# docknetwork/crypto

Hardware: AMD Instinct MI355X
Metric: BLS12-381 G1 MSM/s at n=2^20 (1 GPU) and n=2^24 (8 GPU); bit-exact vs CPU (higher is better)
Workload: dtype i32 (13 signed 30-bit limbs, 381-bit modular integer; 64-bit column accumulators)

## Files before the change

### crypto_amd/csrc/k_g1_pre.hip

```cpp
#include "pre_kernels.hip.h"
#include "msm_launch.hip.h"
namespace msm {
template <class C> void launch_pre_step(hipStream_t s, const uint32_t *prev, size_t n, int c, uint32_t *tmp, uint32_t *out) {
    hipLaunchKernelGGL((k_pre_dbl<typename C::MSM>), dim3((unsigned)((n + 63) / 64)), dim3(64), 0, s, prev, n, c, tmp);
    const size_t groups = (n + PRE_GROUP - 1) / PRE_GROUP;
    hipLaunchKernelGGL((k_pre_norm<typename C::MSM>), dim3((unsigned)((groups + 63) / 64)), dim3(64), 0, s, prev, (const uint32_t *)tmp, n, out);
}
template void launch_pre_step<G1>(hipStream_t, const uint32_t *, size_t, int, uint32_t *, uint32_t *);
}
```

### crypto_amd/csrc/k_g2_pre.hip

```cpp
#include "pre_kernels.hip.h"
#include "msm_launch.hip.h"
namespace msm {
template <class C> void launch_pre_step(hipStream_t s, const uint32_t *prev, size_t n, int c, uint32_t *tmp, uint32_t *out) {
    hipLaunchKernelGGL((k_pre_dbl<typename C::MSM>), dim3((unsigned)((n + 63) / 64)), dim3(64), 0, s, prev, n, c, tmp);
    const size_t groups = (n + PRE_GROUP - 1) / PRE_GROUP;
    hipLaunchKernelGGL((k_pre_norm<typename C::MSM>), dim3((unsigned)((groups + 63) / 64)), dim3(64), 0, s, prev, (const uint32_t *)tmp, n, out);
}
template void launch_pre_step<G2>(hipStream_t, const uint32_t *, size_t, int, uint32_t *, uint32_t *);
}
```

### crypto_amd/csrc/k_psort.hip

```cpp
#include <atomic>
#include "psort_kernels.hip.h"
#include "sort_launch.hip.h"

namespace msm {
void launch_id_flags(hipStream_t s, const uint32_t *bases, int aff_stride, int flag_word, size_t n, uint8_t *out) {
    if (n) hipLaunchKernelGGL(k_id_flags, dim3((unsigned)((n + 255) / 256)), dim3(256), 0, s, bases, aff_stride, flag_word, n, out);
}
void launch_raw_record_hash(hipStream_t s, const uint8_t *raw, size_t stride, size_t x_off, size_t y_off, size_t inf_off, const uint8_t *is_inf, int words, size_t n, uint64_t *out) {
    if (n) hipLaunchKernelGGL(k_raw_record_hash, dim3((unsigned)((n + 255) / 256)), dim3(256), 0, s, raw, stride, x_off, y_off, inf_off, is_inf, words, n, out);
}
void launch_psort(hipStream_t s, const PsParams &q, uint32_t NB, uint32_t *cnt1, uint32_t *off1, uint32_t *bsums, void *pairs, uint32_t *off, uint32_t *entries,
                  uint32_t heavy_thr, uint32_t *heavy, uint32_t heavy_cap, const uint32_t *dyn_args, uint32_t *dyn) {
    const size_t lds1 = (size_t)q.P * 4;
    const size_t lds3 = ((size_t)4 * q.P + 2) * 4 + (size_t)PS_TILE * (size_t)q.W * 8;
    { static std::atomic<uint32_t> done{0}; int dev = 0; (void)hipGetDevice(&dev); const uint32_t bit = 1u << (dev & 31);
      if (!(done.load() & bit)) {
          (void)hipFuncSetAttribute((const void *)k_ps_scatter1<0, 0>, hipFuncAttributeMaxDynamicSharedMemorySize, 160 * 1024 - 2048);
          (void)hipFuncSetAttribute((const void *)k_ps_scatter1<20, 13>, hipFuncAttributeMaxDynamicSharedMemorySize, 160 * 1024 - 2048);
          (void)hipFuncSetAttribute((const void *)k_ps_scatter1<17, 16>, hipFuncAttributeMaxDynamicSharedMemorySize, 160 * 1024 - 2048);
          (void)hipFuncSetAttribute((const void *)k_ps_scatter1<16, 16>, hipFuncAttributeMaxDynamicSharedMemorySize, 160 * 1024 - 2048);
          done.fetch_or(bit); } }
    const int shape = (q.c == 20 && q.W == 13) ? 1 : ((q.c == 17 && q.W == 16) ? 2 : ((q.c == 16 && q.W == 16) ? 3 : 0));
    if (shape == 1) hipLaunchKernelGGL((k_ps_count1<20, 13>), dim3(q.ntiles), dim3(PS_TILE), lds1, s, q, cnt1);
    else if (shape == 2) hipLaunchKernelGGL((k_ps_count1<17, 16>), dim3(q.ntiles), dim3(PS_TILE), lds1, s, q, cnt1);
    else if (shape == 3) hipLaunchKernelGGL((k_ps_count1<16, 16>), dim3(q.ntiles), dim3(PS_TILE), lds1, s, q, cnt1);
    else hipLaunchKernelGGL((k_ps_count1<0, 0>), dim3(q.ntiles), dim3(PS_TILE), lds1, s, q, cnt1);
    launch_scan(s, cnt1, off1, nullptr, bsums, (size_t)q.P * q.ntiles);
    if (dyn) launch_dyn_chunk(s, off1 + (size_t)q.P * q.ntiles, dyn_args[0], dyn_args[1], dyn_args[2], dyn_args[3], dyn_args[4], dyn, dyn_args[5]);
    if (shape == 1) hipLaunchKernelGGL((k_ps_scatter1<20, 13>), dim3(q.ntiles), dim3(PS_TILE), lds3, s, q, (const uint32_t *)cnt1, (const uint32_t *)off1, (uint2 *)pairs);
    else if (shape == 2) hipLaunchKernelGGL((k_ps_scatter1<17, 16>), dim3(q.ntiles), dim3(PS_TILE), lds3, s, q, (const uint32_t *)cnt1, (const uint32_t *)off1, (uint2 *)pairs);
    else if (shape == 3) hipLaunchKernelGGL((k_ps_scatter1<16, 16>), dim3(q.ntiles), dim3(PS_TILE), lds3, s, q, (const uint32_t *)cnt1, (const uint32_t *)off1, (uint2 *)pairs);
    else hipLaunchKernelGGL((k_ps_scatter1<0, 0>), dim3(q.ntiles), dim3(PS_TILE), lds3, s, q, (const uint32_t *)cnt1, (const uint32_t *)off1, (uint2 *)pairs);
    const int wc = ((uint64_t)q.n * (uint64_t)q.W) / q.P >= PS_WC_MIN_PAIRS ? 1 : 0;
    const size_t lds4 = wc ? (size_t)2 * PS_PART * 4 + (size_t)PS_WC_TILE * 8 : (size_t)PS_DIRECT_CAP * 4;
    if (!wc) { static std::atomic<uint32_t> done5{0}; int dev = 0; (void)hipGetDevice(&dev); const uint32_t bit = 1u << (dev & 31);
      if (!(done5.load() & bit)) { (void)hipFuncSetAttribute((const void *)k_ps_bucket<false>, hipFuncAttributeMaxDynamicSharedMemorySize, (int)lds4); done5.fetch_or(bit); } }
    if (wc) { static std::atomic<uint32_t> done4{0}; int dev = 0; (void)hipGetDevice(&dev); const uint32_t bit = 1u << (dev & 31);
      if (!(done4.load() & bit)) { (void)hipFuncSetAttribute((const void *)k_ps_bucket<true>, hipFuncAttributeMaxDynamicSharedMemorySize, (int)lds4); done4.fetch_or(bit); } }
    if (wc) hipLaunchKernelGGL(k_ps_bucket<true>, dim3(q.P), dim3(1024), lds4, s, (const uint2 *)pairs, off1, q.ntiles, q.P, NB, q.part_log, off, entries, heavy_thr, heavy, heavy_cap, (const uint32_t *)dyn);
    else hipLaunchKernelGGL(k_ps_bucket<false>, dim3(q.P), dim3(1024), lds4, s, (const uint2 *)pairs, off1, q.ntiles, q.P, NB, q.part_log, off, entries, heavy_thr, heavy, heavy_cap, (const uint32_t *)dyn);
}
}
```

### crypto_amd/csrc/msm_driver.hip.h

```cpp
#pragma once
#include <chrono>
#include <thread>
#include "dock_ctx.hpp"
#include "bases_cache.hpp"
#include "host_field.hpp"
#include "msm_launch.hip.h"
#include "sort_launch.hip.h"
#include "qap_launch.hip.h"

namespace dock {
using namespace msm;

template <class HF>
void host_fold(const uint64_t *win_abi, const uint8_t *win_inf, int W, int c, uint64_t *out_xyz) {
    typedef hostf::HXyzz<HF> PT;
    PT acc = PT::identity();
    const size_t FWORDS = sizeof(HF) / 8;
    for (int w = W - 1; w >= 0; w--) {
        if (!acc.inf) for (int k = 0; k < c; k++) acc.dbl_in_place();
        if (!win_inf[w]) {
            PT t; t.inf = false;
            const uint64_t *src = win_abi + (size_t)w * 4 * FWORDS;
            memcpy(&t.x, src, sizeof(HF)); memcpy(&t.y, src + FWORDS, sizeof(HF)); memcpy(&t.zz, src + 2 * FWORDS, sizeof(HF)); memcpy(&t.zzz, src + 3 * FWORDS, sizeof(HF));
            acc.add_in_place(t);
        }
    }
    HF X, Y, Z; acc.to_normalised_jacobian(X, Y, Z);
    memcpy(out_xyz, &X, sizeof(HF)); memcpy(out_xyz + FWORDS, &Y, sizeof(HF)); memcpy(out_xyz + 2 * FWORDS, &Z, sizeof(HF));
}

template <class HF>
int32_t host_fold_jacobian(const uint64_t *xyz, size_t k, uint64_t *out_xyz) {
    if (!out_xyz || (k && !xyz)) return DGPU_E_BADARG;
    typedef hostf::HXyzz<HF> PT;
    const size_t FWORDS = sizeof(HF) / 8;
    PT acc = PT::identity();
    for (size_t i = 0; i < k; i++) {
        HF X, Y, Z;
        memcpy(&X, xyz + i * 3 * FWORDS, sizeof(HF)); memcpy(&Y, xyz + i * 3 * FWORDS + FWORDS, sizeof(HF)); memcpy(&Z, xyz + i * 3 * FWORDS + 2 * FWORDS, sizeof(HF));
        if (Z.is_zero()) continue;
        PT t; t.inf = false; t.x = X; t.y = Y; t.zz = Z * Z; t.zzz = t.zz * Z;
        acc.add_in_place(t);
    }
    HF X, Y, Z; acc.to_normalised_jacobian(X, Y, Z);
    memcpy(out_xyz, &X, sizeof(HF)); memcpy(out_xyz + FWORDS, &Y, sizeof(HF)); memcpy(out_xyz + 2 * FWORDS, &Z, sizeof(HF));
    return DGPU_OK;
}

template <class HF>
int32_t host_lincomb(const uint64_t *points_xy, const uint8_t *is_inf, const uint64_t *scalars, size_t k, uint64_t *out_xyz) {
    if (!out_xyz || k > DGPU_MAX_LINCOMB || (k && (!points_xy || !scalars))) return DGPU_E_BADARG;
    typedef hostf::HXyzz<HF> PT;
    const size_t FWORDS = sizeof(HF) / 8;
    std::vector<PT> tab(k * 15);
    std::vector<uint8_t> live(k, 0);
    for (size_t i = 0; i < k; i++) {
        HF X, Y;
        memcpy(&X, points_xy + i * 2 * FWORDS, sizeof(HF)); memcpy(&Y, points_xy + i * 2 * FWORDS + FWORDS, sizeof(HF));
        const uint64_t *sc = scalars + 4 * i;
        uint64_t any = 0; for (size_t w = 0; w < 2 * FWORDS; w++) any |= points_xy[i * 2 * FWORDS + w];
        if ((is_inf && is_inf[i]) || !any || !(sc[0] | sc[1] | sc[2] | sc[3])) continue;
        live[i] = 1;
        PT p; p.inf = false; p.x = X; p.y = Y; p.zz = HF::one(); p.zzz = HF::one();
        tab[i * 15] = p;
        for (int m = 1; m < 15; m++) { PT t = tab[i * 15 + m - 1]; if (m == 1) t.dbl_in_place(); else t.add_in_place(p); tab[i * 15 + m] = t; }
    }
    PT acc = PT::identity();
    for (int w = 63; w >= 0; w--) {
        for (int d = 0; d < 4; d++) acc.dbl_in_place();
        for (size_t i = 0; i < k; i++) {
            if (!live[i]) continue;
            const unsigned nib = (unsigned)(scalars[4 * i + (w >> 4)] >> ((w & 15) * 4)) & 15u;
            if (nib) acc.add_in_place(tab[i * 15 + nib - 1]);
        }
    }
    HF X, Y, Z; acc.to_normalised_jacobian(X, Y, Z);
    memcpy(out_xyz, &X, sizeof(HF)); memcpy(out_xyz + FWORDS, &Y, sizeof(HF)); memcpy(out_xyz + 2 * FWORDS, &Z, sizeof(HF));
    return DGPU_OK;
}

template <class HF> void write_identity(uint64_t *out_xyz) {
    typedef hostf::HXyzz<HF> PT; PT id = PT::identity(); HF X, Y, Z; id.to_normalised_jacobian(X, Y, Z);
    const size_t FWORDS = sizeof(HF) / 8; memcpy(out_xyz, &X, sizeof(HF)); memcpy(out_xyz + FWORDS, &Y, sizeof(HF)); memcpy(out_xyz + 2 * FWORDS, &Z, sizeof(HF));
}

constexpr size_t PLAIN_PSORT_MIN_N = (size_t)1 << 17;
struct PlainGeom {
    int c, W; uint32_t B, NB; int mshift, G; size_t NG, Emax; int CH; size_t T, nblk; bool wide; size_t n_pad; int RANGES, rb_log; unsigned sort_grid; size_t lds_bytes;
    uint32_t min_chunk, max_chunks, lanes_per_chunk, HEAVY_CAP;
    bool psort;
};
template <class C> int32_t plain_geometry(size_t n, PlainGeom &g) {
    if (n >= (1ull << 31)) return DGPU_E_BADARG;
    g.c = choose_c(n, C::NFP == 2);
    g.W = 255 / g.c + 1;
    g.B = 1u << (g.c - 1);
    if ((uint64_t)g.W * g.B >= (1ull << 31) || (uint64_t)n * g.W >= (1ull << 32)) return DGPU_E_BADARG;
    g.NB = (uint32_t)g.W * g.B;
    g.mshift = std::max(0, g.c - 1 - 12);
    g.G = (int)(g.B >> (6 + g.mshift));
    g.NG = (size_t)g.W * g.G;
    g.Emax = (size_t)n * g.W;
    g.CH = C::NFP == 2 ? choose_chunk(g.Emax, 32, 150000, 2) : choose_chunk(g.Emax, 16, 300000, 1);
    g.T = (g.Emax + g.CH - 1) / g.CH;
    g.nblk = scan_blocks(g.NB);
    g.wide = g.c > 16;
    g.n_pad = (n + 7) & ~(size_t)7;
    g.RANGES = 1; while ((g.B / g.RANGES) * 4 > 64 * 1024 || g.W * g.RANGES < 256) { if (g.B / g.RANGES <= 64) break; g.RANGES *= 2; }
    g.rb_log = 0; while ((1u << g.rb_log) < g.B / g.RANGES) g.rb_log++;
    g.sort_grid = (unsigned)(8 * ((g.W + 7) / 8) * g.RANGES);
    g.lds_bytes = ((size_t)1 << g.rb_log) * 4;
    g.min_chunk = C::NFP == 2 ? 32u : 16u; g.max_chunks = C::NFP == 2 ? 150000u : 300000u; g.lanes_per_chunk = C::NFP == 2 ? 2u : 1u;
    g.HEAVY_CAP = (uint32_t)(g.Emax / (16u * 16u)) + 1;
    g.psort = g.W <= PS_MAX_W && n >= PLAIN_PSORT_MIN_N;
    return DGPU_OK;
}
template <class C> int32_t ws_plain(Slot &sl, const PlainGeom &g) {
    int32_t rc;
    const size_t NB = g.NB, T = g.T;
    if ((rc = sl.flags.ensure(64))) return rc;
    if ((rc = sl.cnt.ensure((NB + 1) * 4))) return rc;
    if ((rc = sl.off.ensure((NB + 1) * 4))) return rc;
    if ((rc = sl.cursor.ensure((NB + 1) * 4))) return rc;
    if ((rc = sl.bsums.ensure((g.nblk + 2) * 4))) return rc;
    if ((rc = sl.entries.ensure(g.Emax * 4))) return rc;
    if ((rc = sl.bucket.ensure(soa_points(NB) * C::XW * 4))) return rc;
    if ((rc = sl.bucket_inf.ensure(NB))) return rc;
    if ((rc = sl.head.ensure(soa_points(T) * C::XW * 4))) return rc;
    if ((rc = sl.tail.ensure(soa_points(T) * C::XW * 4))) return rc;
    if ((rc = sl.head_b.ensure(T * 4))) return rc;
    if ((rc = sl.tail_b.ensure(T * 4))) return rc;
    if ((rc = sl.part_inf.ensure(T * 2))) return rc;
    if ((rc = sl.l1.ensure(g.NG * 2 * C::XW * 4))) return rc;
    if ((rc = sl.l1_inf.ensure(g.NG * 2))) return rc;
    if ((rc = sl.win.ensure((size_t)g.W * 4 * C::ABI_W * 4))) return rc;
    if ((rc = sl.win_inf.ensure(g.W))) return rc;
    if ((rc = sl.digits.ensure((size_t)g.W * g.n_pad * (g.wide ? 4 : 2)))) return rc;
    if (g.psort) {
        const size_t n_terms = g.Emax / g.W;
        const uint32_t P = (g.NB + (1u << ps_part_log(g.NB)) - 1) >> ps_part_log(g.NB);
        const size_t n1 = (size_t)P * ((n_terms + PS_TILE - 1) / PS_TILE);
        if ((rc = sl.cnt.ensure((n1 + 1) * 4))) return rc;
        if ((rc = sl.cursor.ensure((n1 + 1) * 4))) return rc;
        if ((rc = sl.bsums.ensure((scan_blocks(n1) + 2) * 4))) return rc;
        if ((rc = sl.digits.ensure(g.Emax * 8))) return rc;
    }
    if ((rc = sl.heavy.ensure(((size_t)g.HEAVY_CAP + 1) * 4))) return rc;
    if ((rc = sl.dyn.ensure(msm::dyn_words(T) * 4))) return rc;
    { const size_t hslots = 2 * (T / msm::HEAVY_RANGE + 2); if ((rc = sl.hpart.ensure(hslots * C::XW * 4))) return rc; if ((rc = sl.hpart_inf.ensure(hslots))) return rc; }
    return DGPU_OK;
}

inline size_t range_count(size_t n, bool operands_in_flight) { return operands_in_flight && n >= ((size_t)1 << 19) ? 2 : 1; }
inline size_t range_lo(size_t n, size_t K, size_t k) { return ((n * k / K) + 7) & ~(size_t)7; }
inline void range_bounds(size_t n, size_t K, size_t k, size_t &lo, size_t &hi) { lo = k == 0 ? 0 : std::min(n, range_lo(n, K, k)); hi = k + 1 == K ? n : std::min(n, range_lo(n, K, k + 1)); }
template <class C> int32_t ws_bucket_sets(Slot &sl, uint32_t NB, size_t K) {
    int32_t rc;
    if ((rc = sl.bucket.ensure(K * soa_points(NB) * C::XW * 4))) return rc;
    return sl.bucket_inf.ensure(K * (size_t)NB);
}

struct SmallSub { const uint32_t *tab; const uint8_t *tab_inf; };
template <class C> inline size_t small_sub_tab_bytes(size_t n) { return n * SMALL_MSM_S * SMALL_MSM_E * (size_t)C::ACC::XW * 4; }
template <class C> inline size_t small_sub_bytes(size_t n) { return small_sub_tab_bytes<C>(n) + n * SMALL_MSM_S * SMALL_MSM_E; }
template <class C> inline SmallSub small_sub_at(const void *aux, size_t handle_n, size_t offset) {
    const uint8_t *base = (const uint8_t *)aux;
    return SmallSub{(const uint32_t *)base + offset * SMALL_MSM_S * SMALL_MSM_E * (size_t)C::ACC::XW, base + small_sub_tab_bytes<C>(handle_n) + offset * SMALL_MSM_S * SMALL_MSM_E};
}
template <class C> int32_t ws_small(Slot &sl, size_t n) {
    int32_t rc;
    typedef typename C::ACC A;
    if ((rc = sl.bucket.ensure(n * SMALL_MSM_E * A::XW * 4))) return rc;
    if ((rc = sl.bucket_inf.ensure(n * SMALL_MSM_E))) return rc;
    if ((rc = sl.head.ensure((size_t)256 * A::XW * 4))) return rc;
    if ((rc = sl.part_inf.ensure(256))) return rc;
    if (!sl.small_cnt.p) {
        if ((rc = sl.small_cnt.ensure((size_t)SMALL_MSM_W * 4))) return rc;
        if (hipMemsetAsync(sl.small_cnt.p, 0, (size_t)SMALL_MSM_W * 4, sl.stream) != hipSuccess) { (void)hipGetLastError(); sl.small_cnt.release(); return DGPU_E_HIP; }
    }
    return sl.win.ensure((size_t)SMALL_MSM_W * 4 * C::ABI_W * 4 + 2 * SMALL_MSM_W);
}
template <class C, class HF, class ReadyS, class ReadyB>
int32_t msm_device_small(Slot &sl, const uint32_t *d_bases, const uint32_t *d_scalars, size_t n, uint64_t *out_xyz, ReadyS ready_scalars, ReadyB ready_bases, const SmallSub *sub = nullptr) {
    int32_t rc;
    if ((rc = ws_small<C>(sl, sub ? 1 : n))) return rc;
    hipStream_t s = sl.stream;
    constexpr int c = SMALL_MSM_C;
    const int S = sub ? SMALL_MSM_S : 1, W = SMALL_MSM_W / S;
    if ((rc = ready_scalars(0, 0, n))) return rc;
    if ((rc = ready_bases(0, 0, n))) return rc;
    constexpr size_t WBYTES = (size_t)SMALL_MSM_W * 4 * C::ABI_W * 4;
    static_assert(WBYTES + 2 * SMALL_MSM_W <= Slot::HPIN_BYTES, "pinned scratch");
    uint8_t *const hbuf = (uint8_t *)sl.hpin;
    uint8_t *const wbuf = hbuf;
    uint8_t *const d_inf = wbuf + WBYTES, *const d_bad = d_inf + SMALL_MSM_W;
    if (!sub) {
        StageTimer st(sl, "msm.small_table");
        launch_small_table<C>(s, d_bases, n, sl.bucket.as<uint32_t>(), sl.bucket_inf.as<uint8_t>());
    }
    {
        StageTimer st(sl, "msm.small_tree");
        launch_small_tree<C>(s, sub ? sub->tab : sl.bucket.as<uint32_t>(), sub ? sub->tab_inf : sl.bucket_inf.as<uint8_t>(), S, d_scalars, n, sl.head.as<uint32_t>(), sl.part_inf.as<uint8_t>(),
                             sl.small_cnt.as<uint32_t>(), (uint32_t *)wbuf, d_inf, d_bad);
    }
    HIPCHK(hipGetLastError());
    HIPCHK(hipStreamSynchronize(s));
    if (gs.prof) prof_flush(sl);
    const uint64_t *hwin = (const uint64_t *)hbuf; const uint8_t *hinf = hbuf + WBYTES, *hbad = hinf + SMALL_MSM_W;
    for (int w = 0; w < W; w++) if (hbad[w]) return DGPU_E_BADARG;
    host_fold<HF>(hwin, hinf, W, c, out_xyz);
    return DGPU_OK;
}

template <class C, class HF, class ReadyS, class ReadyB>
int32_t msm_device_ranges(Slot &sl, const uint32_t *d_bases, const uint32_t *d_scalars, size_t n, size_t K, uint64_t *out_xyz, bool bases_pending, ReadyS ready_scalars, ReadyB ready_bases, const SmallSub *sub = nullptr) {
    if (n == 0) { write_identity<HF>(out_xyz); return DGPU_OK; }
    if (K == 1 && n <= gs.small_max.load() && n <= SMALL_MSM_MAX_N) return msm_device_small<C, HF>(sl, d_bases, d_scalars, n, out_xyz, ready_scalars, ready_bases, sub);
    PlainGeom g; int32_t rc;
    if ((rc = plain_geometry<C>(n, g))) return rc;
    if ((rc = ws_plain<C>(sl, g))) return rc;
    if (K > 1 && (rc = ws_bucket_sets<C>(sl, g.NB, K))) return rc;
    const int c = g.c, W = g.W; const uint32_t NB = g.NB; const size_t T = g.T; const int CH = g.CH;
    hipStream_t s = sl.stream;
    const uint32_t heavy_thr = 0xffffffffu , HEAVY_CAP = g.HEAVY_CAP;
    uint32_t *const dyn = sl.dyn.as<uint32_t>();
    const size_t set_words = soa_points(NB) * C::XW;
    HIPCHK(hipMemsetAsync(sl.bucket_inf.p, 1, K * (size_t)NB, s));
    HIPCHK(hipMemsetAsync(sl.flags.p, 0, 4, s));
    for (size_t k = 0; k < K; k++) {
        size_t lo, hi; range_bounds(n, K, k, lo, hi);
        const size_t nk = hi - lo, nk_pad = (nk + 7) & ~(size_t)7;
        if (nk == 0) continue;
        uint32_t *const bucket = sl.bucket.as<uint32_t>() + k * set_words;
        uint8_t *const bucket_inf = sl.bucket_inf.as<uint8_t>() + k * (size_t)NB;
        const uint32_t *const bases_k = d_bases + lo * C::AFF_STRIDE, *const scalars_k = d_scalars + lo * 8;
        if ((rc = ready_scalars(k, lo, hi))) return rc;
        if (g.psort) {
            StageTimer st(sl, "msm.psort");
            PsParams q;
            q.scalars = scalars_k; q.idflag = nullptr ; q.n = nk; q.flag_base = 0;
            q.c = c; q.W = W; q.key_wstride = g.B; q.val_base = 0; q.val_wstride = 0;
            q.part_log = ps_part_log(NB); q.P = (NB + (1u << q.part_log) - 1) >> q.part_log; q.ntiles = (uint32_t)((nk + PS_TILE - 1) / PS_TILE);
            q.bad = sl.flags.as<uint32_t>();
            const uint32_t dyn_args[6] = {(uint32_t)forced_chunk(), g.min_chunk, g.max_chunks, g.lanes_per_chunk, (uint32_t)T, 0u};
            HIPCHK(hipMemsetAsync(sl.heavy.p, 0, 4, s));
            launch_psort(s, q, NB, sl.cnt.as<uint32_t>(), sl.cursor.as<uint32_t>(), sl.bsums.as<uint32_t>(), sl.digits.p, sl.off.as<uint32_t>(), sl.entries.as<uint32_t>(),
                         16u * (uint32_t)CH , sl.heavy.as<uint32_t>(), HEAVY_CAP, dyn_args, dyn);
        } else {
        {
            StageTimer st(sl, "msm.count");
            HIPCHK(hipMemsetAsync(sl.heavy.p, 0, 4, s));
            launch_digit_codes(s, g.wide, scalars_k, bases_pending ? nullptr : bases_k, C::AFF_STRIDE, C::FLAGW, nk, nk_pad, c, W, sl.digits.p, sl.flags.as<uint32_t>());
            launch_sort_sweep(s, g.wide, false, g.sort_grid, g.lds_bytes, sl.digits.p, nk, nk_pad, W, g.RANGES, g.rb_log, g.B, sl.cnt.as<uint32_t>(), nullptr, nullptr, heavy_thr, sl.heavy.as<uint32_t>(), HEAVY_CAP);
        }
        {
            StageTimer st(sl, "msm.scan");
            launch_scan(s, sl.cnt.as<uint32_t>(), sl.off.as<uint32_t>(), sl.cursor.as<uint32_t>(), sl.bsums.as<uint32_t>(), (size_t)NB);
            launch_dyn_chunk(s, sl.off.as<uint32_t>() + NB, (uint32_t)forced_chunk(), g.min_chunk, g.max_chunks, g.lanes_per_chunk, (uint32_t)T, dyn);
            launch_flag_heavy(s, sl.off.as<uint32_t>(), NB, dyn, sl.heavy.as<uint32_t>(), HEAVY_CAP);
        }
        {
            StageTimer st(sl, "msm.scatter");
            launch_sort_sweep(s, g.wide, true, g.sort_grid, g.lds_bytes, sl.digits.p, nk, nk_pad, W, g.RANGES, g.rb_log, g.B, nullptr, sl.off.as<uint32_t>(), sl.entries.as<uint32_t>(), heavy_thr, sl.heavy.as<uint32_t>(), HEAVY_CAP);
        }
        }
        if ((rc = ready_bases(k, lo, hi))) return rc;
        {
            StageTimer st(sl, "msm.accumulate");
#ifdef DGPU_DEV
            static const uint32_t dbg_mask = getenv("DGPU_DBG_NOGATHER") ? 1023u : 0xffffffffu;
#else
            constexpr uint32_t dbg_mask = 0xffffffffu;
#endif
            if (bases_pending || g.psort) launch_accumulate_skip_identity<C>(s, bases_k, sl.entries.as<uint32_t>(), sl.off.as<uint32_t>(), NB, bucket, bucket_inf,
                               sl.head.as<uint32_t>(), sl.tail.as<uint32_t>(), sl.head_b.as<uint32_t>(), sl.tail_b.as<uint32_t>(), sl.part_inf.as<uint8_t>(), T, (uint32_t)CH, dyn, msm::RowMap{});
            else launch_accumulate<C>(s, bases_k, sl.entries.as<uint32_t>(), sl.off.as<uint32_t>(), NB, bucket, bucket_inf,
                               sl.head.as<uint32_t>(), sl.tail.as<uint32_t>(), sl.head_b.as<uint32_t>(), sl.tail_b.as<uint32_t>(), sl.part_inf.as<uint8_t>(), T, (uint32_t)CH, dbg_mask, dyn);
        }
        {
            StageTimer st(sl, "msm.fixup");
            launch_fixup<C>(s, NB, bucket, bucket_inf, sl.head.as<uint32_t>(), sl.tail.as<uint32_t>(),
                               sl.head_b.as<uint32_t>(), sl.tail_b.as<uint32_t>(), sl.part_inf.as<uint8_t>(), T, sl.off.as<uint32_t>(), heavy_thr, dyn);
            launch_fixup_heavy<C>(s, sl.heavy.as<uint32_t>(), HEAVY_CAP, sl.off.as<uint32_t>(), (uint32_t)CH, NB, bucket, bucket_inf,
                               sl.head.as<uint32_t>(), sl.tail.as<uint32_t>(), sl.part_inf.as<uint8_t>(), T, dyn, sl.hpart.as<uint32_t>(), sl.hpart_inf.as<uint8_t>());
            if (k > 0) launch_merge_buckets<C>(s, NB, sl.bucket.as<uint32_t>(), sl.bucket_inf.as<uint8_t>(), bucket, bucket_inf);
        }
    }
    {
        StageTimer st(sl, "msm.reduce");
        launch_reduce_l0<C>(s, (unsigned)g.NG, sl.bucket.as<uint32_t>(), sl.bucket_inf.as<uint8_t>(), NB, g.mshift, sl.l1.as<uint32_t>(), sl.l1_inf.as<uint8_t>());
        launch_reduce_top<C>(s, (unsigned)W, sl.l1.as<uint32_t>(), sl.l1_inf.as<uint8_t>(), g.G, 6 + g.mshift, sl.win.as<uint32_t>(), sl.win_inf.as<uint8_t>(), gs.reduce_lanes.load() == 1 ? 1 : 4);
    }
    HIPCHK(hipGetLastError());
    std::vector<uint64_t> hwin((size_t)W * 2 * C::ABI_W);
    std::vector<uint8_t> hinf(W);
    const size_t wb = (size_t)W * 4 * C::ABI_W * 4, ib = ((size_t)W + 7) & ~(size_t)7;
    static_assert((size_t)64 * 4 * 24 * 4 + 64 + 16 <= Slot::HPIN_BYTES, "pinned scratch");
    std::vector<uint8_t> big;
    if (wb + ib + 4 > Slot::HPIN_BYTES) big.resize(wb + ib + 4);
    uint8_t *const hp = big.empty() ? (uint8_t *)sl.hpin : big.data();
    HIPCHK(hipMemcpyAsync(hp, sl.win.p, wb, hipMemcpyDeviceToHost, s));
    HIPCHK(hipMemcpyAsync(hp + wb, sl.win_inf.p, W, hipMemcpyDeviceToHost, s));
    HIPCHK(hipMemcpyAsync(hp + wb + ib, sl.flags.p, 4, hipMemcpyDeviceToHost, s));
    auto tsync0 = std::chrono::steady_clock::now();
    HIPCHK(hipStreamSynchronize(s));
    auto tsync1 = std::chrono::steady_clock::now();
    if (gs.prof) prof_flush(sl);
    uint32_t hbad; memcpy(&hbad, hp + wb + ib, 4);
    if (hbad) return DGPU_E_BADARG;
    memcpy(hwin.data(), hp, wb); memcpy(hinf.data(), hp + wb, W);
    host_fold<HF>(hwin.data(), hinf.data(), W, c, out_xyz);
    if (gs.prof) {
        auto t2 = std::chrono::steady_clock::now();
        prof_add_host("msm.host_wait", std::chrono::duration<double, std::milli>(tsync1 - tsync0).count());
        prof_add_host("msm.host_fold", std::chrono::duration<double, std::milli>(t2 - tsync1).count());
    }
    return DGPU_OK;
}
template <class C, class HF>
int32_t msm_device(Slot &sl, const uint32_t *d_bases, const uint32_t *d_scalars, size_t n, uint64_t *out_xyz, const SmallSub *sub = nullptr) {
    auto nothing = [](size_t, size_t, size_t) { return (int32_t)DGPU_OK; };
    return msm_device_ranges<C, HF>(sl, d_bases, d_scalars, n, 1, out_xyz, false, nothing, nothing, sub);
}

template <class C>
bool small_sub_for(Slot &sl, uint64_t handle_id, const Handle &h, size_t offset, size_t n, SmallSub &out, bool force = false) {
    if (h.n == 0 || h.n > SMALL_MSM_MAX_N || n > gs.small_max.load()) return false;
    void *aux = nullptr;
    {
        std::lock_guard<std::mutex> lk(gs.mu);
        auto it = gs.handles.find(handle_id);
        if (it == gs.handles.end()) return false;
        aux = it->second.aux;
        if (!aux && !force && ++it->second.small_uses < 2) return false;
    }
    if (!aux) {
        std::lock_guard<std::mutex> build(gs.small_mu);
        { std::lock_guard<std::mutex> lk(gs.mu); auto it = gs.handles.find(handle_id); if (it == gs.handles.end()) return false; aux = it->second.aux; }
        if (!aux) {
            void *p = nullptr;
            if (dev_malloc(&p, small_sub_bytes<C>(h.n)) != hipSuccess) { (void)hipGetLastError(); return false; }
            {
                StageTimer st(sl, "msm.small_subtable");
                launch_small_subtable<C>(sl.stream, (const uint32_t *)h.p, h.n, (uint32_t *)p, (uint8_t *)p + small_sub_tab_bytes<C>(h.n));
            }
            if (hipGetLastError() != hipSuccess || hipStreamSynchronize(sl.stream) != hipSuccess) { (void)hipGetLastError(); (void)hipFree(p); return false; }
            std::lock_guard<std::mutex> lk(gs.mu);
            auto it = gs.handles.find(handle_id);
            if (it == gs.handles.end()) { (void)hipFree(p); return false; }
            it->second.aux = aux = p;
        }
    }
    out = small_sub_at<C>(aux, h.n, offset);
    return true;
}

inline void shard_bounds(size_t n, size_t parts, std::vector<size_t> &lo) {
    lo.resize(parts + 1);
    const size_t base = n / parts, rem = n % parts;
    for (size_t k = 0; k <= parts; k++) lo[k] = k * base + std::min(k, rem);
}
template <class F> int32_t run_shards(size_t parts, F body) { return par_run(parts, body); }

inline int choose_c_pre(size_t n) {
    if (gs.window_bits.load() >= 16 && gs.window_bits.load() <= 22) return gs.window_bits.load();
    if (n < (1u << 15)) return 0;
    return n >= 320000 ? 20 : 16;
}

template <class HF>
void host_fold_shared(const uint64_t *a_abi, const uint8_t *a_inf, const uint64_t *s_abi, const uint8_t *s_inf, int PW, int lb, uint64_t *out_xyz) {
    typedef hostf::HXyzz<HF> PT;
    const size_t FWORDS = sizeof(HF) / 8;
    auto load = [&](const uint64_t *src, bool inf) { PT t = PT::identity(); if (!inf) { t.inf = false; memcpy(&t.x, src, sizeof(HF)); memcpy(&t.y, src + FWORDS, sizeof(HF)); memcpy(&t.zz, src + 2 * FWORDS, sizeof(HF)); memcpy(&t.zzz, src + 3 * FWORDS, sizeof(HF)); } return t; };
    PT suffix = PT::identity(), weighted = PT::identity(), total = PT::identity();
    for (int j = PW - 1; j >= 1; j--) { suffix.add_in_place(load(s_abi + (size_t)j * 4 * FWORDS, s_inf[j] != 0)); weighted.add_in_place(suffix); }
    for (int k = 0; k < lb; k++) weighted.dbl_in_place();
    for (int j = 0; j < PW; j++) total.add_in_place(load(a_abi + (size_t)j * 4 * FWORDS, a_inf[j] != 0));
    total.add_in_place(weighted);
    HF X, Y, Z; total.to_normalised_jacobian(X, Y, Z);
    memcpy(out_xyz, &X, sizeof(HF)); memcpy(out_xyz + FWORDS, &Y, sizeof(HF)); memcpy(out_xyz + 2 * FWORDS, &Z, sizeof(HF));
}

template <class HF>
void host_fold_marginals(const uint64_t *pts, const uint8_t *inf, int nm, int shift, uint64_t *out_xyz) {
    typedef hostf::HXyzz<HF> PT;
    const size_t FWORDS = sizeof(HF) / 8;
    auto load = [&](int i) { PT t = PT::identity(); if (!inf[i]) { const uint64_t *src = pts + (size_t)i * 4 * FWORDS; t.inf = false; memcpy(&t.x, src, sizeof(HF)); memcpy(&t.y, src + FWORDS, sizeof(HF)); memcpy(&t.zz, src + 2 * FWORDS, sizeof(HF)); memcpy(&t.zzz, src + 3 * FWORDS, sizeof(HF)); } return t; };
    PT acc = PT::identity();
    for (int t = nm - 1; t >= 0; t--) { if (!acc.inf) acc.dbl_in_place(); acc.add_in_place(load(1 + t)); }
    if (!acc.inf) for (int k = 0; k < shift; k++) acc.dbl_in_place();
    acc.add_in_place(load(0));
    HF X, Y, Z; acc.to_normalised_jacobian(X, Y, Z);
    memcpy(out_xyz, &X, sizeof(HF)); memcpy(out_xyz + FWORDS, &Y, sizeof(HF)); memcpy(out_xyz + 2 * FWORDS, &Z, sizeof(HF));
}

struct PreGeom { uint32_t NB; int mshift, lb, PW, G; size_t NG, Emax, T; int CH; uint32_t min_chunk, max_chunks, lanes_per_chunk, HEAVY_CAP; };
template <class C> int32_t pre_geometry(const PreTable &pt, size_t n, PreGeom &g) {
    const int c = pt.c, W = pt.W;
    g.NB = 1u << (c - 1);
    g.mshift = g.NB >= (1u << 18) ? 3 : (g.NB >= (1u << 17) ? 2 : (g.NB >= (1u << 16) ? 1 : 0));
    if (g.NB >= (1u << 19) && cur().busy.load() >= 3) g.mshift = 4;
    { const int f = gs.reduce_shift.load(); if (f >= 0 && c - 1 >= 6 + f) g.mshift = f; }
    g.lb = std::min(c - 1, 12 + g.mshift);
    g.PW = (int)(g.NB >> g.lb);
    g.G = 1 << (g.lb - 6 - g.mshift);
    g.NG = (size_t)g.PW * g.G;
    g.Emax = (size_t)n * W;
    if (g.Emax >= (1ull << 32) || (uint64_t)W * pt.n >= (1ull << 31) || W > PS_MAX_W) return DGPU_E_BADARG;
    g.CH = C::NFP == 2 ? choose_chunk(g.Emax, 32, 150000, 2) : choose_chunk(g.Emax, 16, 300000, 1);
    g.T = (g.Emax + g.CH - 1) / g.CH;
    g.min_chunk = C::NFP == 2 ? 32u : 16u; g.max_chunks = C::NFP == 2 ? 150000u : 300000u; g.lanes_per_chunk = C::NFP == 2 ? 2u : 1u;
    g.HEAVY_CAP = (uint32_t)(g.Emax / (16u * 16u)) + 1;
    return DGPU_OK;
}
template <class C> int32_t ws_pre(Slot &sl, const PreTable &pt, const PreGeom &g, size_t n) {
    const uint32_t NB = g.NB; const size_t T = g.T; const int PW = g.PW;
    const uint32_t P = (NB + (1u << ps_part_log(NB)) - 1) >> ps_part_log(NB);
    const size_t n1 = (size_t)P * ((n + PS_TILE - 1) / PS_TILE);
    int32_t rc;
    if ((rc = sl.flags.ensure(64))) return rc;
    if ((rc = sl.cnt.ensure((n1 + 1) * 4))) return rc;
    if ((rc = sl.cursor.ensure((n1 + 1) * 4))) return rc;
    if ((rc = sl.bsums.ensure((scan_blocks(n1) + 2) * 4))) return rc;
    if ((rc = sl.digits.ensure(g.Emax * 8))) return rc;
    if ((rc = sl.heavy.ensure(((size_t)g.HEAVY_CAP + 1) * 4))) return rc;
    if ((rc = sl.off.ensure(((size_t)NB + 1) * 4))) return rc;
    if ((rc = sl.entries.ensure(g.Emax * 4))) return rc;
    if ((rc = sl.bucket.ensure(soa_points(NB) * C::XW * 4))) return rc;
    if ((rc = sl.bucket_inf.ensure(NB))) return rc;
    if ((rc = sl.head.ensure(soa_points(T) * C::XW * 4))) return rc;
    if ((rc = sl.tail.ensure(soa_points(T) * C::XW * 4))) return rc;
    if ((rc = sl.head_b.ensure(T * 4))) return rc;
    if ((rc = sl.tail_b.ensure(T * 4))) return rc;
    if ((rc = sl.part_inf.ensure(T * 2))) return rc;
    const size_t NGw = std::max(g.NG, (size_t)(NB >> 9)), PWw = std::max((size_t)PW, (size_t)(NB >> 15));
    const size_t mpts = reduce_marginals_points<C>(NGw);
    if ((rc = sl.l1.ensure(std::max(NGw * 2, mpts) * C::XW * 4))) return rc;
    if ((rc = sl.l1_inf.ensure(std::max(NGw * 2, mpts)))) return rc;
    if ((rc = sl.win.ensure(std::max((size_t)2 * PWw, (size_t)32) * 4 * C::ABI_W * 4))) return rc;
    if ((rc = sl.win_inf.ensure(std::max((size_t)2 * PWw, (size_t)32)))) return rc;
    if ((rc = sl.dyn.ensure(msm::dyn_words(T) * 4))) return rc;
    { const size_t hslots = 2 * (T / msm::HEAVY_RANGE + 2); if ((rc = sl.hpart.ensure(hslots * C::XW * 4))) return rc; if ((rc = sl.hpart_inf.ensure(hslots))) return rc; }
    (void)pt;
    return DGPU_OK;
}
template <class C> inline size_t pre_rows_bytes(size_t n, int W) { return (size_t)W * n * C::AFF_STRIDE * 4; }
template <class C> inline size_t pre_tab_bytes(size_t n, int W) { return pre_rows_bytes<C>(n, W) + ((n + 15) & ~(size_t)15); }
template <class C> inline const uint8_t *pre_idflags(const PreTable &pt) { return (const uint8_t *)pt.tab + pre_rows_bytes<C>(pt.n, pt.W); }
inline size_t pre_off_bytes(const PreTable &pt) { return (((size_t)1 << (pt.c - 1)) + 1) * 4; }
inline size_t pre_entries_bytes(const PreTable &pt, size_t n) { return (size_t)n * pt.W * 4; }

template <class C>
int32_t pre_sort(Slot &sl, const PreTable &pt, const PreGeom &g, size_t boff, const uint32_t *d_scalars, size_t n, uint32_t *off, uint32_t *entries, uint32_t *dyn, bool reset_flag = true) {
    PsParams q;
    q.scalars = d_scalars; q.idflag = dyn ? pre_idflags<C>(pt) : nullptr ; q.n = n; q.flag_base = (uint32_t)boff;
    q.c = pt.c; q.W = pt.W; q.key_wstride = 0; q.val_base = (uint32_t)boff; q.val_wstride = (uint32_t)pt.n;
    q.part_log = ps_part_log(g.NB); q.P = (g.NB + (1u << q.part_log) - 1) >> q.part_log; q.ntiles = (uint32_t)((n + PS_TILE - 1) / PS_TILE);
    int32_t rc;
    if ((rc = ws_pre<C>(sl, pt, g, n))) return rc;
    q.bad = sl.flags.as<uint32_t>();
    const uint32_t heavy_thr = dyn ? 16u * (uint32_t)g.CH  : 0xffffffffu ;
    const uint32_t dyn_args[6] = {(uint32_t)forced_chunk(), g.min_chunk, g.max_chunks, g.lanes_per_chunk, (uint32_t)g.T, g.NB};
    StageTimer st(sl, "msm.psort");
    HIPCHK(hipMemsetAsync(sl.heavy.p, 0, 4, sl.stream));
    if (reset_flag) HIPCHK(hipMemsetAsync(sl.flags.p, 0, 4, sl.stream));
    launch_psort(sl.stream, q, g.NB, sl.cnt.as<uint32_t>(), sl.cursor.as<uint32_t>(), sl.bsums.as<uint32_t>(), sl.digits.p, off, entries,
                 heavy_thr, sl.heavy.as<uint32_t>(), g.HEAVY_CAP, dyn_args, dyn);
    return DGPU_OK;
}
template <class C>
int32_t pre_acc(Slot &sl, const PreTable &pt, const PreGeom &g, const uint32_t *off, const uint32_t *entries, bool derive_dyn, const msm::RowMap &map, size_t set) {
    const uint32_t NB = g.NB; const size_t T = g.T;
    uint32_t *const dyn = sl.dyn.as<uint32_t>();
    const uint32_t heavy_thr = 16u * (uint32_t)g.CH;
    hipStream_t s = sl.stream;
    uint32_t *const bucket = sl.bucket.as<uint32_t>() + set * soa_points(NB) * C::XW;
    uint8_t *const bucket_inf = sl.bucket_inf.as<uint8_t>() + set * (size_t)NB;
    HIPCHK(hipMemsetAsync(bucket_inf, 1, NB, s));
    if (derive_dyn) {
        HIPCHK(hipMemsetAsync(sl.heavy.p, 0, 4, s));
        launch_dyn_chunk(s, off + NB, (uint32_t)forced_chunk(), g.min_chunk, g.max_chunks, g.lanes_per_chunk, (uint32_t)T, dyn, NB);
        launch_flag_heavy(s, off, NB, dyn, sl.heavy.as<uint32_t>(), g.HEAVY_CAP);
    }
    {
        StageTimer st(sl, "msm.accumulate");
        if (derive_dyn) launch_accumulate_skip_identity<C>(s, (const uint32_t *)pt.tab, entries, off, NB, bucket, bucket_inf,
                           sl.head.as<uint32_t>(), sl.tail.as<uint32_t>(), sl.head_b.as<uint32_t>(), sl.tail_b.as<uint32_t>(), sl.part_inf.as<uint8_t>(), T, (uint32_t)g.CH, dyn, map);
        else launch_accumulate<C>(s, (const uint32_t *)pt.tab, entries, off, NB, bucket, bucket_inf,
                           sl.head.as<uint32_t>(), sl.tail.as<uint32_t>(), sl.head_b.as<uint32_t>(), sl.tail_b.as<uint32_t>(), sl.part_inf.as<uint8_t>(), T, (uint32_t)g.CH, 0xffffffffu, dyn);
    }
    {
        StageTimer st(sl, "msm.fixup");
        launch_fixup<C>(s, NB, bucket, bucket_inf, sl.head.as<uint32_t>(), sl.tail.as<uint32_t>(),
                           sl.head_b.as<uint32_t>(), sl.tail_b.as<uint32_t>(), sl.part_inf.as<uint8_t>(), T, off, heavy_thr, dyn);
        launch_fixup_heavy<C>(s, sl.heavy.as<uint32_t>(), g.HEAVY_CAP, off, (uint32_t)g.CH, NB, bucket, bucket_inf,
                           sl.head.as<uint32_t>(), sl.tail.as<uint32_t>(), sl.part_inf.as<uint8_t>(), T, dyn, sl.hpart.as<uint32_t>(), sl.hpart_inf.as<uint8_t>());
        if (set > 0) launch_merge_buckets<C>(s, NB, sl.bucket.as<uint32_t>(), sl.bucket_inf.as<uint8_t>(), bucket, bucket_inf);
    }
    return DGPU_OK;
}
template <class C, class HF>
int32_t pre_finish(Slot &sl, const PreGeom &g, bool check_flag, uint64_t *out_xyz) {
    const uint32_t NB = g.NB; const int PW = g.PW;
    hipStream_t s = sl.stream;
    uint32_t *win_a = sl.win.as<uint32_t>(), *win_s = win_a + (size_t)PW * 4 * C::ABI_W;
    uint8_t *inf_a = sl.win_inf.as<uint8_t>(), *inf_s = inf_a + PW;
    const int rl = gs.reduce_lanes.load();
    const bool marginals = (rl == 0 || rl == 2) && g.NG >= 2;
    int nm = 0;
    {
        StageTimer st(sl, "msm.reduce");
        if (marginals) nm = launch_reduce_marginals<C>(s, (unsigned)g.NG, sl.bucket.as<uint32_t>(), sl.bucket_inf.as<uint8_t>(), NB, g.mshift, sl.l1.as<uint32_t>(), sl.l1_inf.as<uint8_t>(), win_a, inf_a, rl == 0);
        else {
            launch_reduce_l0<C>(s, (unsigned)g.NG, sl.bucket.as<uint32_t>(), sl.bucket_inf.as<uint8_t>(), NB, g.mshift, sl.l1.as<uint32_t>(), sl.l1_inf.as<uint8_t>());
            launch_reduce_top_s<C>(s, (unsigned)PW, sl.l1.as<uint32_t>(), sl.l1_inf.as<uint8_t>(), g.G, 6 + g.mshift, win_a, inf_a, win_s, inf_s, gs.reduce_lanes.load() == 1 ? 1 : 4);
        }
    }
    HIPCHK(hipGetLastError());
    const size_t npts = marginals ? (size_t)nm + 1 : (size_t)2 * PW;
    std::vector<uint64_t> hwin(npts * 2 * C::ABI_W);
    std::vector<uint8_t> hinf(npts);
    const size_t wb = npts * 4 * C::ABI_W * 4, ib = (npts + 7) & ~(size_t)7;
    std::vector<uint8_t> big;
    if (wb + ib + 4 > Slot::HPIN_BYTES) big.resize(wb + ib + 4);
    uint8_t *const hp = big.empty() ? (uint8_t *)sl.hpin : big.data();
    memset(hp + wb + ib, 0, 4);
    HIPCHK(hipMemcpyAsync(hp, sl.win.p, wb, hipMemcpyDeviceToHost, s));
    HIPCHK(hipMemcpyAsync(hp + wb, sl.win_inf.p, npts, hipMemcpyDeviceToHost, s));
    if (check_flag) HIPCHK(hipMemcpyAsync(hp + wb + ib, sl.flags.p, 4, hipMemcpyDeviceToHost, s));
    auto tsync0 = std::chrono::steady_clock::now();
    HIPCHK(hipStreamSynchronize(s));
    auto tsync1 = std::chrono::steady_clock::now();
    if (gs.prof) prof_flush(sl);
    uint32_t hbad; memcpy(&hbad, hp + wb + ib, 4);
    if (hbad) return DGPU_E_BADARG;
    memcpy(hwin.data(), hp, wb); memcpy(hinf.data(), hp + wb, npts);
    if (marginals) host_fold_marginals<HF>(hwin.data(), hinf.data(), nm, g.mshift + (C::NFP == 2 ? 1 : 0), out_xyz);
    else host_fold_shared<HF>(hwin.data(), hinf.data(), hwin.data() + (size_t)PW * 2 * C::ABI_W, hinf.data() + PW, PW, g.lb, out_xyz);
    if (gs.prof) {
        auto t2 = std::chrono::steady_clock::now();
        prof_add_host("msm.host_wait", std::chrono::duration<double, std::milli>(tsync1 - tsync0).count());
        prof_add_host("msm.host_fold", std::chrono::duration<double, std::milli>(t2 - tsync1).count());
    }
    return DGPU_OK;
}
template <class C, class HF>
int32_t pre_tail(Slot &sl, const PreTable &pt, const PreGeom &g, const uint32_t *off, const uint32_t *entries, bool derive_dyn, uint64_t *out_xyz, const msm::RowMap &map = msm::RowMap{}) {
    int32_t rc;
    if ((rc = ws_pre<C>(sl, pt, g, g.Emax / pt.W))) return rc;
    if ((rc = pre_acc<C>(sl, pt, g, off, entries, derive_dyn, map, 0))) return rc;
    return pre_finish<C, HF>(sl, g, !derive_dyn, out_xyz);
}
template <class C, class HF, class ReadyS>
int32_t msm_device_pre_ranges(Slot &sl, const PreTable &pt, size_t boff, const uint32_t *d_scalars, size_t n, size_t K, uint64_t *out_xyz, ReadyS ready_scalars) {
    if (n == 0) { write_identity<HF>(out_xyz); return DGPU_OK; }
    PreGeom g; int32_t rc;
    if ((rc = pre_geometry<C>(pt, n, g))) return rc;
    if ((rc = ws_pre<C>(sl, pt, g, n))) return rc;
    if (K > 1 && (rc = ws_bucket_sets<C>(sl, g.NB, K))) return rc;
    HIPCHK(hipMemsetAsync(sl.flags.p, 0, 4, sl.stream));
    for (size_t k = 0; k < K; k++) {
        size_t lo, hi; range_bounds(n, K, k, lo, hi);
        if (hi == lo) continue;
        if ((rc = ready_scalars(k, lo, hi))) return rc;
        if ((rc = pre_sort<C>(sl, pt, g, boff + lo, d_scalars + lo * 8, hi - lo, sl.off.as<uint32_t>(), sl.entries.as<uint32_t>(), sl.dyn.as<uint32_t>(), false))) return rc;
        if ((rc = pre_acc<C>(sl, pt, g, sl.off.as<uint32_t>(), sl.entries.as<uint32_t>(), false, msm::RowMap{}, k))) return rc;
    }
    return pre_finish<C, HF>(sl, g, true, out_xyz);
}
template <class C, class HF>
int32_t msm_device_pre(Slot &sl, const PreTable &pt, size_t boff, const uint32_t *d_scalars, size_t n, uint64_t *out_xyz) {
    return msm_device_pre_ranges<C, HF>(sl, pt, boff, d_scalars, n, 1, out_xyz, [](size_t, size_t, size_t) { return (int32_t)DGPU_OK; });
}

inline int32_t scalars_sort(uint64_t table, size_t boff, uint64_t scalars, size_t soff, size_t n, uint64_t *sorted) {
    if (!sorted || n == 0) return DGPU_E_BADARG;
    if (!cur().ready) return DGPU_E_NODEVICE;
    HandleRef hb(table), hs(scalars);
    if (!hb.ok || !hs.ok || (hb.h.kind != 10 && hb.h.kind != 11) || hs.h.kind != 3 || hb.h.ctx != hs.h.ctx) return DGPU_E_BADARG;
    if (boff > hb.h.n || n > hb.h.n - boff || soff > hs.h.n || n > hs.h.n - soff) return DGPU_E_BADARG;
    CtxScope on_owner(hb.h.ctx);
    SLOT_ACQUIRE(L, sl);
    HIPCHK(hipSetDevice(cur().device));
    const PreTable &pt = *(const PreTable *)hb.h.p;
    PreGeom g; int32_t rc;
    if ((rc = pre_geometry<G1>(pt, n, g))) return rc;
    SortedScalars *ss = new SortedScalars{nullptr, nullptr, pre_off_bytes(pt), pre_entries_bytes(pt, n), n, pt.n, boff, pt.c, pt.W};
    ss->off = scalar_alloc(ss->off_bytes); ss->entries = scalar_alloc(ss->entries_bytes);
    auto drop = [&]() { scalar_release(cur_index(), ss->off, ss->off_bytes); scalar_release(cur_index(), ss->entries, ss->entries_bytes); delete ss; };
    if (!ss->off || !ss->entries) { drop(); return DGPU_E_OOM; }
    rc = pre_sort<G1>(sl, pt, g, boff, (const uint32_t *)hs.h.p + soff * 8, n, (uint32_t *)ss->off, (uint32_t *)ss->entries, nullptr);
    uint32_t hbad = 0;
    if (!rc && hipMemcpyAsync(&hbad, sl.flags.p, 4, hipMemcpyDeviceToHost, sl.stream) != hipSuccess) rc = DGPU_E_HIP;
    if (!rc && hipStreamSynchronize(sl.stream) != hipSuccess) { gs.last_hip = (int32_t)hipGetLastError(); rc = DGPU_E_HIP; }
    if (gs.prof) prof_flush(sl);
    if (!rc && hbad) rc = DGPU_E_BADARG;
    if (rc) { drop(); return rc; }
    *sorted = register_handle(ss, n, 12);
    return DGPU_OK;
}
template <class C, class HF>
int32_t msm_sorted(uint64_t table, uint64_t sorted, size_t row_shift, uint64_t *out, int kind) {
    if (!out) return DGPU_E_BADARG;
    if (!cur().ready) return DGPU_E_NODEVICE;
    HandleRef hb(table), hs(sorted);
    if (!hb.ok || !hs.ok || hb.h.kind != kind + 9 || hs.h.kind != 12 || hb.h.ctx != hs.h.ctx) return DGPU_E_BADARG;
    const PreTable &pt = *(const PreTable *)hb.h.p;
    const SortedScalars &ss = *(const SortedScalars *)hs.h.p;
    if (pt.c != ss.c || pt.W != ss.W || row_shift >= ss.rows || pt.n != ss.rows - row_shift) return DGPU_E_BADARG;
    CtxScope on_owner(hb.h.ctx);
    SLOT_ACQUIRE(L, sl);
    HIPCHK(hipSetDevice(cur().device));
    PreGeom g; int32_t rc;
    if ((rc = pre_geometry<C>(pt, ss.n, g))) return rc;
    msm::RowMap map;
    if (row_shift) {
        map.rows_src = (uint32_t)ss.rows; map.rows_dst = (uint32_t)pt.n; map.shift = (uint32_t)row_shift;
        map.magic = ~(uint64_t)0 / ss.rows + 1;
    }
    return pre_tail<C, HF>(sl, pt, g, (const uint32_t *)ss.off, (const uint32_t *)ss.entries, true, out, map);
}

template <class C> int32_t reserve_slots(int what, size_t n, size_t stride, const PreTable *pt);

template <class C>
int32_t bases_precompute(uint64_t handle, int32_t window_bits, int kind ) {
    if (window_bits != 0 && (window_bits < 16 || window_bits > 22)) return DGPU_E_BADARG;
    Handle hd;
    { Handle peek; if (!lookup_handle(handle, peek)) return DGPU_E_BADARG;
      if (peek.kind == kind + 6) {
          HandleRef ref(handle); if (!ref.ok) return DGPU_E_BADARG;
          const ShardSet &ss = *(const ShardSet *)ref.h.p;
          return run_shards(ss.sub.size(), [&](size_t k) { return bases_precompute<C>(ss.sub[k], window_bits, kind); });
      }
      if (peek.kind == kind + 9) return DGPU_OK; }
    if (!take_handle(handle, [kind](int k) { return k == kind; }, hd)) return DGPU_E_BADARG;
    auto put_back = [&](void *p, int k) { std::lock_guard<std::mutex> lk(gs.mu); gs.handles[handle] = Handle{p, hd.n, k, hd.ctx, 0, k == kind ? hd.aux : nullptr, hd.small_uses}; };
    CtxScope on_owner(hd.ctx);
    if (!cur().ready) { put_back(hd.p, kind); return DGPU_E_NODEVICE; }
    const size_t n = hd.n;
    const int c = window_bits ? window_bits : choose_c_pre(n);
    if (c == 0) {
        put_back(hd.p, kind);
        if (n && n <= SMALL_MSM_MAX_N) {
            HandleRef ref(handle);
            if (ref.ok) { SlotLock L; if (L.ok && hipSetDevice(cur().device) == hipSuccess) { SmallSub sub; (void)small_sub_for<C>(*L.s, handle, ref.h, 0, 0, sub, true); } }
        }
        return DGPU_OK;
    }
    const int W = 255 / c + 1;
    if (n == 0 || (uint64_t)W * n >= (1ull << 31)) { put_back(hd.p, kind); return n == 0 ? DGPU_OK : DGPU_E_BADARG; }
    void *tab = nullptr, *tmp = nullptr;
    int32_t rc = DGPU_OK;
    {
        SLOT_ACQUIRE(L, sl);
        if (hipSetDevice(cur().device) != hipSuccess) rc = DGPU_E_HIP;
        const size_t rec = (size_t)C::AFF_STRIDE * 4;
        if (!rc && dev_malloc(&tab, pre_tab_bytes<C>(n, W)) != hipSuccess) { (void)hipGetLastError(); rc = DGPU_E_OOM; }
        if (!rc && dev_malloc(&tmp, n * (size_t)C::XW * 4) != hipSuccess) { (void)hipGetLastError(); rc = DGPU_E_OOM; }
        if (!rc && hipMemcpyAsync(tab, hd.p, n * rec, hipMemcpyDeviceToDevice, sl.stream) != hipSuccess) rc = DGPU_E_HIP;
        if (!rc) {
            StageTimer st(sl, "msm.precompute");
            for (int w = 1; w < W; w++) launch_pre_step<C>(sl.stream, (const uint32_t *)tab + (size_t)(w - 1) * n * C::AFF_STRIDE, n, c, (uint32_t *)tmp, (uint32_t *)tab + (size_t)w * n * C::AFF_STRIDE);
            launch_id_flags(sl.stream, (const uint32_t *)tab, C::AFF_STRIDE, C::FLAGW, n, (uint8_t *)tab + pre_rows_bytes<C>(n, W));
        }
        if (!rc && (hipGetLastError() != hipSuccess || hipStreamSynchronize(sl.stream) != hipSuccess)) rc = DGPU_E_HIP;
        if (gs.prof) prof_flush(sl);
        if (tmp) (void)hipFree(tmp);
    }
    if (rc) { if (tab) (void)hipFree(tab); (void)hipGetLastError(); put_back(hd.p, kind); return rc; }
    (void)hipFree(hd.p);
    if (hd.aux) (void)hipFree(hd.aux);
    PreTable *npt = new PreTable{tab, n, c, W};
    put_back(npt, kind + 9);
    (void)reserve_slots<C>(3, n, 0, npt);
    return DGPU_OK;
}

struct RawBases {
    const uint8_t *p; size_t stride, x_off, y_off, inf_off; const uint8_t *is_inf;
    template <class C> static RawBases packed(const uint64_t *xy, const uint8_t *is_inf) {
        return RawBases{(const uint8_t *)xy, (size_t)2 * C::ABI_W * 4, 0, (size_t)C::ABI_W * 4, msm::NO_INF_OFF, is_inf};
    }
    template <class C> bool ok() const {
        const size_t fb = (size_t)C::ABI_W * 4;
        return stride >= 2 * fb && stride % 8 == 0 && x_off % 8 == 0 && y_off % 8 == 0 && x_off + fb <= stride && y_off + fb <= stride &&
               (inf_off == msm::NO_INF_OFF || inf_off < stride) && ((uintptr_t)p % 8) == 0 && stride <= 4096;
    }
};
constexpr size_t STAGE_CHUNK_BYTES = (size_t)16 << 20;

template <class C> int32_t ws_stage_bases(Slot &sl, const RawBases &rb, size_t n) {
    int32_t rc;
    if ((rc = sl.in_bases.ensure(n * rb.stride + 16))) return rc;
    if (rb.is_inf && (rc = sl.in_inf.ensure(n + 16))) return rc;
    return DGPU_OK;
}
template <class C>
int32_t stage_bases(Slot &sl, const RawBases &rb, size_t lo0, size_t hi0, uint32_t *d_out) {
    if (hi0 <= lo0) return DGPU_OK;
    const size_t n = hi0 - lo0;
    uint8_t *draw = sl.in_bases.as<uint8_t>();
    const uint8_t *dinf = nullptr;
    if (rb.is_inf) { HIPCHK(hipMemcpyAsync(sl.in_inf.as<uint8_t>() + lo0, rb.is_inf + lo0, n, hipMemcpyHostToDevice, sl.cstream)); dinf = sl.in_inf.as<uint8_t>(); }
    const size_t per = std::max<size_t>(1, STAGE_CHUNK_BYTES / rb.stride);
    size_t pieces = (n + per - 1) / per;
    if (pieces > 6) pieces = 6;
    const size_t len = (n + pieces - 1) / pieces;
    StageTimer st(sl, "msm.prep_bases");
    for (size_t lo = lo0; lo < hi0; lo += len) {
        const size_t cnt = std::min(len, hi0 - lo);
        hipEvent_t ev = sl.copy_ev[sl.ev_next++ % (Slot::N_COPY_EV + 1)];
        HIPCHK(hipMemcpyAsync(draw + lo * rb.stride, rb.p + lo * rb.stride, cnt * rb.stride, hipMemcpyHostToDevice, sl.cstream));
        HIPCHK(hipEventRecord(ev, sl.cstream));
        HIPCHK(hipStreamWaitEvent(sl.stream, ev, 0));
        launch_prep_bases_raw<C>(sl.stream, draw + lo * rb.stride, rb.stride, rb.x_off, rb.y_off, rb.inf_off, dinf ? dinf + lo : nullptr, cnt, d_out + lo * C::AFF_STRIDE);
    }
    return DGPU_OK;
}
template <class C> int32_t stage_bases(Slot &sl, const RawBases &rb, size_t n, uint32_t *d_out) { return stage_bases<C>(sl, rb, 0, n, d_out); }
inline int32_t stage_scalars(Slot &sl, const uint64_t *h, size_t lo, size_t hi, bool mont, uint32_t *d_out) {
    if (hi <= lo) return DGPU_OK;
    hipEvent_t ev = sl.copy_ev[sl.ev_next++ % (Slot::N_COPY_EV + 1)];
    HIPCHK(hipMemcpyAsync(d_out + lo * 8, h + lo * 4, (hi - lo) * 32, hipMemcpyHostToDevice, sl.cstream));
    HIPCHK(hipEventRecord(ev, sl.cstream));
    HIPCHK(hipStreamWaitEvent(sl.stream, ev, 0));
    if (mont) ntt::launch_fr_mont_to_canonical(sl.stream, d_out + lo * 8, hi - lo);
    return DGPU_OK;
}
inline int32_t stage_scalars(Slot &sl, const uint64_t *h, size_t n, bool mont, uint32_t *d_out) { return stage_scalars(sl, h, 0, n, mont, d_out); }

template <class C> int32_t ws_for(Slot &sl, int what, size_t n, size_t stride, const PreTable *pt) {
    if (n == 0) return DGPU_OK;
    int32_t rc;
    if ((rc = sl.in_scalars.ensure(n * 32))) return rc;
    if (what == 1) {
        if ((rc = sl.in_bases.ensure(n * stride + 16))) return rc;
        if ((rc = sl.in_inf.ensure(n + 16))) return rc;
        if ((rc = sl.prepped.ensure(n * C::AFF_STRIDE * 4))) return rc;
    }
    if (what == 3) { PreGeom g; if ((rc = pre_geometry<C>(*pt, n, g))) return rc; if ((rc = ws_pre<C>(sl, *pt, g, n))) return rc; return ws_bucket_sets<C>(sl, g.NB, range_count(n, true)); }
    if (n <= SMALL_MSM_MAX_N && (rc = ws_small<C>(sl, n))) return rc;
    PlainGeom g; if ((rc = plain_geometry<C>(n, g))) return rc;
    if ((rc = ws_plain<C>(sl, g))) return rc;
    return ws_bucket_sets<C>(sl, g.NB, range_count(n, true));
}
template <class C> int32_t reserve_slots(int what, size_t n, size_t stride, const PreTable *pt) {
    Ctx &cx = cur();
    if (!cx.ready) return DGPU_E_NODEVICE;
    int32_t first = DGPU_OK;
    for (int k = 0; k < N_SLOTS; k++) {
        std::lock_guard<std::mutex> lk(cx.slots[k].mu);
        if (hipSetDevice(cx.device) != hipSuccess) return DGPU_E_HIP;
        const int32_t rc = ws_for<C>(cx.slots[k], what, n, stride, pt);
        if (rc && !first) first = rc;
    }
    return first;
}
template <class C> void reserve_idle_slots(const Slot *mine, int what, size_t n, size_t stride) {
    Ctx &cx = cur();
    for (int k = 0; k < N_SLOTS; k++) {
        Slot &o = cx.slots[k];
        if (&o == mine || !o.mu.try_lock()) continue;
        (void)ws_for<C>(o, what, n, stride, nullptr);
        o.mu.unlock();
    }
}

template <class C, class HF>
int32_t msm_oneshot_here(const RawBases &rb, const uint64_t *scalars, size_t n, bool mont, uint64_t *out) {
    if (!cur().ready) return DGPU_E_NODEVICE;
    SLOT_ACQUIRE(L, sl);
    HIPCHK(hipSetDevice(cur().device));
    if (n == 0) { write_identity<HF>(out); return DGPU_OK; }
    int32_t rc;
    const uint64_t allocs0 = g_dev_allocs.load();
    if ((rc = ws_for<C>(sl, 1, n, rb.stride, nullptr))) return rc;
    const size_t K = range_count(n, true);
    const bool grew = g_dev_allocs.load() != allocs0;
    rc = msm_device_ranges<C, HF>(sl, sl.prepped.as<uint32_t>(), sl.in_scalars.as<uint32_t>(), n, K, out, true,
                                  [&](size_t, size_t lo, size_t hi) { return stage_scalars(sl, scalars, lo, hi, mont, sl.in_scalars.as<uint32_t>()); },
                                  [&](size_t, size_t lo, size_t hi) { return stage_bases<C>(sl, rb, lo, hi, sl.prepped.as<uint32_t>()); });
    if (rc) { (void)hipStreamSynchronize(sl.cstream); (void)hipStreamSynchronize(sl.stream); }
    if (grew) reserve_idle_slots<C>(&sl, 1, n, rb.stride);
    return rc;
}
template <class C, class HF> bool msm_oneshot_cached(const RawBases &rb, const uint64_t *scalars, size_t n, bool mont, uint64_t *out, int kind, int32_t &rc);
template <class C, class HF>
int32_t msm_oneshot_ctx(const RawBases &rb, const uint64_t *scalars, size_t n, bool mont, uint64_t *out) {
    if (gcache.enabled.load(std::memory_order_relaxed) && n >= gcache.min_n.load(std::memory_order_relaxed)) {
        int32_t rc;
        if (msm_oneshot_cached<C, HF>(rb, scalars, n, mont, out, C::NFP, rc)) return rc;
    }
    return msm_oneshot_here<C, HF>(rb, scalars, n, mont, out);
}
template <class C, class HF>
int32_t msm_oneshot(const RawBases &rb, const uint64_t *scalars, size_t n, bool mont, uint64_t *out) {
    if (!out || (n && (!rb.p || !scalars)) || n >= (1ull << 31) || !rb.ok<C>()) return DGPU_E_BADARG;
    if (!cur().ready) return DGPU_E_NODEVICE;
    if (!tl_no_min && n < gs.min_gpu_n) return DGPU_E_TOO_SMALL;
    if (n >= gs.auto_shard_min_n.load(std::memory_order_relaxed)) {
        const std::vector<int> cx = ready_contexts(0);
        if (cx.size() > 1) {
            std::vector<size_t> lo; shard_bounds(n, cx.size(), lo);
            const size_t JW = 3 * sizeof(HF) / 8;
            std::vector<uint64_t> parts(cx.size() * JW);
            const int32_t rc = run_shards(cx.size(), [&](size_t k) {
                CtxScope here(cx[k]);
                RawBases part = rb; part.p = rb.p + lo[k] * rb.stride; if (rb.is_inf) part.is_inf = rb.is_inf + lo[k];
                return msm_oneshot_ctx<C, HF>(part, scalars + lo[k] * 4, lo[k + 1] - lo[k], mont, parts.data() + k * JW);
            });
            if (rc) return rc;
            return host_fold_jacobian<HF>(parts.data(), cx.size(), out);
        }
    }
    return msm_oneshot_ctx<C, HF>(rb, scalars, n, mont, out);
}

template <class C>
void bases_register(void *p, size_t n, uint64_t *handle, int kind) {
    *handle = register_handle(p, n, kind);
    (void)reserve_slots<C>(2, n, 0, nullptr);
    if (n && n <= SMALL_MSM_MAX_N && n <= gs.small_max.load()) {
        HandleRef ref(*handle);
        if (ref.ok) { SlotLock L; if (L.ok && hipSetDevice(cur().device) == hipSuccess) { SmallSub sub; (void)small_sub_for<C>(*L.s, *handle, ref.h, 0, 0, sub, true); } }
    }
}
template <class C>
int32_t bases_upload(const RawBases &rb, size_t n, uint64_t *handle, int kind, std::vector<uint64_t> *rec_hash = nullptr) {
    if (!handle || (n && !rb.p) || n >= (1ull << 31) || !rb.ok<C>()) return DGPU_E_BADARG;
    if (!cur().ready) return DGPU_E_NODEVICE;
    void *p = nullptr;
    {
        SLOT_ACQUIRE(L, sl);
        HIPCHK(hipSetDevice(cur().device));
        if (dev_malloc(&p, std::max<size_t>(n, 1) * C::AFF_STRIDE * 4) != hipSuccess) { (void)hipGetLastError(); return DGPU_E_OOM; }
        int32_t rc = ws_stage_bases<C>(sl, rb, n);
        if (!rc) rc = stage_bases<C>(sl, rb, n, (uint32_t *)p);
        if (!rc && rec_hash && n) {
            rc = sl.digits.ensure(n * 8);
            if (!rc) {
                launch_raw_record_hash(sl.stream, sl.in_bases.as<uint8_t>(), rb.stride, rb.x_off, rb.y_off, rb.inf_off, rb.is_inf ? sl.in_inf.as<uint8_t>() : nullptr, C::ABI_W / 2, n, sl.digits.as<uint64_t>());
                if (hipMemcpyAsync(rec_hash->data(), sl.digits.p, n * 8, hipMemcpyDeviceToHost, sl.stream) != hipSuccess) { (void)hipGetLastError(); rc = DGPU_E_HIP; }
            }
        }
        if (hipStreamSynchronize(sl.cstream) != hipSuccess || hipStreamSynchronize(sl.stream) != hipSuccess) { if (!rc) rc = DGPU_E_HIP; }
        if (gs.prof) prof_flush(sl);
        if (rc) { (void)hipFree(p); return rc; }
    }
    bases_register<C>(p, n, handle, kind);
    return DGPU_OK;
}

template <class C, class HF>
int32_t msm_handle(uint64_t bases, size_t offset, const uint64_t *scalars, size_t n, int mont, uint64_t *out, int kind, bool check_min = true) {
    if (!out || (n && !scalars)) return DGPU_E_BADARG;
    if (!cur().ready) return DGPU_E_NODEVICE;
    if (check_min && !tl_no_min && n < std::min<size_t>(gs.min_gpu_n, DGPU_MIN_GPU_N_HANDLE)) return DGPU_E_TOO_SMALL;
    HandleRef hb(bases);
    if (!hb.ok || (hb.h.kind != kind && hb.h.kind != kind + 9) || offset > hb.h.n || n > hb.h.n - offset) return DGPU_E_BADARG;
    CtxScope on_owner(hb.h.ctx);
    SLOT_ACQUIRE(L, sl);
    HIPCHK(hipSetDevice(cur().device));
    int32_t rc;
    if ((rc = sl.in_scalars.ensure(std::max<size_t>(n, 1) * 32))) return rc;
    const size_t K = range_count(n, true);
    auto ready = [&](size_t, size_t lo, size_t hi) { return stage_scalars(sl, scalars, lo, hi, mont != 0, sl.in_scalars.as<uint32_t>()); };
    auto nothing = [](size_t, size_t, size_t) { return (int32_t)DGPU_OK; };
    if (hb.h.kind == kind + 9) rc = msm_device_pre_ranges<C, HF>(sl, *(const PreTable *)hb.h.p, offset, sl.in_scalars.as<uint32_t>(), n, K, out, ready);
    else {
        SmallSub sub; const bool have = K == 1 && n && small_sub_for<C>(sl, bases, hb.h, offset, n, sub);
        rc = msm_device_ranges<C, HF>(sl, (const uint32_t *)hb.h.p + offset * C::AFF_STRIDE, sl.in_scalars.as<uint32_t>(), n, K, out, false, ready, nothing, have ? &sub : nullptr);
    }
    if (rc) { (void)hipStreamSynchronize(sl.cstream); (void)hipStreamSynchronize(sl.stream); }
    return rc;
}

inline size_t many_chunk_rows(size_t n) {
    const int forced = gs.many_chunk.load();
    if (forced > 0) return (size_t)forced;
    const size_t r = ((size_t)1 << 17) / std::max<size_t>(n, 1);
    return std::min<size_t>(4096, std::max<size_t>(r, 1));
}
template <class C> int32_t ws_many(Slot &sl, size_t n, size_t rows, const ManyGeom &g) {
    int32_t rc;
    typedef typename C::ACC A;
    constexpr size_t WPS = SMALL_MSM_W / SMALL_MSM_S;
    if ((rc = sl.flags.ensure(64))) return rc;
    if ((rc = sl.in_scalars.ensure(rows * n * 32))) return rc;
    if ((rc = sl.bucket.ensure(rows * WPS * A::XW * 4))) return rc;
    if ((rc = sl.bucket_inf.ensure(rows * WPS))) return rc;
    if (g.nblk > 1) {
        if ((rc = sl.head.ensure(rows * WPS * g.nblk * A::XW * 4))) return rc;
        if ((rc = sl.part_inf.ensure(rows * WPS * g.nblk))) return rc;
        if ((rc = sl.cnt.ensure(rows * WPS * 4))) return rc;
    }
    if ((rc = sl.win.ensure(rows * 3 * C::ABI_W * 4))) return rc;
    return sl.win_inf.ensure(rows);
}
template <class C>
int32_t msm_device_many(Slot &sl, const SmallSub &sub, const uint64_t *scalars, size_t row_stride, size_t n, size_t m, bool mont, uint64_t *out, uint8_t *out_inf) {
    int32_t rc;
    constexpr size_t JW = 3 * C::ABI_W / 2;
    const ManyGeom g = many_geometry(n);
    const size_t chunk = std::min(m, many_chunk_rows(n));
    const uint64_t allocs0 = g_dev_allocs.load();
    if ((rc = ws_many<C>(sl, n, chunk, g))) return rc;
    if (g_dev_allocs.load() != allocs0) {
        Ctx &cx = cur();
        for (int k = 0; k < N_SLOTS; k++) {
            Slot &o = cx.slots[k];
            if (&o == &sl || !o.mu.try_lock()) continue;
            (void)ws_many<C>(o, n, chunk, g);
            o.mu.unlock();
        }
    }
    hipStream_t s = sl.stream;
    uint32_t *const d_sc = sl.in_scalars.as<uint32_t>(), *const d_bad = sl.flags.as<uint32_t>();
    HIPCHK(hipMemsetAsync(d_bad, 0, 4, s));
    uint32_t *const hbad = (uint32_t *)sl.hpin;
    for (size_t r0 = 0; r0 < m; r0 += chunk) {
        const size_t rows = std::min(chunk, m - r0);
        const uint64_t *src = scalars + r0 * row_stride * 4;
        hipEvent_t ev = sl.copy_ev[sl.ev_next++ % (Slot::N_COPY_EV + 1)];
        if (row_stride == n) HIPCHK(hipMemcpyAsync(d_sc, src, rows * n * 32, hipMemcpyHostToDevice, sl.cstream));
        else HIPCHK(hipMemcpy2DAsync(d_sc, n * 32, src, row_stride * 32, n * 32, rows, hipMemcpyHostToDevice, sl.cstream));
        HIPCHK(hipEventRecord(ev, sl.cstream));
        HIPCHK(hipStreamWaitEvent(s, ev, 0));
        if (mont) ntt::launch_fr_mont_to_canonical(s, d_sc, rows * n);
        if (g.nblk > 1) HIPCHK(hipMemsetAsync(sl.cnt.p, 0, rows * (SMALL_MSM_W / SMALL_MSM_S) * 4, s));
        {
            StageTimer st(sl, "msm.many_tree");
            launch_many_tree<C>(s, sub.tab, sub.tab_inf, d_sc, n, n, rows, sl.head.as<uint32_t>(), sl.part_inf.as<uint8_t>(), sl.cnt.as<uint32_t>(), sl.bucket.as<uint32_t>(), sl.bucket_inf.as<uint8_t>(), d_bad);
        }
        {
            StageTimer st(sl, "msm.many_fold");
            launch_many_fold<C>(s, sl.bucket.as<uint32_t>(), sl.bucket_inf.as<uint8_t>(), rows, sl.win.as<uint32_t>(), sl.win_inf.as<uint8_t>());
        }
        HIPCHK(hipGetLastError());
        HIPCHK(hipMemcpyAsync(out + r0 * JW, sl.win.p, rows * JW * 8, hipMemcpyDeviceToHost, s));
        if (out_inf) HIPCHK(hipMemcpyAsync(out_inf + r0, sl.win_inf.p, rows, hipMemcpyDeviceToHost, s));
        HIPCHK(hipMemcpyAsync(hbad, d_bad, 4, hipMemcpyDeviceToHost, s));
        HIPCHK(hipStreamSynchronize(s));
        if (gs.prof) prof_flush(sl);
        if (*hbad) return DGPU_E_BADARG;
    }
    return DGPU_OK;
}
template <class C, class HF>
int32_t msm_handle_many(uint64_t bases, size_t offset, const uint64_t *scalars, size_t row_stride, size_t n, size_t m, int mont, uint64_t *out, uint8_t *out_inf, int kind) {
    if (m == 0) return DGPU_OK;
    constexpr size_t JW = 3 * sizeof(HF) / 8;
    if (!out || (n && (!scalars || row_stride < n)) || m >= (1ull << 31) || n >= (1ull << 31) || row_stride >= (1ull << 31)) return DGPU_E_BADARG;
    if (!cur().ready) return DGPU_E_NODEVICE;
    if (!tl_no_min && m * n < std::min<size_t>(gs.min_gpu_n, DGPU_MIN_GPU_N_HANDLE)) return DGPU_E_TOO_SMALL;
    bool served = false;
    int32_t rc = DGPU_OK;
    {
        HandleRef hb(bases);
        if (!hb.ok || (hb.h.kind != kind && hb.h.kind != kind + 9) || offset > hb.h.n || n > hb.h.n - offset) return DGPU_E_BADARG;
        if (n == 0) {
            for (size_t j = 0; j < m; j++) { write_identity<HF>(out + j * JW); if (out_inf) out_inf[j] = 1; }
            return DGPU_OK;
        }
        if (hb.h.kind == kind && hb.h.n <= SMALL_MSM_MAX_N && n <= gs.small_max.load()) {
            CtxScope on_owner(hb.h.ctx);
            SLOT_ACQUIRE(L, sl);
            HIPCHK(hipSetDevice(cur().device));
            SmallSub sub;
            if (small_sub_for<C>(sl, bases, hb.h, offset, n, sub, true)) {
                served = true;
                rc = msm_device_many<C>(sl, sub, scalars, row_stride, n, m, mont != 0, out, out_inf);
                if (rc) { (void)hipStreamSynchronize(sl.cstream); (void)hipStreamSynchronize(sl.stream); }
            }
        }
    }
    if (served) return rc;
    for (size_t j = 0; j < m; j++) {
        if ((rc = msm_handle<C, HF>(bases, offset, scalars + 4 * row_stride * j, n, mont, out + j * JW, kind, false))) return rc;
        if (out_inf) { uint64_t z = 0; for (size_t k = 2 * JW / 3; k < JW; k++) z |= out[j * JW + k]; out_inf[j] = z == 0; }
    }
    return DGPU_OK;
}

constexpr size_t SEG_CHUNK_TERMS = (size_t)1 << 16, SEG_CHUNK_SEGS = 4096;
constexpr size_t SEG_DEVICE_FOLD_MIN = 24;
template <class C> int32_t ws_seg(Slot &sl, const RawBases &rb, size_t terms, size_t nseg, size_t blocks, size_t pslots) {
    int32_t rc;
    typedef typename C::ACC A;
    constexpr size_t W = SMALL_MSM_W, WIN_BYTES = std::max<size_t>(A::XW * 4, 4 * C::ABI_W * 4);
    if ((rc = sl.flags.ensure(64))) return rc;
    if ((rc = sl.in_scalars.ensure(terms * 32))) return rc;
    if ((rc = ws_stage_bases<C>(sl, rb, terms))) return rc;
    if ((rc = sl.prepped.ensure(terms * C::AFF_STRIDE * 4))) return rc;
    if ((rc = sl.bucket.ensure(terms * SMALL_MSM_E * A::XW * 4))) return rc;
    if ((rc = sl.bucket_inf.ensure(terms * SMALL_MSM_E))) return rc;
    if ((rc = sl.entries.ensure(blocks * 64 * sizeof(SegDesc)))) return rc;
    if ((rc = sl.l1.ensure(nseg * W * WIN_BYTES))) return rc;
    if ((rc = sl.l1_inf.ensure(nseg * W))) return rc;
    if (pslots) {
        if ((rc = sl.head.ensure(pslots * W * A::XW * 4))) return rc;
        if ((rc = sl.part_inf.ensure(pslots * W))) return rc;
        if ((rc = sl.cnt.ensure(pslots * W * 4))) return rc;
    }
    if ((rc = sl.win.ensure(nseg * 3 * C::ABI_W * 4))) return rc;
    return sl.win_inf.ensure(nseg);
}
inline bool jac_is_identity(const uint64_t *xyz, size_t JW) { uint64_t z = 0; for (size_t k = 2 * JW / 3; k < JW; k++) z |= xyz[k]; return z == 0; }
template <class C, class HF>
int32_t msm_seg_chunk(Slot &sl, const RawBases &rb, const uint64_t *scalars, const uint64_t *seg_end, size_t s0, size_t s1, bool mont, const SegLayout &lay, bool device_fold,
                      std::vector<uint64_t> &hwin, std::vector<uint8_t> &hinf, uint64_t *out, uint8_t *out_inf) {
    constexpr size_t JW = 3 * sizeof(HF) / 8, W = SMALL_MSM_W, WW = 4 * sizeof(HF) / 8;
    const size_t t0 = s0 ? seg_end[s0 - 1] : 0, T = seg_end[s1 - 1] - t0, ns = s1 - s0;
    hipStream_t s = sl.stream;
    uint32_t *const d_sc = sl.in_scalars.as<uint32_t>(), *const d_bad = sl.flags.as<uint32_t>();
    uint32_t *const hbad = (uint32_t *)sl.hpin;
    int32_t rc;
    HIPCHK(hipMemsetAsync(d_bad, 0, 4, s));
    HIPCHK(hipMemcpyAsync(sl.entries.p, lay.desc.data(), lay.blocks * 64 * sizeof(SegDesc), hipMemcpyHostToDevice, sl.cstream));
    RawBases part = rb; part.p = rb.p + t0 * rb.stride; if (rb.is_inf) part.is_inf = rb.is_inf + t0;
    if ((rc = stage_scalars(sl, scalars + t0 * 4, T, mont, d_sc))) return rc;
    if ((rc = stage_bases<C>(sl, part, T, sl.prepped.as<uint32_t>()))) return rc;
    {
        StageTimer st(sl, "msm.small_table");
        launch_small_table<C>(s, sl.prepped.as<uint32_t>(), T, sl.bucket.as<uint32_t>(), sl.bucket_inf.as<uint8_t>());
    }
    if (lay.pslots) HIPCHK(hipMemsetAsync(sl.cnt.p, 0, lay.pslots * W * 4, s));
    {
        StageTimer st(sl, "msm.seg_tree");
        launch_seg_tree<C>(s, sl.bucket.as<uint32_t>(), sl.bucket_inf.as<uint8_t>(), d_sc, sl.entries.p, lay.blocks, sl.head.as<uint32_t>(), sl.part_inf.as<uint8_t>(), sl.cnt.as<uint32_t>(),
                           sl.l1.as<uint32_t>(), sl.l1_inf.as<uint8_t>(), !device_fold, d_bad);
    }
    if (device_fold) {
        {
            StageTimer st(sl, "msm.seg_fold");
            launch_seg_fold<C>(s, sl.l1.as<uint32_t>(), sl.l1_inf.as<uint8_t>(), ns, sl.win.as<uint32_t>(), sl.win_inf.as<uint8_t>());
        }
        HIPCHK(hipGetLastError());
        HIPCHK(hipMemcpyAsync(out + s0 * JW, sl.win.p, ns * JW * 8, hipMemcpyDeviceToHost, s));
        if (out_inf) HIPCHK(hipMemcpyAsync(out_inf + s0, sl.win_inf.p, ns, hipMemcpyDeviceToHost, s));
    } else {
        HIPCHK(hipGetLastError());
        hwin.resize(ns * W * WW); hinf.resize(ns * W);
        HIPCHK(hipMemcpyAsync(hwin.data(), sl.l1.p, ns * W * WW * 8, hipMemcpyDeviceToHost, s));
        HIPCHK(hipMemcpyAsync(hinf.data(), sl.l1_inf.p, ns * W, hipMemcpyDeviceToHost, s));
    }
    HIPCHK(hipMemcpyAsync(hbad, d_bad, 4, hipMemcpyDeviceToHost, s));
    HIPCHK(hipStreamSynchronize(s));
    if (gs.prof) prof_flush(sl);
    if (*hbad) return DGPU_E_BADARG;
    if (!device_fold) {
        const size_t TH = std::min<size_t>(std::min<size_t>(ns, 16), std::max<size_t>(1, std::thread::hardware_concurrency()));
        auto tail = [&](size_t g) {
            host_fold<HF>(hwin.data() + g * W * WW, hinf.data() + g * W, (int)W, SMALL_MSM_C, out + (s0 + g) * JW);
            if (out_inf) out_inf[s0 + g] = jac_is_identity(out + (s0 + g) * JW, JW);
        };
        if (TH <= 1) { for (size_t g = 0; g < ns; g++) tail(g); }
        else if ((rc = par_run(TH, [&](size_t k) -> int32_t { for (size_t g = k; g < ns; g += TH) tail(g); return DGPU_OK; }))) return rc;
    }
    return DGPU_OK;
}
template <class C, class HF>
int32_t msm_segments(const uint64_t *bases, const uint8_t *is_inf, const uint64_t *scalars, size_t N, const uint64_t *seg_end, size_t nseg, int mont, uint64_t *out, uint8_t *out_inf) {
    if (nseg == 0) return DGPU_OK;
    constexpr size_t JW = 3 * sizeof(HF) / 8;
    if (!bases || !scalars || !out || !seg_end || N >= (1ull << 31)) return DGPU_E_BADARG;
    { uint64_t prev = 0; for (size_t g = 0; g < nseg; g++) { if (seg_end[g] < prev) return DGPU_E_BADARG; prev = seg_end[g]; } if (prev != N) return DGPU_E_BADARG; }
    if (!cur().ready) return DGPU_E_NODEVICE;
    if (!tl_no_min && N < gs.min_gpu_n) return DGPU_E_TOO_SMALL;
    const RawBases rb = RawBases::packed<C>(bases, is_inf);
    const size_t reach = std::min<size_t>(SMALL_MSM_MAX_N, gs.small_max.load());
    const int forced_terms = gs.seg_chunk.load(), forced_fold = gs.seg_fold.load();
    const size_t chunk_terms = forced_terms > 0 ? (size_t)forced_terms : SEG_CHUNK_TERMS;
    auto len = [&](size_t g) { return (size_t)(seg_end[g] - (g ? seg_end[g - 1] : 0)); };
    struct Chunk { size_t s0, s1; };
    std::vector<Chunk> chunks; std::vector<size_t> slow;
    for (size_t g = 0; g < nseg;) {
        if (len(g) > reach) { slow.push_back(g++); continue; }
        size_t e = g, terms = 0;
        while (e < nseg && len(e) <= reach && e - g < SEG_CHUNK_SEGS && (e == g || terms + len(e) <= chunk_terms)) terms += len(e++);
        chunks.push_back(Chunk{g, e});
        g = e;
    }
    if (!chunks.empty()) {
        SLOT_ACQUIRE(L, sl);
        HIPCHK(hipSetDevice(cur().device));
        SegLayout lay;
        size_t mt = 0, ms = 0, mb = 0, mp = 0;
        for (const Chunk &c : chunks) {
            const size_t T = seg_end[c.s1 - 1] - (c.s0 ? seg_end[c.s0 - 1] : 0);
            if (T == 0) continue;
            seg_layout(seg_end, c.s0, c.s1, lay);
            mt = std::max(mt, T); ms = std::max(ms, c.s1 - c.s0); mb = std::max(mb, lay.blocks); mp = std::max(mp, lay.pslots);
        }
        int32_t rc;
        const uint64_t allocs0 = g_dev_allocs.load();
        if (mt && (rc = ws_seg<C>(sl, rb, mt, ms, mb, mp))) return rc;
        if (g_dev_allocs.load() != allocs0) {
            Ctx &cx = cur();
            for (int k = 0; k < N_SLOTS; k++) {
                Slot &o = cx.slots[k];
                if (&o == &sl || !o.mu.try_lock()) continue;
                (void)ws_seg<C>(o, rb, mt, ms, mb, mp);
                o.mu.unlock();
            }
        }
        std::vector<uint64_t> hwin; std::vector<uint8_t> hinf;
        for (const Chunk &c : chunks) {
            const size_t T = seg_end[c.s1 - 1] - (c.s0 ? seg_end[c.s0 - 1] : 0), ns = c.s1 - c.s0;
            if (T == 0) {
                for (size_t g = c.s0; g < c.s1; g++) { write_identity<HF>(out + g * JW); if (out_inf) out_inf[g] = 1; }
                continue;
            }
            seg_layout(seg_end, c.s0, c.s1, lay);
            const bool device_fold = forced_fold == 2 || (forced_fold != 1 && ns >= SEG_DEVICE_FOLD_MIN);
            rc = msm_seg_chunk<C, HF>(sl, rb, scalars, seg_end, c.s0, c.s1, mont != 0, lay, device_fold, hwin, hinf, out, out_inf);
            if (rc) { (void)hipStreamSynchronize(sl.cstream); (void)hipStreamSynchronize(sl.stream); return rc; }
        }
    }
    for (size_t g : slow) {
        const size_t lo = g ? seg_end[g - 1] : 0;
        RawBases part = rb; part.p = rb.p + lo * rb.stride; if (rb.is_inf) part.is_inf = rb.is_inf + lo;
        const int32_t rc = msm_oneshot_ctx<C, HF>(part, scalars + lo * 4, len(g), mont != 0, out + g * JW);
        if (rc) return rc;
        if (out_inf) out_inf[g] = jac_is_identity(out + g * JW, JW);
    }
    return DGPU_OK;
}

template <class C> inline size_t cache_entry_bytes(size_t n, int c) {
    if (c == 0) c = choose_c_pre(n);
    if (c == 0) return n * (size_t)C::AFF_STRIDE * 4 + (n <= SMALL_MSM_MAX_N ? small_sub_bytes<C>(n) : 0);
    return pre_tab_bytes<C>(n, 255 / c + 1);
}
template <class C>
bool cache_acquire(const RawBases &rb, size_t n, int kind, int table_c, std::shared_ptr<CacheEntry> &e, size_t &off, bool verify_now = true, bool *was_resident = nullptr) {
    const CacheKey key{rb.p, n, rb.stride, rb.x_off, rb.y_off, rb.inf_off, rb.is_inf, kind, cur_index()};
    constexpr int words = C::ABI_W / 2;
    std::vector<std::shared_ptr<CacheEntry>> dropped;
    e.reset(); off = 0;
    bool fill = false;
    {
        std::lock_guard<std::mutex> lk(gcache.mu);
        for (auto &c : gcache.entries) if (c->state == CacheEntry::READY && key.inside(c->k, &off)) { e = c; e->last_use = ++gcache.tick; break; }
    }
    if (was_resident) *was_resident = (bool)e;
    if (e && verify_now && !cache_verify(*e, key, off, words)) {
        std::lock_guard<std::mutex> lk(gcache.mu);
        cache_remove_locked(e.get(), dropped);
        gcache.stale++; e.reset();
    }
    if (e) return true;
    off = 0;
    const uint64_t fp = range_fingerprint(key, words);
    size_t budget_auto = 0;
    if (gcache.budget.load() == CACHE_BUDGET_AUTO) {
        size_t fr = 0, tot = 0;
        if (hipSetDevice(cur().device) == hipSuccess && hipMemGetInfo(&fr, &tot) == hipSuccess) budget_auto = fr / 4; else (void)hipGetLastError();
    }
    {
        std::lock_guard<std::mutex> lk(gcache.mu);
        if (gcache.budget.load() == CACHE_BUDGET_AUTO) gcache.budget = budget_auto;
        std::shared_ptr<CacheEntry> seen;
        for (auto &c : gcache.entries) if (c->state != CacheEntry::READY && c->k.same(key)) { seen = c; break; }
        if (!seen) {
            size_t n_seen = 0, oldest = gcache.entries.size();
            for (size_t i = 0; i < gcache.entries.size(); i++) if (gcache.entries[i]->state == CacheEntry::SEEN) { n_seen++; if (oldest == gcache.entries.size() || gcache.entries[i]->last_use < gcache.entries[oldest]->last_use) oldest = i; }
            if (n_seen >= CACHE_MAX_SEEN) { dropped.push_back(std::move(gcache.entries[oldest])); gcache.entries.erase(gcache.entries.begin() + oldest); }
            auto c = std::make_shared<CacheEntry>(); c->k = key; c->fp = fp; c->last_use = ++gcache.tick;
            gcache.entries.push_back(std::move(c));
        } else if (seen->state == CacheEntry::SEEN) {
            seen->last_use = ++gcache.tick;
            if (seen->fp != fp) seen->fp = fp;
            else if (cache_make_room_locked(cache_entry_bytes<C>(n, table_c), seen.get(), dropped)) { seen->state = CacheEntry::FILLING; e = seen; fill = true; }
        }
    }
    if (!fill) { gcache.misses++; return false; }
    e->rec_hash.resize(n);
    uint64_t h = 0;
    int32_t frc = bases_upload<C>(rb, n, &h, kind, &e->rec_hash);
    if (!frc) {
        frc = bases_precompute<C>(h, table_c, kind);
        if (frc) { (void)dgpu_bases_free(h); h = 0; }
    }
    std::lock_guard<std::mutex> lk(gcache.mu);
    if (frc) { cache_remove_locked(e.get(), dropped); e.reset(); gcache.misses++; return false; }
    e->handle = h; e->bytes = cache_entry_bytes<C>(n, table_c); gcache.fills++;
    bool listed = false;
    for (auto &c : gcache.entries) if (c.get() == e.get()) listed = true;
    if (listed) {
        e->state = CacheEntry::READY; e->last_use = ++gcache.tick; gcache.used += e->bytes;
        for (size_t i = 0; i < gcache.entries.size();) {
            size_t o; CacheEntry &c = *gcache.entries[i];
            if (&c != e.get() && c.state == CacheEntry::READY && c.k.inside(e->k, &o)) { gcache.used -= c.bytes; dropped.push_back(std::move(gcache.entries[i])); gcache.entries.erase(gcache.entries.begin() + i); }
            else i++;
        }
    }
    return true;
}
template <class C, class HF>
bool msm_oneshot_cached(const RawBases &rb, const uint64_t *scalars, size_t n, bool mont, uint64_t *out, int kind, int32_t &rc) {
    std::shared_ptr<CacheEntry> e; size_t off = 0;
    const bool full = gcache.verify_samples.load(std::memory_order_relaxed) < 0;
    bool was_resident = false;
    if (!cache_acquire<C>(rb, n, kind, 0, e, off, !full, &was_resident)) return false;
    if (full && was_resident) {
        const CacheKey key{rb.p, n, rb.stride, rb.x_off, rb.y_off, rb.inf_off, rb.is_inf, kind, cur_index()};
        bool same = true; int32_t mrc = DGPU_OK;
        const int32_t prc = par_run(2, [&](size_t part) -> int32_t {
            if (part == 0) mrc = msm_handle<C, HF>(e->handle, off, scalars, n, mont, out, kind, false);
            else same = cache_verify(*e, key, off, C::ABI_W / 2);
            return DGPU_OK;
        });
        if (prc) same = false;
        if (!same) {
            std::vector<std::shared_ptr<CacheEntry>> dropped;
            std::lock_guard<std::mutex> lk(gcache.mu);
            cache_remove_locked(e.get(), dropped);
            gcache.stale++; return false;
        }
        rc = mrc;
    } else
    rc = msm_handle<C, HF>(e->handle, off, scalars, n, mont, out, kind, false);
    if (rc != DGPU_OK && rc != DGPU_E_BADARG) {
        std::vector<std::shared_ptr<CacheEntry>> dropped;
        std::lock_guard<std::mutex> lk(gcache.mu);
        cache_remove_locked(e.get(), dropped);
        gcache.misses++; return false;
    }
    gcache.hits++;
    return true;
}
struct ViewPin { std::shared_ptr<CacheEntry> e; uint64_t temp = 0; bool check = false; CacheKey key{}; int words = 0; };
template <class C>
int32_t view_acquire(const RawBases &rb, size_t n, int kind, int table_c, uint64_t *handle, void **pin) {
    if (!handle || !pin || (n && !rb.p) || n >= (1ull << 31) || !rb.ok<C>()) return DGPU_E_BADARG;
    if (!cur().ready) return DGPU_E_NODEVICE;
    ViewPin *vp = new ViewPin();
    size_t off = 0;
    const bool full = gcache.verify_samples.load(std::memory_order_relaxed) < 0;
    bool was_resident = false;
    if (n && gcache.enabled.load() && n >= gcache.min_n.load() && cache_acquire<C>(rb, n, kind, table_c, vp->e, off, !full, &was_resident)) {
        if (off == 0 && vp->e->k.n == n) {
            gcache.hits++; *handle = vp->e->handle; *pin = vp;
            if (full && was_resident) { vp->check = true; vp->key = CacheKey{rb.p, n, rb.stride, rb.x_off, rb.y_off, rb.inf_off, rb.is_inf, kind, cur_index()}; vp->words = C::ABI_W / 2; }
            return DGPU_OK;
        }
        vp->e.reset();
    }
    const int32_t rc = bases_upload<C>(rb, n, &vp->temp, kind);
    if (rc) { delete vp; return rc; }
    *handle = vp->temp; *pin = vp;
    return DGPU_OK;
}
inline bool view_verify(void *pin) {
    ViewPin *vp = (ViewPin *)pin;
    if (!vp || !vp->check || !vp->e) return true;
    if (cache_verify(*vp->e, vp->key, 0, vp->words)) return true;
    std::vector<std::shared_ptr<CacheEntry>> dropped;
    std::lock_guard<std::mutex> lk(gcache.mu);
    cache_remove_locked(vp->e.get(), dropped);
    gcache.stale++;
    return false;
}
inline void view_release(void *pin) {
    ViewPin *vp = (ViewPin *)pin;
    if (!vp) return;
    if (vp->temp) (void)dgpu_bases_free(vp->temp);
    delete vp;
}

template <class C, class HF>
int32_t msm_resident(uint64_t bases, size_t boff, uint64_t scalars, size_t soff, size_t n, uint64_t *out, int kind, bool check_min = true) {
    if (!out) return DGPU_E_BADARG;
    if (!cur().ready) return DGPU_E_NODEVICE;
    if (check_min && !tl_no_min && n < std::min<size_t>(gs.min_gpu_n, DGPU_MIN_GPU_N_HANDLE)) return DGPU_E_TOO_SMALL;
    HandleRef hb(bases), hs(scalars);
    if (!hb.ok || !hs.ok || (hb.h.kind != kind && hb.h.kind != kind + 9) || hs.h.kind != 3 || hb.h.ctx != hs.h.ctx) return DGPU_E_BADARG;
    if (boff > hb.h.n || n > hb.h.n - boff || soff > hs.h.n || n > hs.h.n - soff) return DGPU_E_BADARG;
    CtxScope on_owner(hb.h.ctx);
    SLOT_ACQUIRE(L, sl);
    HIPCHK(hipSetDevice(cur().device));
    if (hb.h.kind == kind + 9) return msm_device_pre<C, HF>(sl, *(const PreTable *)hb.h.p, boff, (const uint32_t *)hs.h.p + soff * 8, n, out);
    SmallSub sub; const bool have = n && small_sub_for<C>(sl, bases, hb.h, boff, n, sub);
    return msm_device<C, HF>(sl, (const uint32_t *)hb.h.p + boff * C::AFF_STRIDE, (const uint32_t *)hs.h.p + soff * 8, n, out, have ? &sub : nullptr);
}

template <class C, class HF>
int32_t msm_sharded_oneshot(const uint64_t *bases, const uint8_t *is_inf, const uint64_t *scalars, size_t n, int32_t ngpus, bool mont, uint64_t *out) {
    if (!out || (n && (!bases || !scalars)) || n >= (1ull << 31) || ngpus < 0) return DGPU_E_BADARG;
    const std::vector<int> cx = ready_contexts(ngpus);
    if (cx.empty()) return DGPU_E_NODEVICE;
    if (ngpus > 0 && (int)cx.size() < ngpus) return DGPU_E_BADARG;
    if (!tl_no_min && n < gs.min_gpu_n) return DGPU_E_TOO_SMALL;
    std::vector<size_t> lo; shard_bounds(n, cx.size(), lo);
    const size_t JW = 3 * sizeof(HF) / 8, BW = 2 * sizeof(HF) / 8;
    std::vector<uint64_t> parts(cx.size() * JW);
    int32_t rc = run_shards(cx.size(), [&](size_t k) {
        CtxScope here(cx[k]);
        const size_t cnt = lo[k + 1] - lo[k];
        return msm_oneshot_here<C, HF>(RawBases::packed<C>(bases + lo[k] * BW, is_inf ? is_inf + lo[k] : nullptr), scalars + lo[k] * 4, cnt, mont, parts.data() + k * JW);
    });
    if (rc) return rc;
    return host_fold_jacobian<HF>(parts.data(), cx.size(), out);
}
template <class C>
int32_t bases_upload_sharded(const uint64_t *bases, const uint8_t *is_inf, size_t n, int32_t ngpus, uint64_t *handle, int kind ) {
    if (!handle || (n && !bases) || n >= (1ull << 31) || ngpus < 0) return DGPU_E_BADARG;
    const std::vector<int> cx = ready_contexts(ngpus);
    if (cx.empty()) return DGPU_E_NODEVICE;
    if (ngpus > 0 && (int)cx.size() < ngpus) return DGPU_E_BADARG;
    ShardSet *ss = new ShardSet();
    ss->n = n; ss->sub.assign(cx.size(), 0); shard_bounds(n, cx.size(), ss->lo);
    const size_t BW = 2 * C::ABI_W / 2;
    int32_t rc = run_shards(cx.size(), [&](size_t k) {
        CtxScope here(cx[k]);
        return bases_upload<C>(RawBases::packed<C>(bases + ss->lo[k] * BW, is_inf ? is_inf + ss->lo[k] : nullptr), ss->lo[k + 1] - ss->lo[k], &ss->sub[k], kind);
    });
    if (rc) { for (uint64_t h : ss->sub) if (h) (void)dgpu_bases_free(h); delete ss; return rc; }
    *handle = register_handle(ss, n, kind + 6);
    return DGPU_OK;
}
template <class C, class HF>
int32_t msm_sharded_handle(uint64_t bases, const uint64_t *scalars, size_t n, int mont, uint64_t *out, int kind) {
    if (!out || (n && !scalars)) return DGPU_E_BADARG;
    HandleRef hb(bases);
    if (!hb.ok || hb.h.kind != kind + 6 || n > hb.h.n) return DGPU_E_BADARG;
    if (!tl_no_min && n < gs.min_gpu_n) return DGPU_E_TOO_SMALL;
    const ShardSet &ss = *(const ShardSet *)hb.h.p;
    const size_t G = ss.sub.size(), JW = 3 * sizeof(HF) / 8;
    std::vector<uint64_t> parts(G * JW);
    int32_t rc = run_shards(G, [&](size_t k) {
        const size_t lo = std::min(ss.lo[k], n), hi = std::min(ss.lo[k + 1], n);
        return msm_handle<C, HF>(ss.sub[k], 0, scalars + lo * 4, hi - lo, mont, parts.data() + k * JW, kind, false);
    });
    if (rc) return rc;
    return host_fold_jacobian<HF>(parts.data(), G, out);
}
template <class C, class HF>
int32_t msm_sharded_resident(uint64_t bases, uint64_t scalars, uint64_t *out, int kind) {
    if (!out) return DGPU_E_BADARG;
    HandleRef hb(bases), hs(scalars);
    if (!hb.ok || !hs.ok || hb.h.kind != kind + 6 || hs.h.kind != 9) return DGPU_E_BADARG;
    const ShardSet &sb = *(const ShardSet *)hb.h.p, &sv = *(const ShardSet *)hs.h.p;
    if (sb.sub.size() != sv.sub.size() || sv.n > sb.n) return DGPU_E_BADARG;
    for (size_t k = 0; k < sb.sub.size(); k++) if (sv.lo[k] != std::min(sb.lo[k], sv.n) || sv.lo[k + 1] != std::min(sb.lo[k + 1], sv.n)) return DGPU_E_BADARG;
    if (sv.n < gs.min_gpu_n) return DGPU_E_TOO_SMALL;
    const size_t G = sb.sub.size(), JW = 3 * sizeof(HF) / 8;
    std::vector<uint64_t> parts(G * JW);
    int32_t rc = run_shards(G, [&](size_t k) { return msm_resident<C, HF>(sb.sub[k], 0, sv.sub[k], 0, sv.lo[k + 1] - sv.lo[k], parts.data() + k * JW, kind, false); });
    if (rc) return rc;
    return host_fold_jacobian<HF>(parts.data(), G, out);
}


}
```

### crypto_amd/csrc/msm_launch.hip.h

```cpp
#pragma once
#include <hip/hip_runtime.h>
#include "msm_kernels.hip.h"
#include "many_fold.hip.h"
#include "seg_layout.hip.h"

namespace msm {

template <class C> void launch_prep_bases(hipStream_t s, const uint32_t *abi, const uint8_t *is_inf, size_t n, uint32_t *out);
template <class C> void launch_prep_bases_fp(hipStream_t s, const uint32_t *abi, const uint8_t *is_inf, size_t n, uint32_t *out);
template <class C> void launch_prep_bases_raw(hipStream_t s, const uint8_t *raw, size_t stride, size_t x_off, size_t y_off, size_t inf_off, const uint8_t *is_inf, size_t n, uint32_t *out);
template <class C> void launch_accumulate(hipStream_t s, const uint32_t *bases, const uint32_t *entries, const uint32_t *off, uint32_t NB, uint32_t *bucket, uint8_t *bucket_inf,
                                          uint32_t *head, uint32_t *tail, uint32_t *head_b, uint32_t *tail_b, uint8_t *part_inf, size_t T, uint32_t CH, uint32_t dbg_mask, const uint32_t *dyn = nullptr);
template <class C> void launch_accumulate_skip_identity(hipStream_t s, const uint32_t *bases, const uint32_t *entries, const uint32_t *off, uint32_t NB, uint32_t *bucket, uint8_t *bucket_inf,
                                          uint32_t *head, uint32_t *tail, uint32_t *head_b, uint32_t *tail_b, uint8_t *part_inf, size_t T, uint32_t CH, const uint32_t *dyn, const RowMap &map);
template <class C> void launch_fixup(hipStream_t s, uint32_t NB, uint32_t *bucket, uint8_t *bucket_inf, const uint32_t *head, const uint32_t *tail, const uint32_t *head_b,
                                     const uint32_t *tail_b, const uint8_t *part_inf, size_t T, const uint32_t *off, uint32_t heavy_thr, const uint32_t *dyn = nullptr);
template <class C> void launch_fixup_heavy(hipStream_t s, const uint32_t *heavy, uint32_t heavy_cap, const uint32_t *off, uint32_t CH, uint32_t NB, uint32_t *bucket, uint8_t *bucket_inf,
                                           const uint32_t *head, const uint32_t *tail, const uint8_t *part_inf, size_t T, uint32_t *dyn, uint32_t *hpart, uint8_t *hpart_inf);
template <class C> void launch_merge_buckets(hipStream_t s, uint32_t NB, uint32_t *dst, uint8_t *dst_inf, const uint32_t *src, const uint8_t *src_inf);
template <class C> void launch_reduce_l0(hipStream_t s, unsigned NG, const uint32_t *bucket, const uint8_t *bucket_inf, uint32_t NB, int mshift, uint32_t *l1, uint8_t *l1_inf);
template <class C> int launch_reduce_marginals(hipStream_t s, unsigned NG, const uint32_t *bucket, const uint8_t *bucket_inf, uint32_t NB, int mshift, uint32_t *cls, uint8_t *cls_inf, uint32_t *win_abi, uint8_t *win_inf, bool quad);
template <class C> size_t reduce_marginals_points(size_t NG);
template <class C> void launch_reduce_top(hipStream_t s, unsigned W, const uint32_t *l1, const uint8_t *l1_inf, int G, int gshift, uint32_t *win_abi, uint8_t *win_inf, int lanes);

constexpr int SMALL_MSM_C = 4, SMALL_MSM_W = 64, SMALL_MSM_E = 8, SMALL_MSM_LEAVES = 128, SMALL_MSM_S = 4;
constexpr size_t SMALL_MSM_MAX_N = 8192;
inline int small_per_group(size_t L, int subtables) { const int g = (int)((L + 256 * (size_t)subtables - 1) / (256 * (size_t)subtables)); return g < 2 ? 2 : g; }
template <class C> void launch_small_table(hipStream_t s, const uint32_t *bases, size_t n, uint32_t *tab, uint8_t *tab_inf);
template <class C> void launch_small_subtable(hipStream_t s, const uint32_t *bases, size_t n, uint32_t *tab, uint8_t *tab_inf);
template <class C> void launch_small_tree(hipStream_t s, const uint32_t *tab, const uint8_t *tab_inf, int subtables, const uint32_t *scalars, size_t n, uint32_t *partial, uint8_t *partial_inf,
                                          uint32_t *count, uint32_t *win_abi, uint8_t *win_inf, uint8_t *win_bad);

template <class C> void launch_many_tree(hipStream_t s, const uint32_t *tab, const uint8_t *tab_inf, const uint32_t *scalars, size_t n, size_t row_stride, size_t rows, uint32_t *partial,
                                         uint8_t *partial_inf, uint32_t *count, uint32_t *win, uint8_t *win_inf, uint32_t *bad_flag);
template <class C> void launch_many_fold(hipStream_t s, const uint32_t *win, const uint8_t *win_inf, size_t rows, uint32_t *out_xyz, uint8_t *out_inf);

template <class C> void launch_seg_tree(hipStream_t s, const uint32_t *tab, const uint8_t *tab_inf, const uint32_t *scalars, const void *desc, size_t blocks, uint32_t *partial,
                                        uint8_t *partial_inf, uint32_t *count, uint32_t *win, uint8_t *win_inf, bool abi, uint32_t *bad_flag);
template <class C> void launch_seg_fold(hipStream_t s, const uint32_t *win, const uint8_t *win_inf, size_t nseg, uint32_t *out_xyz, uint8_t *out_inf);

template <class C> void launch_pre_step(hipStream_t s, const uint32_t *prev, size_t n, int c, uint32_t *tmp, uint32_t *out);
template <class C> void launch_reduce_top_s(hipStream_t s, unsigned W, const uint32_t *l1, const uint8_t *l1_inf, int G, int gshift, uint32_t *win_abi, uint8_t *win_inf, uint32_t *win_s_abi, uint8_t *win_s_inf, int lanes);

}
```

### crypto_amd/csrc/msm_launch_impl.hip.h

```cpp
#pragma once
#include "msm_launch.hip.h"
#include "reduce_kernels.hip.h"

namespace msm {
template <class C> void launch_prep_bases(hipStream_t s, const uint32_t *abi, const uint8_t *is_inf, size_t n, uint32_t *out) {
    hipLaunchKernelGGL((k_prep_bases<typename C::MSM>), dim3((unsigned)((n + 255) / 256)), dim3(256), 0, s, abi, is_inf, n, out);
}
template <class C> void launch_prep_bases_raw(hipStream_t s, const uint8_t *raw, size_t stride, size_t x_off, size_t y_off, size_t inf_off, const uint8_t *is_inf, size_t n, uint32_t *out) {
    hipLaunchKernelGGL((k_prep_bases_raw<typename C::MSM>), dim3((unsigned)((n + 255) / 256)), dim3(256), 0, s, raw, stride, x_off, y_off, inf_off, is_inf, n, out);
}
template <class C> void launch_prep_bases_fp(hipStream_t s, const uint32_t *abi, const uint8_t *is_inf, size_t n, uint32_t *out) {
    hipLaunchKernelGGL((k_prep_bases<C>), dim3((unsigned)((n + 255) / 256)), dim3(256), 0, s, abi, is_inf, n, out);
}
template <class C> void launch_accumulate(hipStream_t s, const uint32_t *bases, const uint32_t *entries, const uint32_t *off, uint32_t NB, uint32_t *bucket, uint8_t *bucket_inf,
                                          uint32_t *head, uint32_t *tail, uint32_t *head_b, uint32_t *tail_b, uint8_t *part_inf, size_t T, uint32_t CH, uint32_t dbg_mask, const uint32_t *dyn) {
    typedef typename C::ACC A;
    hipLaunchKernelGGL((k_accumulate<A>), dim3((unsigned)((T * A::LPP + 255) / 256)), dim3(256), 0, s, bases, entries, off, NB, bucket, bucket_inf, head, tail, head_b, tail_b, part_inf, T, CH, dbg_mask, dyn, RowMap{});
}
template <class C> void launch_accumulate_skip_identity(hipStream_t s, const uint32_t *bases, const uint32_t *entries, const uint32_t *off, uint32_t NB, uint32_t *bucket, uint8_t *bucket_inf,
                                          uint32_t *head, uint32_t *tail, uint32_t *head_b, uint32_t *tail_b, uint8_t *part_inf, size_t T, uint32_t CH, const uint32_t *dyn, const RowMap &map) {
    typedef typename C::ACC A;
    hipLaunchKernelGGL((k_accumulate<A, true>), dim3((unsigned)((T * A::LPP + 255) / 256)), dim3(256), 0, s, bases, entries, off, NB, bucket, bucket_inf, head, tail, head_b, tail_b, part_inf, T, CH, 0xffffffffu, dyn, map);
}
template <class C> void launch_fixup(hipStream_t s, uint32_t NB, uint32_t *bucket, uint8_t *bucket_inf, const uint32_t *head, const uint32_t *tail, const uint32_t *head_b,
                                     const uint32_t *tail_b, const uint8_t *part_inf, size_t T, const uint32_t *off, uint32_t heavy_thr, const uint32_t *dyn) {
    if constexpr (C::NFP == 2) hipLaunchKernelGGL((k_fixup_pair<G2P>), dim3((unsigned)((2 * T + 255) / 256)), dim3(256), 0, s, NB, bucket, bucket_inf, head, tail, head_b, tail_b, part_inf, T, off, heavy_thr, dyn);
    else hipLaunchKernelGGL((k_fixup<typename C::MSM>), dim3((unsigned)((T + 255) / 256)), dim3(256), 0, s, NB, bucket, bucket_inf, head, tail, head_b, tail_b, part_inf, T, off, heavy_thr, dyn);
}
template <class C> void launch_fixup_heavy(hipStream_t s, const uint32_t *heavy, uint32_t heavy_cap, const uint32_t *off, uint32_t CH, uint32_t NB, uint32_t *bucket, uint8_t *bucket_inf,
                                           const uint32_t *head, const uint32_t *tail, const uint8_t *part_inf, size_t T, uint32_t *dyn, uint32_t *hpart, uint8_t *hpart_inf) {
    typedef typename C::ACC A;
    hipLaunchKernelGGL((k_fixup_heavy<A>), dim3(512), dim3(A::HEAVY_T), 0, s, heavy, heavy_cap, off, CH, NB, bucket, bucket_inf, head, tail, part_inf, T, dyn);
    hipLaunchKernelGGL((k_fixup_heavy_ranges<A>), dim3(64, 32), dim3(A::HEAVY_T), 0, s, off, head, tail, part_inf, (const uint32_t *)dyn, hpart, hpart_inf);
    hipLaunchKernelGGL((k_fixup_heavy_join<A>), dim3(32), dim3(A::HEAVY_T), 0, s, off, NB, bucket, bucket_inf, (const uint32_t *)dyn, (const uint32_t *)hpart, (const uint8_t *)hpart_inf);
}
template <class C> void launch_merge_buckets(hipStream_t s, uint32_t NB, uint32_t *dst, uint8_t *dst_inf, const uint32_t *src, const uint8_t *src_inf) {
    typedef typename C::ACC A;
    hipLaunchKernelGGL((k_merge_buckets<A>), dim3((unsigned)(((size_t)NB * A::LPP + 255) / 256)), dim3(256), 0, s, NB, dst, dst_inf, src, src_inf);
}
template <class C> void launch_reduce_l0(hipStream_t s, unsigned NG, const uint32_t *bucket, const uint8_t *bucket_inf, uint32_t NB, int mshift, uint32_t *l1, uint8_t *l1_inf) {
    const unsigned blocks = (NG + 3) / 4;
    if constexpr (C::NFP == 2) hipLaunchKernelGGL((k_reduce_l0_pair<G2P>), dim3(blocks), dim3(256), 0, s, bucket, bucket_inf, NB, mshift, l1, l1_inf, NG);
    else hipLaunchKernelGGL((k_reduce_l0<typename C::MSM>), dim3(blocks), dim3(256), 0, s, bucket, bucket_inf, NB, mshift, l1, l1_inf, NG);
}
template <class C> inline void red_levels(bool quad, int &PL, int &KK) { typedef RedGeom<typename C::ACC> RG; PL = quad ? 64 : RG::PL; KK = quad ? 6 : RG::K; }
template <class C> size_t reduce_marginals_points(size_t NG) {
    typedef RedGeom<typename C::ACC> RG;
    size_t best = 0;
    for (int quad = 0; quad < 2; quad++) {
        int PL, KK; red_levels<C>(quad != 0, PL, KK);
        size_t total = (size_t)(RG::K + 2) * NG, cnt = NG; int nm = RG::K;
        while (cnt > 1) { const int steps = std::min(KK, red_log2((unsigned)cnt)); const size_t chunks = std::max<size_t>(1, cnt / PL); nm += steps; total += (size_t)(nm + 2) * chunks; cnt = chunks; }
        best = std::max(best, total + 64);
    }
    return best;
}
template <class C> int launch_reduce_marginals(hipStream_t s, unsigned NG, const uint32_t *bucket, const uint8_t *bucket_inf, uint32_t NB, int mshift, uint32_t *cls, uint8_t *cls_inf, uint32_t *win_abi, uint8_t *win_inf, bool quad) {
    typedef typename C::ACC A; typedef RedGeom<A> RG;
    hipLaunchKernelGGL((k_reduce_m0<A>), dim3((NG + 3) / 4), dim3(256), 0, s, bucket, bucket_inf, NB, mshift, cls, cls_inf, NG);
    int PL, KK; red_levels<C>(quad, PL, KK);
    unsigned cnt = NG; int nm = RG::K;
    uint32_t *in = cls; uint8_t *in_inf = cls_inf;
    while (cnt > 1) {
        const int steps = std::min(KK, red_log2(cnt));
        const unsigned chunks = std::max(1u, cnt / (unsigned)PL), npairs = 1u + (unsigned)(nm + 1) / 2u, waves = npairs * chunks;
        uint32_t *out = in + (size_t)(nm + 2) * cnt * A::XW; uint8_t *out_inf = in_inf + (size_t)(nm + 2) * cnt;
        if (quad) hipLaunchKernelGGL((k_reduce_cls_quad<A>), dim3(waves), dim3(256 * A::LPP), 0, s, (const uint32_t *)in, (const uint8_t *)in_inf, cnt, nm, out, out_inf, chunks == 1 ? 1 : 0, win_abi, win_inf);
        else hipLaunchKernelGGL((k_reduce_cls<A>), dim3((waves + 3) / 4), dim3(256), 0, s, (const uint32_t *)in, (const uint8_t *)in_inf, cnt, nm, out, out_inf, chunks == 1 ? 1 : 0, win_abi, win_inf);
        nm += steps; cnt = chunks; in = out; in_inf = out_inf;
    }
    return nm;
}
template <class C> void launch_reduce_top(hipStream_t s, unsigned W, const uint32_t *l1, const uint8_t *l1_inf, int G, int gshift, uint32_t *win_abi, uint8_t *win_inf, int lanes) {
    if (lanes == 4) {
        typedef typename C::ACC A;
        hipLaunchKernelGGL((k_reduce_top_quad<A>), dim3(W), dim3(256 * A::LPP), 0, s, l1, l1_inf, G, gshift, win_abi, win_inf, (uint32_t *)nullptr, (uint8_t *)nullptr);
        return;
    }
    if constexpr (C::NFP == 2) hipLaunchKernelGGL((k_reduce_top_pair<G2P>), dim3(W), dim3(64), 0, s, l1, l1_inf, G, gshift, win_abi, win_inf, (uint32_t *)nullptr, (uint8_t *)nullptr);
    else hipLaunchKernelGGL((k_reduce_top<typename C::MSM>), dim3(W), dim3(64), 0, s, l1, l1_inf, G, gshift, win_abi, win_inf, (uint32_t *)nullptr, (uint8_t *)nullptr);
}
template <class C> void launch_reduce_top_s(hipStream_t s, unsigned W, const uint32_t *l1, const uint8_t *l1_inf, int G, int gshift, uint32_t *win_abi, uint8_t *win_inf, uint32_t *win_s_abi, uint8_t *win_s_inf, int lanes) {
    if (lanes == 4) {
        typedef typename C::ACC A;
        hipLaunchKernelGGL((k_reduce_top_quad<A>), dim3(W), dim3(256 * A::LPP), 0, s, l1, l1_inf, G, gshift, win_abi, win_inf, win_s_abi, win_s_inf);
        return;
    }
    if constexpr (C::NFP == 2) hipLaunchKernelGGL((k_reduce_top_pair<G2P>), dim3(W), dim3(64), 0, s, l1, l1_inf, G, gshift, win_abi, win_inf, win_s_abi, win_s_inf);
    else hipLaunchKernelGGL((k_reduce_top<typename C::MSM>), dim3(W), dim3(64), 0, s, l1, l1_inf, G, gshift, win_abi, win_inf, win_s_abi, win_s_inf);
}
}
```

### crypto_amd/csrc/pre_kernels.hip.h

```cpp
#pragma once
#include <hip/hip_runtime.h>
#include "msm_kernels.hip.h"
#include "fp_inv.hip.h"

namespace msm {
using namespace bls29;

constexpr int PRE_GROUP = 8;

__device__ __forceinline__ void inv_key(Fp &k, const Fp &a) { fp_norm(k, a); }
__device__ __forceinline__ void inv_key(Fp &k, const Fp2 &a) { Fp n0, n1, t; fp_sqr(n0, a.c0); fp_sqr(n1, a.c1); fp_add(t, n0, n1); fp_norm(k, t); }
__device__ __forceinline__ void inv_from_key(Fp &r, const Fp &, const Fp &kinv) { r = kinv; }
__device__ __forceinline__ void inv_key(Fp &k, const Fs &a) { fp_from_fs(k, a); }
__device__ __forceinline__ void inv_from_key(Fs &r, const Fs &, const Fp &kinv) { fs_from_fp(r, kinv); }
__device__ __forceinline__ void inv_key(Fp &k, const Fs2 &a) { Fs n0, n1, t; fs_sqr(n0, a.c0); fs_sqr(n1, a.c1); fs_add(t, n0, n1); fs_bal(t, t); fp_from_fs(k, t); }
__device__ __forceinline__ void inv_from_key(Fs2 &r, const Fs2 &a, const Fp &kinv) {
    Fs ki, n1; fs_from_fp(ki, kinv); fs_mul(r.c0, a.c0, ki); fs_mul(n1, a.c1, ki); fs_neg(r.c1, n1);
}
__device__ __forceinline__ void inv_from_key(Fp2 &r, const Fp2 &a, const Fp &kinv) {
    Fp n1, z; fp_mul(r.c0, a.c0, kinv); fp_mul(n1, a.c1, kinv); fp_zero(z); fp_sub<4>(r.c1, z, n1); fp_norm(r.c1, r.c1);
}

template <class C>
__global__ void __launch_bounds__(64) k_pre_dbl(const uint32_t *__restrict__ prev, size_t n, int c, uint32_t *__restrict__ tmp) {
    typedef typename C::F F;
    const size_t i = (size_t)blockIdx.x * blockDim.x + threadIdx.x;
    if (i >= n) return;
    const uint32_t *rec = prev + i * C::AFF_STRIDE;
    if (rec[C::FLAGW] != 0) return;
    Aff<F> p; load_aff<C>(p, rec);
    Xyzz<F> acc; xyzz_dbl_affine(acc, p);
    for (int k = 1; k < c; k++) { Xyzz<F> d; xyzz_dbl(d, acc); acc = d; }
    uint32_t *dst = tmp + i * C::XW;
    const uint32_t *w = reinterpret_cast<const uint32_t *>(&acc);
#pragma unroll
    for (int k = 0; k < C::XW; k += 4) *reinterpret_cast<uint4 *>(dst + k) = make_uint4(w[k], w[k + 1], w[k + 2], w[k + 3]);
}

template <class C> __device__ __forceinline__ void load_xyzz_aos(Xyzz<typename C::F> &p, const uint32_t *__restrict__ src) {
    uint32_t *w = reinterpret_cast<uint32_t *>(&p);
#pragma unroll
    for (int k = 0; k < C::XW; k += 4) { uint4 v = *reinterpret_cast<const uint4 *>(src + k); w[k] = v.x; w[k + 1] = v.y; w[k + 2] = v.z; w[k + 3] = v.w; }
}

template <class C>
__global__ void __launch_bounds__(64) k_pre_norm(const uint32_t *__restrict__ prev, const uint32_t *__restrict__ tmp, size_t n, uint32_t *__restrict__ out) {
    typedef typename C::F F;
    const size_t t = (size_t)blockIdx.x * blockDim.x + threadIdx.x;
    const size_t i0 = t * PRE_GROUP;
    if (i0 >= n) return;
    Fp pre[PRE_GROUP], run; fp_set_one(run);
    bool live[PRE_GROUP];
#pragma unroll
    for (int k = 0; k < PRE_GROUP; k++) {
        const size_t i = i0 + k;
        live[k] = i < n && prev[i * C::AFF_STRIDE + C::FLAGW] == 0;
        pre[k] = run;
        if (live[k]) {
            F zzz; const uint32_t *src = tmp + i * C::XW + 3 * C::FW; uint32_t *w = reinterpret_cast<uint32_t *>(&zzz);
            for (int j = 0; j < C::FW; j++) w[j] = src[j];
            Fp key; inv_key(key, zzz);
            Fp nr; fp_mul(nr, run, key); run = nr;
        }
    }
    Fp inv; fp_inv_device(inv, run);
#pragma unroll
    for (int k = PRE_GROUP - 1; k >= 0; k--) {
        const size_t i = i0 + k;
        if (i >= n) continue;
        uint32_t *dst = out + i * C::AFF_STRIDE;
        if (!live[k]) { for (int j = 0; j < C::AFF_STRIDE; j++) dst[j] = prev[i * C::AFF_STRIDE + j]; continue; }
        Xyzz<F> p; load_xyzz_aos<C>(p, tmp + i * C::XW);
        Fp key, kinv, ni; inv_key(key, p.zzz);
        fp_mul(kinv, inv, pre[k]);
        fp_mul(ni, inv, key); inv = ni;
        F i3, tt, i2, xn, yn; Aff<F> a;
        inv_from_key(i3, p.zzz, kinv);
        fmul(tt, p.zz, i3); fsqr(i2, tt);
        fnorm(xn, p.x); fnorm(yn, p.y);
        fmul(a.x, xn, i2); fmul(a.y, yn, i3);
        store_aff_record<C>(dst, a);
    }
}

}
```

### crypto_amd/csrc/psort_kernels.hip.h

```cpp
#pragma once
#include "dyn_chunk.hip.h"
#include <hip/hip_runtime.h>
#include <stdint.h>
#include "sort_launch.hip.h"

namespace msm {


__device__ __forceinline__ uint32_t lds_inc_agg(uint32_t *cnt, uint32_t bin, bool active) {
    const uint64_t mask = __ballot(active);
    if (mask == 0) return 0;
    const int lane = threadIdx.x & 63, first = __ffsll((long long)mask) - 1;
    const uint32_t fb = (uint32_t)__shfl((int)bin, first, 64);
    const bool same = active && bin == fb;
    const uint64_t smask = __ballot(same);
    uint32_t base = 0;
    if (lane == first) base = atomicAdd(&cnt[fb], (uint32_t)__popcll(smask));
    base = (uint32_t)__shfl((int)base, first, 64);
    if (same) return base + (uint32_t)__popcll(smask & ((1ull << lane) - 1ull));
    return active ? atomicAdd(&cnt[bin], 1u) : 0u;
}

template <int CC, int CW, class F> __device__ __forceinline__ void ps_digits(const PsParams &q, size_t i, bool live, F f) {
    uint4 a = make_uint4(0, 0, 0, 0), b = a;
    if (live) { const uint4 *p = reinterpret_cast<const uint4 *>(q.scalars + i * 8); a = p[0]; b = p[1]; }
    uint32_t s[8] = {a.x, a.y, a.z, a.w, b.x, b.y, b.z, b.w & 0x7fffffffu};
    uint32_t carry = 0;
    if constexpr (CC != 0) {
        constexpr uint32_t B = 1u << (CC - 1);
#pragma unroll
        for (int w = 0; w < CW; w++) {
            const int bitpos = w * CC;
            uint32_t raw = 0;
            if (bitpos < 256) {
                const int wd = bitpos >> 5, sh = bitpos & 31;
                const uint32_t lo = s[wd], hi = wd + 1 < 8 ? s[wd + 1] : 0u;
                raw = (sh ? ((lo >> sh) | (hi << (32 - sh))) : lo) & ((1u << CC) - 1u);
            }
            const uint32_t v = raw + carry;
            const uint32_t neg = v > B ? 1u : 0u;
            const uint32_t mag = neg ? (2u * B - v) : v;
            carry = neg;
            f(w, mag - 1, neg, live && mag != 0);
        }
    } else {
        const uint32_t B = 1u << (q.c - 1);
        for (int w = 0; w < q.W; w++) {
            const int bitpos = w * q.c;
            uint32_t raw = 0;
            if (bitpos < 256) {
                const int wd = bitpos >> 5, sh = bitpos & 31;
                uint64_t v = 0;
#pragma unroll
                for (int k = 0; k < 8; k++) { if (k == wd) v |= s[k]; if (k == wd + 1) v |= (uint64_t)s[k] << 32; }
                raw = (uint32_t)(v >> sh) & ((1u << q.c) - 1u);
            }
            const uint32_t v = raw + carry;
            const uint32_t neg = v > B ? 1u : 0u;
            const uint32_t mag = neg ? (2u * B - v) : v;
            carry = neg;
            f(w, mag - 1, neg, live && mag != 0);
        }
    }
}
__device__ __forceinline__ bool ps_live(const PsParams &q, size_t i) {
    return i < q.n && (!q.idflag || q.idflag[(size_t)q.flag_base + i] == 0);
}

__global__ void __launch_bounds__(256) k_id_flags(const uint32_t *__restrict__ bases, int aff_stride, int flag_word, size_t n, uint8_t *__restrict__ out) {
    const size_t i = (size_t)blockIdx.x * blockDim.x + threadIdx.x;
    if (i < n) out[i] = bases[i * (size_t)aff_stride + flag_word] != 0 ? 1 : 0;
}

__global__ void __launch_bounds__(256) k_raw_record_hash(const uint8_t *__restrict__ raw, size_t stride, size_t x_off, size_t y_off, size_t inf_off, const uint8_t *__restrict__ is_inf,
                                                         int words, size_t n, uint64_t *__restrict__ out) {
    const size_t i = (size_t)blockIdx.x * blockDim.x + threadIdx.x;
    if (i >= n) return;
    const uint8_t *pt = raw + i * stride;
    uint64_t h = 0x9E3779B97F4A7C15ull;
    for (int part = 0; part < 2; part++) {
        const uint8_t *src = pt + (part ? y_off : x_off);
        for (int k = 0; k < words; k++) {
            const uint2 v = *reinterpret_cast<const uint2 *>(src + 8 * k);
            h = (h ^ ((uint64_t)v.x | ((uint64_t)v.y << 32))) * 0xff51afd7ed558ccdull;
            h ^= h >> 32;
        }
    }
    uint64_t flag = 0;
    if (is_inf && is_inf[i]) flag = 1;
    if (inf_off != ~(size_t)0 && pt[inf_off]) flag = 1;
    h = (h ^ flag) * 0xc4ceb9fe1a85ec53ull;
    out[i] = h ^ (h >> 29);
}

__device__ __forceinline__ uint32_t ps_tile_of_block(uint32_t b, uint32_t ntiles) {
    const uint32_t per = ntiles >> 3;
    return b < (per << 3) ? (b & 7u) * per + (b >> 3) : b;
}

template <int CC, int CW>
__global__ void __launch_bounds__(PS_TILE) k_ps_count1(PsParams q, uint32_t *__restrict__ cnt1) {
    extern __shared__ __align__(16) uint32_t lds[];
    for (uint32_t j = threadIdx.x; j < q.P; j += blockDim.x) lds[j] = 0;
    __syncthreads();
    const uint32_t tile = ps_tile_of_block(blockIdx.x, q.ntiles);
    const size_t i = (size_t)tile * PS_TILE + threadIdx.x;
    if (i < q.n && (q.scalars[i * 8 + 7] >> 31)) atomicOr(q.bad, 1u);
    ps_digits<CC, CW>(q, i, ps_live(q, i), [&](int w, uint32_t m1, uint32_t, bool nz) { (void)lds_inc_agg(lds, nz ? ((uint32_t)w * q.key_wstride + m1) >> q.part_log : 0u, nz); });
    __syncthreads();
    for (uint32_t j = threadIdx.x; j < q.P; j += blockDim.x) cnt1[(size_t)j * q.ntiles + tile] = lds[j];
}

template <int CC, int CW>
__global__ void __launch_bounds__(PS_TILE) k_ps_scatter1(PsParams q, const uint32_t *__restrict__ cnt1, const uint32_t *__restrict__ off1, uint2 *__restrict__ pairs) {
    extern __shared__ __align__(16) uint32_t lds[];
    uint32_t *cnt = lds, *pre = lds + q.P, *cur = lds + 2 * q.P, *goff = lds + 3 * q.P;
    uint2 *stage = reinterpret_cast<uint2 *>(lds + 4 * q.P);
    __shared__ uint32_t wave_tot[PS_TILE / 64 + 1];
    const uint32_t tile = ps_tile_of_block(blockIdx.x, q.ntiles);
    for (uint32_t j = threadIdx.x; j < q.P; j += blockDim.x) { const size_t idx = (size_t)j * q.ntiles + tile; const uint32_t o0 = off1[idx], o1 = off1[idx + 1]; goff[j] = o0; cnt[j] = o1 - o0; }
    const size_t i = (size_t)tile * PS_TILE + threadIdx.x;
    const bool live = ps_live(q, i);
    __syncthreads();
    {
        const uint32_t per = (q.P + PS_TILE - 1) / PS_TILE;
        const uint32_t b0 = threadIdx.x * per;
        uint32_t sum = 0;
        for (uint32_t k = 0; k < per; k++) if (b0 + k < q.P) sum += cnt[b0 + k];
        uint32_t incl = sum;
        for (int d = 1; d < 64; d <<= 1) { uint32_t t = __shfl_up(incl, d, 64); if ((int)(threadIdx.x & 63) >= d) incl += t; }
        if ((threadIdx.x & 63) == 63) wave_tot[threadIdx.x >> 6] = incl;
        __syncthreads();
        uint32_t base = 0;
        for (uint32_t wv = 0; wv < (threadIdx.x >> 6); wv++) base += wave_tot[wv];
        uint32_t run = base + incl - sum;
        for (uint32_t k = 0; k < per; k++) if (b0 + k < q.P) { pre[b0 + k] = run; cur[b0 + k] = run; run += cnt[b0 + k]; }
    }
    __syncthreads();
    ps_digits<CC, CW>(q, i, live, [&](int w, uint32_t m1, uint32_t neg, bool nz) {
        const uint32_t key = nz ? (uint32_t)w * q.key_wstride + m1 : 0u;
        const uint32_t pos = lds_inc_agg(cur, key >> q.part_log, nz);
        if (nz) stage[pos] = make_uint2(key, (q.val_base + (uint32_t)w * q.val_wstride + (uint32_t)i) | (neg << 31));
    });
    __syncthreads();
    uint32_t total = 0;
    for (uint32_t wv = 0; wv < PS_TILE / 64; wv++) total += wave_tot[wv];
    for (uint32_t k = threadIdx.x; k < total; k += blockDim.x) {
        const uint2 pr = stage[k];
        const uint32_t p = pr.x >> q.part_log;
        pairs[(size_t)goff[p] + (k - pre[p])] = pr;
    }
}

template <bool WC>
__global__ void __launch_bounds__(1024, WC ? 4 : 8) k_ps_bucket(const uint2 *__restrict__ pairs, const uint32_t *__restrict__ off1, uint32_t ntiles, uint32_t P, uint32_t NB, int part_log,
                                                    uint32_t *__restrict__ off, uint32_t *__restrict__ entries,
                                                    uint32_t heavy_thr, uint32_t *__restrict__ heavy, uint32_t heavy_cap, const uint32_t *__restrict__ dyn) {
    if (dyn) heavy_thr = dyn[DYN_HEAVY];
    __shared__ uint32_t cnt[PS_PART];
    __shared__ uint32_t wave_tot[17];
    const uint32_t p = blockIdx.x, PB = 1u << part_log, mask = PB - 1;
    const uint32_t lo = off1[(size_t)p * ntiles], hi = off1[(size_t)(p + 1) * ntiles];
    for (uint32_t j = threadIdx.x; j < PS_PART; j += blockDim.x) cnt[j] = 0;
    __syncthreads();
    constexpr int U = WC ? 4 : 8;
    for (uint32_t base = lo; base < hi; base += U * 1024) {
        uint32_t key[U];
#pragma unroll
        for (int j = 0; j < U; j++) { const uint32_t k = base + j * 1024 + threadIdx.x; key[j] = k < hi ? pairs[k].x : 0xffffffffu; }
#pragma unroll
        for (int j = 0; j < U; j++) (void)lds_inc_agg(cnt, key[j] & mask, key[j] != 0xffffffffu);
    }
    __syncthreads();
    const uint32_t c0 = cnt[2 * threadIdx.x], c1 = cnt[2 * threadIdx.x + 1];
    const uint32_t sum = c0 + c1;
    uint32_t incl = sum;
    for (int d = 1; d < 64; d <<= 1) { uint32_t t = __shfl_up(incl, d, 64); if ((int)(threadIdx.x & 63) >= d) incl += t; }
    if ((threadIdx.x & 63) == 63) wave_tot[threadIdx.x >> 6] = incl;
    __syncthreads();
    uint32_t basep = lo;
    for (uint32_t wv = 0; wv < (threadIdx.x >> 6); wv++) basep += wave_tot[wv];
    const uint32_t e0 = basep + incl - sum, e1 = e0 + c0;
    __syncthreads();
    cnt[2 * threadIdx.x] = e0; cnt[2 * threadIdx.x + 1] = e1;
    const uint32_t j0 = 2 * threadIdx.x, k0 = p * PB + j0;
    if (j0 < PB && k0 < NB) { off[k0] = e0; if (c0 >= heavy_thr) { uint32_t h = atomicAdd(&heavy[0], 1u); if (h < heavy_cap) heavy[1 + h] = k0; } }
    if (j0 + 1 < PB && k0 + 1 < NB) { off[k0 + 1] = e1; if (c1 >= heavy_thr) { uint32_t h = atomicAdd(&heavy[0], 1u); if (h < heavy_cap) heavy[1 + h] = k0 + 1; } }
    if (p == P - 1 && threadIdx.x == 0) off[NB] = hi;
    __syncthreads();
    if constexpr (!WC) {
        extern __shared__ __align__(16) uint32_t dv_lds[];
        for (uint32_t base = lo; base < hi; base += U * 1024) {
            uint2 pr[U];
#pragma unroll
            for (int j = 0; j < U; j++) { const uint32_t k = base + j * 1024 + threadIdx.x; pr[j] = k < hi ? pairs[k] : make_uint2(0xffffffffu, 0u); }
#pragma unroll
            for (int j = 0; j < U; j++) {
                const bool on = pr[j].x != 0xffffffffu; const uint32_t pos = lds_inc_agg(cnt, pr[j].x & mask, on);
                if (on) { const uint32_t r = pos - lo; if (r < (uint32_t)PS_DIRECT_CAP) dv_lds[r] = pr[j].y; else entries[pos] = pr[j].y; }
            }
        }
        __syncthreads();
        const uint32_t staged = hi - lo < (uint32_t)PS_DIRECT_CAP ? hi - lo : (uint32_t)PS_DIRECT_CAP;
        for (uint32_t k = threadIdx.x; k < staged; k += 1024) entries[lo + k] = dv_lds[k];
        return;
    } else {
    extern __shared__ __align__(16) uint32_t wc_lds[];
    uint32_t *lcnt = wc_lds, *lpre = wc_lds + PS_PART;
    uint2 *stage = reinterpret_cast<uint2 *>(wc_lds + 2 * PS_PART);
    constexpr int V = PS_WC_TILE / 1024;
    for (uint32_t base = lo; base < hi; base += PS_WC_TILE) {
        lcnt[2 * threadIdx.x] = 0; lcnt[2 * threadIdx.x + 1] = 0;
        __syncthreads();
        uint2 pr[V]; uint32_t rank[V];
#pragma unroll
        for (int j = 0; j < V; j++) { const uint32_t k = base + j * 1024 + threadIdx.x; pr[j] = k < hi ? pairs[k] : make_uint2(0xffffffffu, 0u); }
#pragma unroll
        for (int j = 0; j < V; j++) rank[j] = lds_inc_agg(lcnt, pr[j].x & mask, pr[j].x != 0xffffffffu);
        __syncthreads();
        const uint32_t l0 = lcnt[2 * threadIdx.x], l1 = lcnt[2 * threadIdx.x + 1];
        const uint32_t ls = l0 + l1;
        uint32_t li = ls;
        for (int d = 1; d < 64; d <<= 1) { uint32_t t = __shfl_up(li, d, 64); if ((int)(threadIdx.x & 63) >= d) li += t; }
        if ((threadIdx.x & 63) == 63) wave_tot[threadIdx.x >> 6] = li;
        __syncthreads();
        uint32_t lb = 0;
        for (uint32_t wv = 0; wv < (threadIdx.x >> 6); wv++) lb += wave_tot[wv];
        lpre[2 * threadIdx.x] = lb + li - ls; lpre[2 * threadIdx.x + 1] = lb + li - ls + l0;
        __syncthreads();
#pragma unroll
        for (int j = 0; j < V; j++)
            if (pr[j].x != 0xffffffffu) { const uint32_t bk = pr[j].x & mask; stage[lpre[bk] + rank[j]] = make_uint2(pr[j].y, cnt[bk] + rank[j]); }
        __syncthreads();
        cnt[2 * threadIdx.x] += l0; cnt[2 * threadIdx.x + 1] += l1;
        const uint32_t tile_n = hi - base < (uint32_t)PS_WC_TILE ? hi - base : (uint32_t)PS_WC_TILE;
        for (uint32_t q = threadIdx.x; q < tile_n; q += 1024) { const uint2 e = stage[q]; entries[e.y] = e.x; }
        __syncthreads();
    }
    }
}

}
```

### crypto_amd/csrc/reduce_kernels.hip.h

```cpp
#pragma once
#include "msm_kernels.hip.h"

namespace msm {

template <class C> struct RedGeom {
    static constexpr int LPP = C::LPP;
    static constexpr int PL = 64 / LPP;
    static constexpr int K = LPP == 1 ? 6 : 5;
    static constexpr int PW = (int)(sizeof(Xyzz<typename C::F>) / 4);
};
__host__ __device__ inline int red_log2(unsigned v) { int r = 0; while ((1u << (r + 1)) <= v) r++; return r; }
inline size_t reduce_m_points(size_t NG, int PL, int K) {
    size_t total = (size_t)(K + 2) * NG; size_t cnt = NG; int nm = K;
    while (cnt > 1) { const int steps = std::min(K, red_log2((unsigned)cnt)); const size_t chunks = std::max<size_t>(1, cnt / PL); nm += steps; total += (size_t)(nm + 2) * chunks; cnt = chunks; }
    return total + 64;
}

template <class C> __device__ __forceinline__ void shfl_xor_point(Xyzz<typename C::F> &o, bool &oinf, const Xyzz<typename C::F> &x, bool xinf, int d) {
    constexpr int PW_ = RedGeom<C>::PW;
    const uint32_t *w = reinterpret_cast<const uint32_t *>(&x);
    uint32_t *q = reinterpret_cast<uint32_t *>(&o);
#pragma unroll
    for (int k = 0; k < PW_; k++) q[k] = (uint32_t)__shfl_xor((int)w[k], d * C::LPP, 64);
    oinf = __shfl_xor((int)xinf, d * C::LPP, 64) != 0;
}
template <class C> __device__ __forceinline__ void tree_step(Xyzz<typename C::F> &S, bool &sinf, Xyzz<typename C::F> &A, bool &ainf, int pl, int d, bool weighted) {
    typedef typename C::F F;
    constexpr int PW_ = RedGeom<C>::PW;
    const bool hi = (pl & d) != 0;
    uint32_t *ws = reinterpret_cast<uint32_t *>(&S), *wa = reinterpret_cast<uint32_t *>(&A);
#pragma unroll
    for (int k = 0; k < PW_; k++) { const uint32_t s = ws[k], a = wa[k]; ws[k] = hi ? a : s; wa[k] = hi ? s : a; }
    { const bool s = sinf, a = ainf; sinf = hi ? a : s; ainf = hi ? s : a; }
    Xyzz<F> o; bool oinf;
    shfl_xor_point<C>(o, oinf, A, ainf, d);
    const int low = pl & (d - 1);
    const bool active = hi ? (low == d - 1) : (low == 0 || (weighted && (low & (low - 1)) == 0));
    xyzz_add(S, sinf, o, oinf || !active);
#pragma unroll
    for (int k = 0; k < PW_; k++) { const uint32_t s = ws[k], a = wa[k]; ws[k] = hi ? a : s; wa[k] = hi ? s : a; }
    { const bool s = sinf, a = ainf; sinf = hi ? a : s; ainf = hi ? s : a; }
}

template <class C>
__global__ void __launch_bounds__(256, 1) k_reduce_m0(const uint32_t *__restrict__ bucket, const uint8_t *__restrict__ bucket_inf, uint32_t NB, int mshift,
                                                      uint32_t *__restrict__ cls, uint8_t *__restrict__ cls_inf, unsigned NG) {
    typedef typename C::F F;
    constexpr int LPP = RedGeom<C>::LPP, PL = RedGeom<C>::PL, K = RedGeom<C>::K;
    const int lane = threadIdx.x & 63, pl = lane / LPP;
    const uint32_t m = (uint32_t)LPP << mshift;
    const size_t g = (size_t)blockIdx.x * (blockDim.x >> 6) + (threadIdx.x >> 6);
    if (g >= NG) return;
    const size_t b0 = (g * PL + pl) * (size_t)m;
    { bool any = false; for (uint32_t k = 0; k < m; k++) any = any || bucket_inf[b0 + k] == 0;
      if (!__any(any)) { if (lane < K + 2) cls_inf[(size_t)lane * NG + g] = 1; return; } }
    Xyzz<F> run, tot; bool rinf, tinf;
    {
        const size_t b = b0 + m - 1;
        rinf = bucket_inf[b] != 0;
        fzero(run.x); fzero(run.y); fzero(run.zz); fzero(run.zzz);
        if (!rinf) load_soa<C>(run, bucket, NB, b);
        tot = run; tinf = rinf;
    }
    const int nserial = 2 * ((int)m - 1);
    constexpr int PW_ = RedGeom<C>::PW;
    uint32_t *wr = reinterpret_cast<uint32_t *>(&run), *wt = reinterpret_cast<uint32_t *>(&tot);
#pragma unroll 1
    for (int it = 0; it < nserial + K; it++) {
        const bool serial = it < nserial;
        const int d = serial ? 0 : 1 << (it - nserial);
        const bool hi = serial ? (it & 1) != 0 : (pl & d) != 0;
#pragma unroll
        for (int k = 0; k < PW_; k++) { const uint32_t r = wr[k], t = wt[k]; wr[k] = hi ? t : r; wt[k] = hi ? r : t; }
        { const bool r = rinf, t = tinf; rinf = hi ? t : r; tinf = hi ? r : t; }
        Xyzz<F> o; bool oinf;
        if (serial) {
            if ((it & 1) == 0) { const size_t b = b0 + (m - 2 - (uint32_t)(it >> 1)); oinf = bucket_inf[b] != 0; if (!oinf) load_soa<C>(o, bucket, NB, b); else o = run; }
            else { o = tot; oinf = tinf; }
        } else {
            shfl_xor_point<C>(o, oinf, tot, tinf, d);
            const int low = pl & (d - 1);
            const bool active = hi ? (low == d - 1) : (low == 0 || (low & (low - 1)) == 0);
            oinf = oinf || !active;
        }
        xyzz_add(run, rinf, o, oinf);
#pragma unroll
        for (int k = 0; k < PW_; k++) { const uint32_t r = wr[k], t = wt[k]; wr[k] = hi ? t : r; wt[k] = hi ? r : t; }
        { const bool r = rinf, t = tinf; rinf = hi ? t : r; tinf = hi ? r : t; }
    }
    const bool first = (lane % LPP) == 0;
    if (pl == 0) { store_soa<C>(cls, NG, g, run); if (first) cls_inf[g] = rinf; }
    else if ((pl & (pl - 1)) == 0) { const size_t c = 2 + red_log2((unsigned)pl); store_soa<C>(cls + c * NG * C::XW, NG, g, run); if (first) cls_inf[c * NG + g] = rinf; }
    if (pl == PL - 1) { store_soa<C>(cls + (size_t)NG * C::XW, NG, g, tot); if (first) cls_inf[NG + g] = tinf; }
}

template <class C>
__global__ void __launch_bounds__(256, 1) k_reduce_cls(const uint32_t *__restrict__ in, const uint8_t *__restrict__ in_inf, unsigned cnt, int nm,
                                                       uint32_t *__restrict__ out, uint8_t *__restrict__ out_inf, int final_,
                                                       uint32_t *__restrict__ win_abi, uint8_t *__restrict__ win_inf) {
    typedef typename C::F F;
    constexpr int LPP = RedGeom<C>::LPP, PL = RedGeom<C>::PL, K = RedGeom<C>::K;
    const int lane = threadIdx.x & 63, pl = lane / LPP, h = lane % LPP;
    const unsigned chunks = cnt / PL ? cnt / PL : 1u;
    const int steps = red_log2(cnt) < K ? red_log2(cnt) : K;
    const unsigned npairs = 1u + (unsigned)(nm + 1) / 2u;
    const unsigned w = blockIdx.x * (blockDim.x >> 6) + (threadIdx.x >> 6);
    const unsigned pair = w / chunks, j = w % chunks;
    if (pair >= npairs) return;
    const unsigned c0 = pair == 0 ? 0u : 2u * pair, c1 = c0 + 1;
    const bool has1 = c1 < 2u + (unsigned)nm;
    const unsigned idx = j * PL + pl;
    Xyzz<F> S, A; bool sinf = true, ainf = true;
    fzero(S.x); fzero(S.y); fzero(S.zz); fzero(S.zzz); A = S;
    if (idx < cnt) {
        sinf = in_inf[(size_t)c0 * cnt + idx] != 0;
        if (!sinf) load_soa<C>(S, in + (size_t)c0 * cnt * C::XW, cnt, idx);
        if (has1) { ainf = in_inf[(size_t)c1 * cnt + idx] != 0; if (!ainf) load_soa<C>(A, in + (size_t)c1 * cnt * C::XW, cnt, idx); }
    }
#pragma unroll 1
    for (int s = 0; s < steps; s++) tree_step<C>(S, sinf, A, ainf, pl, 1 << s, pair == 0);
    const bool outS = pl == 0, outA = has1 && pl == (1 << steps) - 1;
    const bool outM = pair == 0 && pl < (1 << steps) && pl != 0 && (pl & (pl - 1)) == 0;
    const unsigned cm = 2u + (unsigned)nm + (unsigned)red_log2((unsigned)pl);
    if (!final_) {
        if (outS) { store_soa<C>(out + (size_t)c0 * chunks * C::XW, chunks, j, S); if (h == 0) out_inf[(size_t)c0 * chunks + j] = sinf; }
        if (outA) { store_soa<C>(out + (size_t)c1 * chunks * C::XW, chunks, j, A); if (h == 0) out_inf[(size_t)c1 * chunks + j] = ainf; }
        if (outM) { store_soa<C>(out + (size_t)cm * chunks * C::XW, chunks, j, S); if (h == 0) out_inf[(size_t)cm * chunks + j] = sinf; }
        return;
    }
    constexpr int WS = 4 * 12 * LPP;
    auto emit = [&](unsigned c, const Xyzz<F> &pt, bool inf) __attribute__((always_inline)) {
        if (c == 0) return;
        const unsigned slot = c - 1;
        if (h == 0) win_inf[slot] = inf;
        if (inf) return;
        const Fs *f = reinterpret_cast<const Fs *>(&pt);
#pragma unroll 1
        for (int k = 0; k < 4; k++) {
            Fs v;
#pragma unroll
            for (int i = 0; i < SN; i++) v.l[i] = pick4(k, f[0].l[i], f[1].l[i], f[2].l[i], f[3].l[i]);
            fs_to_abi(win_abi + (size_t)slot * WS + 12 * (LPP * k + h), v);
        }
    };
    if (outS || outM) emit(outS ? c0 : cm, S, sinf);
    if (outA) emit(c1, A, ainf);
}

template <class C>
__global__ void __launch_bounds__(256 * C::LPP) k_reduce_cls_quad(const uint32_t *__restrict__ in, const uint8_t *__restrict__ in_inf, unsigned cnt, int nm,
                                                                  uint32_t *__restrict__ out, uint8_t *__restrict__ out_inf, int final_,
                                                                  uint32_t *__restrict__ win_abi, uint8_t *__restrict__ win_inf) {
    typedef typename C::F F;
    constexpr int LPP = C::LPP, GL = 4 * LPP, PW_ = 4 * SN, PLQ = 64;
    __shared__ uint32_t xs[64 * LPP * PW_];
    __shared__ uint8_t fl[64];
    const int t = (int)threadIdx.x, gi = t / GL, h = t % LPP;
    const QuadLanes<LPP> q4;
    const unsigned chunks = cnt / PLQ ? cnt / PLQ : 1u;
    const int steps = red_log2(cnt) < 6 ? red_log2(cnt) : 6;
    const unsigned pair = blockIdx.x / chunks, j = blockIdx.x % chunks;
    const unsigned c0 = pair == 0 ? 0u : 2u * pair, c1 = c0 + 1;
    const bool has1 = c1 < 2u + (unsigned)nm;
    const unsigned idx = j * PLQ + (unsigned)gi;
    Xyzz<F> S, A; bool sinf = true, ainf = true;
    fzero(S.x); fzero(S.y); fzero(S.zz); fzero(S.zzz); A = S;
    if (idx < cnt) {
        sinf = in_inf[(size_t)c0 * cnt + idx] != 0;
        if (!sinf) load_soa<C>(S, in + (size_t)c0 * cnt * C::XW, cnt, idx);
        if (has1) { ainf = in_inf[(size_t)c1 * cnt + idx] != 0; if (!ainf) load_soa<C>(A, in + (size_t)c1 * cnt * C::XW, cnt, idx); }
    }
    uint32_t *ws = reinterpret_cast<uint32_t *>(&S), *wa = reinterpret_cast<uint32_t *>(&A);
#pragma unroll 1
    for (int s = 0; s < steps; s++) {
        const int d = 1 << s;
        const bool hi = (gi & d) != 0;
#pragma unroll
        for (int k = 0; k < PW_; k++) { const uint32_t a = ws[k], b = wa[k]; ws[k] = hi ? b : a; wa[k] = hi ? a : b; }
        { const bool a = sinf, b = ainf; sinf = hi ? b : a; ainf = hi ? a : b; }
        __syncthreads();
        { uint32_t *dst = xs + ((gi * 4 + q4.role) * LPP + h) * SN;
#pragma unroll
          for (int k = 0; k < SN; k++) dst[k] = pick4(q4.role, wa[k], wa[SN + k], wa[2 * SN + k], wa[3 * SN + k]);
          if (t % GL == 0) fl[gi] = ainf; }
        __syncthreads();
        Xyzz<F> o; bool oinf;
        { const int sg = gi ^ d;
          uint32_t *ov = reinterpret_cast<uint32_t *>(&o);
#pragma unroll
          for (int c = 0; c < 4; c++) {
              const uint32_t *sv = xs + ((sg * 4 + c) * LPP + h) * SN;
#pragma unroll
              for (int k = 0; k < SN; k++) ov[c * SN + k] = sv[k];
          }
          oinf = fl[sg] != 0; }
        const int low = gi & (d - 1);
        const bool active = hi ? (low == d - 1) : (low == 0 || (pair == 0 && (low & (low - 1)) == 0));
        xyzz_add_rounds(S, sinf, o, oinf || !active, q4);
#pragma unroll
        for (int k = 0; k < PW_; k++) { const uint32_t a = ws[k], b = wa[k]; ws[k] = hi ? b : a; wa[k] = hi ? a : b; }
        { const bool a = sinf, b = ainf; sinf = hi ? b : a; ainf = hi ? a : b; }
    }
    const bool outS = gi == 0, outA = has1 && gi == (1 << steps) - 1;
    const bool outM = pair == 0 && gi < (1 << steps) && gi != 0 && (gi & (gi - 1)) == 0;
    const unsigned cm = 2u + (unsigned)nm + (unsigned)red_log2((unsigned)gi);
    const bool first = t % GL == 0;
    if (!final_) {
        if (q4.role == 0) {
            if (outS) { store_soa<C>(out + (size_t)c0 * chunks * C::XW, chunks, j, S); if (first) out_inf[(size_t)c0 * chunks + j] = sinf; }
            if (outA) { store_soa<C>(out + (size_t)c1 * chunks * C::XW, chunks, j, A); if (first) out_inf[(size_t)c1 * chunks + j] = ainf; }
            if (outM) { store_soa<C>(out + (size_t)cm * chunks * C::XW, chunks, j, S); if (first) out_inf[(size_t)cm * chunks + j] = sinf; }
        }
        return;
    }
    constexpr int WS = 4 * 12 * LPP;
    auto emit = [&](unsigned c, const Xyzz<F> &pt, bool inf) __attribute__((always_inline)) {
        if (c == 0) return;
        const unsigned slot = c - 1;
        if (first) win_inf[slot] = inf;
        if (inf) return;
        const Fs *f = reinterpret_cast<const Fs *>(&pt);
        Fs v;
#pragma unroll
        for (int i = 0; i < SN; i++) v.l[i] = pick4(q4.role, f[0].l[i], f[1].l[i], f[2].l[i], f[3].l[i]);
        fs_to_abi(win_abi + (size_t)slot * WS + 12 * (LPP * q4.role + h), v);
    };
    if (outS || outM) emit(outS ? c0 : cm, S, sinf);
    if (outA) emit(c1, A, ainf);
}

}
```

### crypto_amd/csrc/sort_launch.hip.h

```cpp
#pragma once
#include <hip/hip_runtime.h>
#include <stddef.h>
#include <stdint.h>

namespace msm {
void launch_digit_codes(hipStream_t s, bool wide, const uint32_t *scalars, const uint32_t *bases, int aff_stride, int flag_word, size_t n, size_t n_pad, int c, int W, void *dig, uint32_t *bad );
void launch_sort_sweep(hipStream_t s, bool wide, bool scatter, unsigned grid, size_t lds_bytes, const void *dig, size_t n, size_t n_pad, int W, int RANGES, int rb_log, uint32_t B,
                       uint32_t *cnt, const uint32_t *off, uint32_t *entries, uint32_t heavy_thr, uint32_t *heavy, uint32_t heavy_cap);
void launch_scan(hipStream_t s, const uint32_t *cnt, uint32_t *off, uint32_t *cursor, uint32_t *bsums, size_t NB);
void launch_dyn_chunk(hipStream_t s, const uint32_t *total, uint32_t fixed_ch, uint32_t min_chunk, uint32_t max_chunks, uint32_t lanes_per_chunk, uint32_t T_max, uint32_t *dyn,
                      uint32_t nb_shared = 0 );
void launch_flag_heavy(hipStream_t s, const uint32_t *off, uint32_t NB, const uint32_t *dyn, uint32_t *heavy, uint32_t heavy_cap);
size_t scan_blocks(size_t NB);
constexpr int PS_TILE = 512;
constexpr int PS_PART_LOG_MAX = 11;
constexpr int PS_PART = 1 << PS_PART_LOG_MAX;
constexpr int PS_WC_TILE = 16384;
#ifdef PS_NO_WC
constexpr uint32_t PS_WC_MIN_PAIRS = 0xffffffffu;
#else
constexpr uint32_t PS_WC_MIN_PAIRS = 65536;
#endif
constexpr int PS_DIRECT_CAP = 16384;
constexpr int PS_MAX_W = 16;
struct PsParams {
    const uint32_t *scalars;
    const uint8_t *idflag;
    size_t n;
    uint32_t flag_base;
    int c, W;
    uint32_t key_wstride;
    uint32_t val_base, val_wstride;
    int part_log;
    uint32_t P;
    uint32_t ntiles;
    uint32_t *bad;
};

inline int ps_part_log(uint32_t NB) { int lg = 0; while ((1u << lg) < NB) lg++; int pl = lg - 10; return pl < 5 ? 5 : (pl > PS_PART_LOG_MAX ? PS_PART_LOG_MAX : pl); }
void launch_psort(hipStream_t s, const PsParams &q, uint32_t NB, uint32_t *cnt1, uint32_t *off1, uint32_t *bsums, void *pairs, uint32_t *off, uint32_t *entries,
                  uint32_t heavy_thr, uint32_t *heavy, uint32_t heavy_cap, const uint32_t *dyn_args = nullptr, uint32_t *dyn = nullptr);
void launch_id_flags(hipStream_t s, const uint32_t *bases, int aff_stride, int flag_word, size_t n, uint8_t *out);
void launch_raw_record_hash(hipStream_t s, const uint8_t *raw, size_t stride, size_t x_off, size_t y_off, size_t inf_off, const uint8_t *is_inf, int words, size_t n, uint64_t *out);
void launch_g1_scale(hipStream_t s, const uint32_t *p_abi, const uint8_t *is_inf, const uint32_t *scalars, int scalar_stride, const uint8_t *negate, size_t n, uint32_t *out_abi, uint8_t *out_inf,
                     const uint32_t *add_abi = nullptr, const uint8_t *add_inf = nullptr);
void launch_selftest_fp_mul(hipStream_t s, const uint32_t *a, const uint32_t *b, size_t n, uint32_t *out);
void launch_selftest_g1_sum(hipStream_t s, const uint32_t *pts, const uint8_t *neg, size_t n, uint32_t *out, uint8_t *out_inf);

}
```

Baseline: 449.2.

## Use radix 13·2^16 signed digits for precomputed c=20, W=13 MSM

Result: no change. 451.8 (median of 4 runs) (+0.6%).

```diff
diff --git a/crypto_amd/csrc/k_g1_pre.hip b/crypto_amd/csrc/k_g1_pre.hip
--- a/crypto_amd/csrc/k_g1_pre.hip
+++ b/crypto_amd/csrc/k_g1_pre.hip
@@ -1,10 +1,10 @@
 #include "pre_kernels.hip.h"
 #include "msm_launch.hip.h"
 namespace msm {
-template <class C> void launch_pre_step(hipStream_t s, const uint32_t *prev, size_t n, int c, uint32_t *tmp, uint32_t *out) {
-    hipLaunchKernelGGL((k_pre_dbl<typename C::MSM>), dim3((unsigned)((n + 63) / 64)), dim3(64), 0, s, prev, n, c, tmp);
+template <class C> void launch_pre_step(hipStream_t s, const uint32_t *prev, size_t n, int c, bool mul13, uint32_t *tmp, uint32_t *out) {
+    hipLaunchKernelGGL((k_pre_dbl<typename C::MSM>), dim3((unsigned)((n + 63) / 64)), dim3(64), 0, s, prev, n, c, mul13 ? 1 : 0, tmp);
     const size_t groups = (n + PRE_GROUP - 1) / PRE_GROUP;
     hipLaunchKernelGGL((k_pre_norm<typename C::MSM>), dim3((unsigned)((groups + 63) / 64)), dim3(64), 0, s, prev, (const uint32_t *)tmp, n, out);
 }
-template void launch_pre_step<G1>(hipStream_t, const uint32_t *, size_t, int, uint32_t *, uint32_t *);
+template void launch_pre_step<G1>(hipStream_t, const uint32_t *, size_t, int, bool, uint32_t *, uint32_t *);
 }
diff --git a/crypto_amd/csrc/k_g2_pre.hip b/crypto_amd/csrc/k_g2_pre.hip
--- a/crypto_amd/csrc/k_g2_pre.hip
+++ b/crypto_amd/csrc/k_g2_pre.hip
@@ -1,10 +1,10 @@
 #include "pre_kernels.hip.h"
 #include "msm_launch.hip.h"
 namespace msm {
-template <class C> void launch_pre_step(hipStream_t s, const uint32_t *prev, size_t n, int c, uint32_t *tmp, uint32_t *out) {
-    hipLaunchKernelGGL((k_pre_dbl<typename C::MSM>), dim3((unsigned)((n + 63) / 64)), dim3(64), 0, s, prev, n, c, tmp);
+template <class C> void launch_pre_step(hipStream_t s, const uint32_t *prev, size_t n, int c, bool mul13, uint32_t *tmp, uint32_t *out) {
+    hipLaunchKernelGGL((k_pre_dbl<typename C::MSM>), dim3((unsigned)((n + 63) / 64)), dim3(64), 0, s, prev, n, c, mul13 ? 1 : 0, tmp);
     const size_t groups = (n + PRE_GROUP - 1) / PRE_GROUP;
     hipLaunchKernelGGL((k_pre_norm<typename C::MSM>), dim3((unsigned)((groups + 63) / 64)), dim3(64), 0, s, prev, (const uint32_t *)tmp, n, out);
 }
-template void launch_pre_step<G2>(hipStream_t, const uint32_t *, size_t, int, uint32_t *, uint32_t *);
+template void launch_pre_step<G2>(hipStream_t, const uint32_t *, size_t, int, bool, uint32_t *, uint32_t *);
 }
diff --git a/crypto_amd/csrc/k_psort.hip b/crypto_amd/csrc/k_psort.hip
--- a/crypto_amd/csrc/k_psort.hip
+++ b/crypto_amd/csrc/k_psort.hip
@@ -5,6 +5,9 @@
 namespace msm {
 void launch_id_flags(hipStream_t s, const uint32_t *bases, int aff_stride, int flag_word, size_t n, uint8_t *out) {
     if (n) hipLaunchKernelGGL(k_id_flags, dim3((unsigned)((n + 255) / 256)), dim3(256), 0, s, bases, aff_stride, flag_word, n, out);
+}
+void launch_id_rows(hipStream_t s, const uint32_t *tab, int aff_stride, int flag_word, size_t n, int W, uint8_t *out) {
+    if (n) hipLaunchKernelGGL(k_id_rows, dim3((unsigned)((n + 255) / 256)), dim3(256), 0, s, tab, aff_stride, flag_word, n, W, out);
 }
 void launch_raw_record_hash(hipStream_t s, const uint8_t *raw, size_t stride, size_t x_off, size_t y_off, size_t inf_off, const uint8_t *is_inf, int words, size_t n, uint64_t *out) {
     if (n) hipLaunchKernelGGL(k_raw_record_hash, dim3((unsigned)((n + 255) / 256)), dim3(256), 0, s, raw, stride, x_off, y_off, inf_off, is_inf, words, n, out);
@@ -17,17 +20,20 @@
       if (!(done.load() & bit)) {
           (void)hipFuncSetAttribute((const void *)k_ps_scatter1<0, 0>, hipFuncAttributeMaxDynamicSharedMemorySize, 160 * 1024 - 2048);
           (void)hipFuncSetAttribute((const void *)k_ps_scatter1<20, 13>, hipFuncAttributeMaxDynamicSharedMemorySize, 160 * 1024 - 2048);
+          (void)hipFuncSetAttribute((const void *)k_ps_scatter1<PS_R13, 13>, hipFuncAttributeMaxDynamicSharedMemorySize, 160 * 1024 - 2048);
           (void)hipFuncSetAttribute((const void *)k_ps_scatter1<17, 16>, hipFuncAttributeMaxDynamicSharedMemorySize, 160 * 1024 - 2048);
           (void)hipFuncSetAttribute((const void *)k_ps_scatter1<16, 16>, hipFuncAttributeMaxDynamicSharedMemorySize, 160 * 1024 - 2048);
           done.fetch_or(bit); } }
-    const int shape = (q.c == 20 && q.W == 13) ? 1 : ((q.c == 17 && q.W == 16) ? 2 : ((q.c == 16 && q.W == 16) ? 3 : 0));
-    if (shape == 1) hipLaunchKernelGGL((k_ps_count1<20, 13>), dim3(q.ntiles), dim3(PS_TILE), lds1, s, q, cnt1);
+    const int shape = q.radix13 ? 4 : (q.c == 20 && q.W == 13) ? 1 : ((q.c == 17 && q.W == 16) ? 2 : ((q.c == 16 && q.W == 16) ? 3 : 0));
+    if (shape == 4) hipLaunchKernelGGL((k_ps_count1<PS_R13, 13>), dim3(q.ntiles), dim3(PS_TILE), lds1, s, q, cnt1);
+    else if (shape == 1) hipLaunchKernelGGL((k_ps_count1<20, 13>), dim3(q.ntiles), dim3(PS_TILE), lds1, s, q, cnt1);
     else if (shape == 2) hipLaunchKernelGGL((k_ps_count1<17, 16>), dim3(q.ntiles), dim3(PS_TILE), lds1, s, q, cnt1);
     else if (shape == 3) hipLaunchKernelGGL((k_ps_count1<16, 16>), dim3(q.ntiles), dim3(PS_TILE), lds1, s, q, cnt1);
     else hipLaunchKernelGGL((k_ps_count1<0, 0>), dim3(q.ntiles), dim3(PS_TILE), lds1, s, q, cnt1);
     launch_scan(s, cnt1, off1, nullptr, bsums, (size_t)q.P * q.ntiles);
     if (dyn) launch_dyn_chunk(s, off1 + (size_t)q.P * q.ntiles, dyn_args[0], dyn_args[1], dyn_args[2], dyn_args[3], dyn_args[4], dyn, dyn_args[5]);
-    if (shape == 1) hipLaunchKernelGGL((k_ps_scatter1<20, 13>), dim3(q.ntiles), dim3(PS_TILE), lds3, s, q, (const uint32_t *)cnt1, (const uint32_t *)off1, (uint2 *)pairs);
+    if (shape == 4) hipLaunchKernelGGL((k_ps_scatter1<PS_R13, 13>), dim3(q.ntiles), dim3(PS_TILE), lds3, s, q, (const uint32_t *)cnt1, (const uint32_t *)off1, (uint2 *)pairs);
+    else if (shape == 1) hipLaunchKernelGGL((k_ps_scatter1<20, 13>), dim3(q.ntiles), dim3(PS_TILE), lds3, s, q, (const uint32_t *)cnt1, (const uint32_t *)off1, (uint2 *)pairs);
     else if (shape == 2) hipLaunchKernelGGL((k_ps_scatter1<17, 16>), dim3(q.ntiles), dim3(PS_TILE), lds3, s, q, (const uint32_t *)cnt1, (const uint32_t *)off1, (uint2 *)pairs);
     else if (shape == 3) hipLaunchKernelGGL((k_ps_scatter1<16, 16>), dim3(q.ntiles), dim3(PS_TILE), lds3, s, q, (const uint32_t *)cnt1, (const uint32_t *)off1, (uint2 *)pairs);
     else hipLaunchKernelGGL((k_ps_scatter1<0, 0>), dim3(q.ntiles), dim3(PS_TILE), lds3, s, q, (const uint32_t *)cnt1, (const uint32_t *)off1, (uint2 *)pairs);
diff --git a/crypto_amd/csrc/msm_driver.hip.h b/crypto_amd/csrc/msm_driver.hip.h
--- a/crypto_amd/csrc/msm_driver.hip.h
+++ b/crypto_amd/csrc/msm_driver.hip.h
@@ -6,6 +6,7 @@
 #include "host_field.hpp"
 #include "msm_launch.hip.h"
 #include "sort_launch.hip.h"
+#include "radix13.hip.h"
 #include "qap_launch.hip.h"
 
 namespace dock {
@@ -239,7 +240,7 @@
             StageTimer st(sl, "msm.psort");
             PsParams q;
             q.scalars = scalars_k; q.idflag = nullptr ; q.n = nk; q.flag_base = 0;
-            q.c = c; q.W = W; q.key_wstride = g.B; q.val_base = 0; q.val_wstride = 0;
+            q.c = c; q.W = W; q.radix13 = 0; q.key_wstride = g.B; q.val_base = 0; q.val_wstride = 0;
             q.part_log = ps_part_log(NB); q.P = (NB + (1u << q.part_log) - 1) >> q.part_log; q.ntiles = (uint32_t)((nk + PS_TILE - 1) / PS_TILE);
             q.bad = sl.flags.as<uint32_t>();
             const uint32_t dyn_args[6] = {(uint32_t)forced_chunk(), g.min_chunk, g.max_chunks, g.lanes_per_chunk, (uint32_t)T, 0u};
@@ -395,14 +396,15 @@
     memcpy(out_xyz, &X, sizeof(HF)); memcpy(out_xyz + FWORDS, &Y, sizeof(HF)); memcpy(out_xyz + 2 * FWORDS, &Z, sizeof(HF));
 }
 
-struct PreGeom { uint32_t NB; int mshift, lb, PW, G; size_t NG, Emax, T; int CH; uint32_t min_chunk, max_chunks, lanes_per_chunk, HEAVY_CAP; };
+struct PreGeom { uint32_t NB; bool r13 ; int mshift, lb, PW, G; size_t NG, Emax, T; int CH; uint32_t min_chunk, max_chunks, lanes_per_chunk, HEAVY_CAP; };
 template <class C> int32_t pre_geometry(const PreTable &pt, size_t n, PreGeom &g) {
     const int c = pt.c, W = pt.W;
-    g.NB = 1u << (c - 1);
+    g.r13 = msm::r13_shape(c, W);
+    g.NB = msm::pre_buckets(c, W);
     g.mshift = g.NB >= (1u << 18) ? 3 : (g.NB >= (1u << 17) ? 2 : (g.NB >= (1u << 16) ? 1 : 0));
-    if (g.NB >= (1u << 19) && cur().busy.load() >= 3) g.mshift = 4;
-    { const int f = gs.reduce_shift.load(); if (f >= 0 && c - 1 >= 6 + f) g.mshift = f; }
-    g.lb = std::min(c - 1, 12 + g.mshift);
+    if (g.NB >= msm::R13_NB && cur().busy.load() >= 3) g.mshift = 4;
+    { const int f = gs.reduce_shift.load(); if (f >= 0 && c - 1 >= 6 + f && g.NB % (64u << f) == 0) g.mshift = f; }
+    g.lb = msm::pre_lb(c, W, g.mshift);
     g.PW = (int)(g.NB >> g.lb);
     g.G = 1 << (g.lb - 6 - g.mshift);
     g.NG = (size_t)g.PW * g.G;
@@ -448,14 +450,14 @@
 template <class C> inline size_t pre_rows_bytes(size_t n, int W) { return (size_t)W * n * C::AFF_STRIDE * 4; }
 template <class C> inline size_t pre_tab_bytes(size_t n, int W) { return pre_rows_bytes<C>(n, W) + ((n + 15) & ~(size_t)15); }
 template <class C> inline const uint8_t *pre_idflags(const PreTable &pt) { return (const uint8_t *)pt.tab + pre_rows_bytes<C>(pt.n, pt.W); }
-inline size_t pre_off_bytes(const PreTable &pt) { return (((size_t)1 << (pt.c - 1)) + 1) * 4; }
+inline size_t pre_off_bytes(const PreTable &pt) { return ((size_t)msm::pre_buckets(pt.c, pt.W) + 1) * 4; }
 inline size_t pre_entries_bytes(const PreTable &pt, size_t n) { return (size_t)n * pt.W * 4; }
 
 template <class C>
 int32_t pre_sort(Slot &sl, const PreTable &pt, const PreGeom &g, size_t boff, const uint32_t *d_scalars, size_t n, uint32_t *off, uint32_t *entries, uint32_t *dyn, bool reset_flag = true) {
     PsParams q;
     q.scalars = d_scalars; q.idflag = dyn ? pre_idflags<C>(pt) : nullptr ; q.n = n; q.flag_base = (uint32_t)boff;
-    q.c = pt.c; q.W = pt.W; q.key_wstride = 0; q.val_base = (uint32_t)boff; q.val_wstride = (uint32_t)pt.n;
+    q.c = pt.c; q.W = pt.W; q.radix13 = g.r13 ? 1 : 0; q.key_wstride = 0; q.val_base = (uint32_t)boff; q.val_wstride = (uint32_t)pt.n;
     q.part_log = ps_part_log(g.NB); q.P = (g.NB + (1u << q.part_log) - 1) >> q.part_log; q.ntiles = (uint32_t)((n + PS_TILE - 1) / PS_TILE);
     int32_t rc;
     if ((rc = ws_pre<C>(sl, pt, g, n))) return rc;
@@ -662,8 +664,10 @@
         if (!rc && hipMemcpyAsync(tab, hd.p, n * rec, hipMemcpyDeviceToDevice, sl.stream) != hipSuccess) rc = DGPU_E_HIP;
         if (!rc) {
             StageTimer st(sl, "msm.precompute");
-            for (int w = 1; w < W; w++) launch_pre_step<C>(sl.stream, (const uint32_t *)tab + (size_t)(w - 1) * n * C::AFF_STRIDE, n, c, (uint32_t *)tmp, (uint32_t *)tab + (size_t)w * n * C::AFF_STRIDE);
-            launch_id_flags(sl.stream, (const uint32_t *)tab, C::AFF_STRIDE, C::FLAGW, n, (uint8_t *)tab + pre_rows_bytes<C>(n, W));
+            const bool r13 = msm::r13_shape(c, W);
+            for (int w = 1; w < W; w++) launch_pre_step<C>(sl.stream, (const uint32_t *)tab + (size_t)(w - 1) * n * C::AFF_STRIDE, n, r13 ? msm::R13_DBL : c, r13, (uint32_t *)tmp, (uint32_t *)tab + (size_t)w * n * C::AFF_STRIDE);
+            if (r13) launch_id_rows(sl.stream, (const uint32_t *)tab, C::AFF_STRIDE, C::FLAGW, n, W, (uint8_t *)tab + pre_rows_bytes<C>(n, W));
+            else launch_id_flags(sl.stream, (const uint32_t *)tab, C::AFF_STRIDE, C::FLAGW, n, (uint8_t *)tab + pre_rows_bytes<C>(n, W));
         }
         if (!rc && (hipGetLastError() != hipSuccess || hipStreamSynchronize(sl.stream) != hipSuccess)) rc = DGPU_E_HIP;
         if (gs.prof) prof_flush(sl);
diff --git a/crypto_amd/csrc/msm_launch.hip.h b/crypto_amd/csrc/msm_launch.hip.h
--- a/crypto_amd/csrc/msm_launch.hip.h
+++ b/crypto_amd/csrc/msm_launch.hip.h
@@ -39,7 +39,7 @@
                                         uint8_t *partial_inf, uint32_t *count, uint32_t *win, uint8_t *win_inf, bool abi, uint32_t *bad_flag);
 template <class C> void launch_seg_fold(hipStream_t s, const uint32_t *win, const uint8_t *win_inf, size_t nseg, uint32_t *out_xyz, uint8_t *out_inf);
 
-template <class C> void launch_pre_step(hipStream_t s, const uint32_t *prev, size_t n, int c, uint32_t *tmp, uint32_t *out);
+template <class C> void launch_pre_step(hipStream_t s, const uint32_t *prev, size_t n, int c, bool mul13, uint32_t *tmp, uint32_t *out);
 template <class C> void launch_reduce_top_s(hipStream_t s, unsigned W, const uint32_t *l1, const uint8_t *l1_inf, int G, int gshift, uint32_t *win_abi, uint8_t *win_inf, uint32_t *win_s_abi, uint8_t *win_s_inf, int lanes);
 
 }
diff --git a/crypto_amd/csrc/msm_launch_impl.hip.h b/crypto_amd/csrc/msm_launch_impl.hip.h
--- a/crypto_amd/csrc/msm_launch_impl.hip.h
+++ b/crypto_amd/csrc/msm_launch_impl.hip.h
@@ -50,7 +50,7 @@
     for (int quad = 0; quad < 2; quad++) {
         int PL, KK; red_levels<C>(quad != 0, PL, KK);
         size_t total = (size_t)(RG::K + 2) * NG, cnt = NG; int nm = RG::K;
-        while (cnt > 1) { const int steps = std::min(KK, red_log2((unsigned)cnt)); const size_t chunks = std::max<size_t>(1, cnt / PL); nm += steps; total += (size_t)(nm + 2) * chunks; cnt = chunks; }
+        while (cnt > 1) { const int steps = red_fold_steps((unsigned)cnt, KK); const size_t chunks = red_fold_chunks((unsigned)cnt, PL); nm += steps; total += (size_t)(nm + 2) * chunks; cnt = chunks; }
         best = std::max(best, total + 64);
     }
     return best;
@@ -62,8 +62,8 @@
     unsigned cnt = NG; int nm = RG::K;
     uint32_t *in = cls; uint8_t *in_inf = cls_inf;
     while (cnt > 1) {
-        const int steps = std::min(KK, red_log2(cnt));
-        const unsigned chunks = std::max(1u, cnt / (unsigned)PL), npairs = 1u + (unsigned)(nm + 1) / 2u, waves = npairs * chunks;
+        const int steps = red_fold_steps(cnt, KK);
+        const unsigned chunks = red_fold_chunks(cnt, PL), npairs = 1u + (unsigned)(nm + 1) / 2u, waves = npairs * chunks;
         uint32_t *out = in + (size_t)(nm + 2) * cnt * A::XW; uint8_t *out_inf = in_inf + (size_t)(nm + 2) * cnt;
         if (quad) hipLaunchKernelGGL((k_reduce_cls_quad<A>), dim3(waves), dim3(256 * A::LPP), 0, s, (const uint32_t *)in, (const uint8_t *)in_inf, cnt, nm, out, out_inf, chunks == 1 ? 1 : 0, win_abi, win_inf);
         else hipLaunchKernelGGL((k_reduce_cls<A>), dim3((waves + 3) / 4), dim3(256), 0, s, (const uint32_t *)in, (const uint8_t *)in_inf, cnt, nm, out, out_inf, chunks == 1 ? 1 : 0, win_abi, win_inf);
diff --git a/crypto_amd/csrc/pre_kernels.hip.h b/crypto_amd/csrc/pre_kernels.hip.h
--- a/crypto_amd/csrc/pre_kernels.hip.h
+++ b/crypto_amd/csrc/pre_kernels.hip.h
@@ -2,6 +2,7 @@
 #include <hip/hip_runtime.h>
 #include "msm_kernels.hip.h"
 #include "fp_inv.hip.h"
+#include "radix13.hip.h"
 
 namespace msm {
 using namespace bls29;
@@ -22,7 +23,7 @@
 }
 
 template <class C>
-__global__ void __launch_bounds__(64) k_pre_dbl(const uint32_t *__restrict__ prev, size_t n, int c, uint32_t *__restrict__ tmp) {
+__global__ void __launch_bounds__(64) k_pre_dbl(const uint32_t *__restrict__ prev, size_t n, int c, int mul13, uint32_t *__restrict__ tmp) {
     typedef typename C::F F;
     const size_t i = (size_t)blockIdx.x * blockDim.x + threadIdx.x;
     if (i >= n) return;
@@ -31,6 +32,11 @@
     Aff<F> p; load_aff<C>(p, rec);
     Xyzz<F> acc; xyzz_dbl_affine(acc, p);
     for (int k = 1; k < c; k++) { Xyzz<F> d; xyzz_dbl(d, acc); acc = d; }
+    if (mul13) {
+        Xyzz<F> q = acc; bool inf;
+        xyzz_mul13(acc, inf, q);
+        if (inf) { fzero(acc.x); fzero(acc.y); fzero(acc.zz); fzero(acc.zzz); }
+    }
     uint32_t *dst = tmp + i * C::XW;
     const uint32_t *w = reinterpret_cast<const uint32_t *>(&acc);
 #pragma unroll
@@ -50,11 +56,17 @@
     const size_t i0 = t * PRE_GROUP;
     if (i0 >= n) return;
     Fp pre[PRE_GROUP], run; fp_set_one(run);
-    bool live[PRE_GROUP];
+    bool live[PRE_GROUP], gone[PRE_GROUP];
 #pragma unroll
     for (int k = 0; k < PRE_GROUP; k++) {
         const size_t i = i0 + k;
         live[k] = i < n && prev[i * C::AFF_STRIDE + C::FLAGW] == 0;
+        gone[k] = false;
+        if (live[k]) {
+            const uint32_t *src = tmp + i * C::XW + 3 * C::FW; uint32_t any = 0;
+            for (int j = 0; j < C::FW; j++) any |= src[j];
+            if (any == 0) { live[k] = false; gone[k] = true; }
+        }
         pre[k] = run;
         if (live[k]) {
             F zzz; const uint32_t *src = tmp + i * C::XW + 3 * C::FW; uint32_t *w = reinterpret_cast<uint32_t *>(&zzz);
@@ -69,6 +81,7 @@
         const size_t i = i0 + k;
         if (i >= n) continue;
         uint32_t *dst = out + i * C::AFF_STRIDE;
+        if (gone[k]) { for (int j = 0; j < C::AFF_STRIDE; j++) dst[j] = 0u; dst[C::FLAGW] = 1u; continue; }
         if (!live[k]) { for (int j = 0; j < C::AFF_STRIDE; j++) dst[j] = prev[i * C::AFF_STRIDE + j]; continue; }
         Xyzz<F> p; load_xyzz_aos<C>(p, tmp + i * C::XW);
         Fp key, kinv, ni; inv_key(key, p.zzz);
diff --git a/crypto_amd/csrc/psort_kernels.hip.h b/crypto_amd/csrc/psort_kernels.hip.h
--- a/crypto_amd/csrc/psort_kernels.hip.h
+++ b/crypto_amd/csrc/psort_kernels.hip.h
@@ -3,6 +3,7 @@
 #include <hip/hip_runtime.h>
 #include <stdint.h>
 #include "sort_launch.hip.h"
+#include "radix13.hip.h"
 
 namespace msm {
 
@@ -21,12 +22,17 @@
     return active ? atomicAdd(&cnt[bin], 1u) : 0u;
 }
 
-template <int CC, int CW, class F> __device__ __forceinline__ void ps_digits(const PsParams &q, size_t i, bool live, F f) {
+constexpr int PS_R13 = -13;
+template <int CC, int CW, class F> __device__ __forceinline__ void ps_digits(const PsParams &q, size_t i, uint32_t rows, F f) {
+    const bool live = rows != 0;
     uint4 a = make_uint4(0, 0, 0, 0), b = a;
     if (live) { const uint4 *p = reinterpret_cast<const uint4 *>(q.scalars + i * 8); a = p[0]; b = p[1]; }
     uint32_t s[8] = {a.x, a.y, a.z, a.w, b.x, b.y, b.z, b.w & 0x7fffffffu};
     uint32_t carry = 0;
-    if constexpr (CC != 0) {
+    if constexpr (CC == PS_R13) {
+        (void)carry;
+        (void)radix13_digits(s, [&](int w, uint32_t m1, uint32_t neg, bool nz) { f(w, m1, neg, nz && (uint32_t)w < rows); });
+    } else if constexpr (CC != 0) {
         constexpr uint32_t B = 1u << (CC - 1);
 #pragma unroll
         for (int w = 0; w < CW; w++) {
@@ -63,8 +69,18 @@
         }
     }
 }
-__device__ __forceinline__ bool ps_live(const PsParams &q, size_t i) {
-    return i < q.n && (!q.idflag || q.idflag[(size_t)q.flag_base + i] == 0);
+__device__ __forceinline__ uint32_t ps_live(const PsParams &q, size_t i) {
+    if (i >= q.n) return 0;
+    const uint32_t v = q.idflag ? q.idflag[(size_t)q.flag_base + i] : 0u;
+    return v ? v - 1u : (uint32_t)q.W;
+}
+
+__global__ void __launch_bounds__(256) k_id_rows(const uint32_t *__restrict__ tab, int aff_stride, int flag_word, size_t n, int W, uint8_t *__restrict__ out) {
+    const size_t i = (size_t)blockIdx.x * blockDim.x + threadIdx.x;
+    if (i >= n) return;
+    uint32_t v = 0;
+    for (int w = W - 1; w >= 0; w--) if (tab[((size_t)w * n + i) * (size_t)aff_stride + flag_word] != 0) v = (uint32_t)w + 1u;
+    out[i] = (uint8_t)v;
 }
 
 __global__ void __launch_bounds__(256) k_id_flags(const uint32_t *__restrict__ bases, int aff_stride, int flag_word, size_t n, uint8_t *__restrict__ out) {
@@ -120,7 +136,7 @@
     const uint32_t tile = ps_tile_of_block(blockIdx.x, q.ntiles);
     for (uint32_t j = threadIdx.x; j < q.P; j += blockDim.x) { const size_t idx = (size_t)j * q.ntiles + tile; const uint32_t o0 = off1[idx], o1 = off1[idx + 1]; goff[j] = o0; cnt[j] = o1 - o0; }
     const size_t i = (size_t)tile * PS_TILE + threadIdx.x;
-    const bool live = ps_live(q, i);
+    const uint32_t live = ps_live(q, i);
     __syncthreads();
     {
         const uint32_t per = (q.P + PS_TILE - 1) / PS_TILE;
diff --git a/crypto_amd/csrc/radix13.hip.h b/crypto_amd/csrc/radix13.hip.h
--- /dev/null
+++ b/crypto_amd/csrc/radix13.hip.h
@@ -0,0 +1,77 @@
+#pragma once
+#include <stddef.h>
+#include <stdint.h>
+
+#if defined(__HIPCC__)
+#define R13_FD __host__ __device__ __forceinline__
+#else
+#define R13_FD inline
+#endif
+
+namespace msm {
+
+constexpr int R13_C = 20, R13_W = 13;
+constexpr uint32_t R13_RADIX = 13u << 16;
+constexpr uint32_t R13_NB = 13u << 15;
+constexpr int R13_DBL = 16;
+
+R13_FD bool r13_shape(int c, int W) { return c == R13_C && W == R13_W; }
+R13_FD uint32_t pre_buckets(int c, int W) { return r13_shape(c, W) ? R13_NB : 1u << (c - 1); }
+
+R13_FD uint32_t r13_div169(uint32_t limb, uint32_t &rem) {
+    const uint32_t t = rem * 113u, s = limb + t, co = s < t ? 1u : 0u;
+    const uint32_t v = s + (co ? 113u : 0u), qq = v / 169u;
+    const uint32_t q = (rem + co) * 25414007u + qq;
+    rem = v - qq * 169u;
+    return q;
+}
+
+template <class F> R13_FD bool radix13_digits(const uint32_t (&k)[8], F f) {
+    uint32_t s[8];
+#if defined(__HIPCC__)
+#pragma unroll
+#endif
+    for (int j = 0; j < 8; j++) s[j] = k[j];
+    const bool over = (s[7] >> 31) != 0;
+    s[7] &= 0x7fffffffu;
+    uint32_t carry = 0;
+    auto emit = [&](int w, uint32_t raw) {
+        const uint32_t v = raw + carry;
+        const uint32_t neg = v > R13_NB ? 1u : 0u;
+        const uint32_t mag = neg ? R13_RADIX - v : v;
+        carry = neg;
+        f(w, mag - 1u, neg, mag != 0u);
+    };
+#if defined(__HIPCC__)
+#pragma unroll
+#endif
+    for (int j = 0; j < 6; j++) {
+        uint32_t rem = 0;
+#if defined(__HIPCC__)
+#pragma unroll
+#endif
+        for (int i = 7; i > j; i--) s[i] = r13_div169(s[i], rem);
+        const uint32_t t = (rem << 16) | (s[j] >> 16), hi = t / 13u;
+        emit(2 * j, ((t - hi * 13u) << 16) | (s[j] & 0xffffu));
+        emit(2 * j + 1, hi);
+    }
+    emit(12, s[6]);
+    return over;
+}
+
+template <class PT> R13_FD void xyzz_mul13(PT &r, bool &rinf, const PT &q) {
+    PT q2, q4;
+    xyzz_dbl(q2, q);
+    xyzz_dbl(q4, q2);
+    xyzz_dbl(r, q4);
+    rinf = false;
+    xyzz_add(r, rinf, q4, false);
+    xyzz_add(r, rinf, q, false);
+}
+
+R13_FD int pre_lb(int c, int W, int mshift) { const int cap = r13_shape(c, W) ? 15 : c - 1, lb = 12 + mshift; return lb < cap ? lb : cap; }
+
+R13_FD unsigned red_fold_chunks(unsigned cnt, int PL) { return (cnt + (unsigned)PL - 1u) / (unsigned)PL; }
+R13_FD int red_fold_steps(unsigned cnt, int K) { int s = 0; while (s < K && (1u << s) < cnt) s++; return s; }
+
+}
diff --git a/crypto_amd/csrc/reduce_kernels.hip.h b/crypto_amd/csrc/reduce_kernels.hip.h
--- a/crypto_amd/csrc/reduce_kernels.hip.h
+++ b/crypto_amd/csrc/reduce_kernels.hip.h
@@ -1,5 +1,6 @@
 #pragma once
 #include "msm_kernels.hip.h"
+#include "radix13.hip.h"
 
 namespace msm {
 
@@ -12,7 +13,7 @@
 __host__ __device__ inline int red_log2(unsigned v) { int r = 0; while ((1u << (r + 1)) <= v) r++; return r; }
 inline size_t reduce_m_points(size_t NG, int PL, int K) {
     size_t total = (size_t)(K + 2) * NG; size_t cnt = NG; int nm = K;
-    while (cnt > 1) { const int steps = std::min(K, red_log2((unsigned)cnt)); const size_t chunks = std::max<size_t>(1, cnt / PL); nm += steps; total += (size_t)(nm + 2) * chunks; cnt = chunks; }
+    while (cnt > 1) { const int steps = red_fold_steps((unsigned)cnt, K); const size_t chunks = red_fold_chunks((unsigned)cnt, PL); nm += steps; total += (size_t)(nm + 2) * chunks; cnt = chunks; }
     return total + 64;
 }
 
@@ -101,8 +102,8 @@
     typedef typename C::F F;
     constexpr int LPP = RedGeom<C>::LPP, PL = RedGeom<C>::PL, K = RedGeom<C>::K;
     const int lane = threadIdx.x & 63, pl = lane / LPP, h = lane % LPP;
-    const unsigned chunks = cnt / PL ? cnt / PL : 1u;
-    const int steps = red_log2(cnt) < K ? red_log2(cnt) : K;
+    const unsigned chunks = red_fold_chunks(cnt, PL);
+    const int steps = red_fold_steps(cnt, K);
     const unsigned npairs = 1u + (unsigned)(nm + 1) / 2u;
     const unsigned w = blockIdx.x * (blockDim.x >> 6) + (threadIdx.x >> 6);
     const unsigned pair = w / chunks, j = w % chunks;
@@ -157,8 +158,8 @@
     __shared__ uint8_t fl[64];
     const int t = (int)threadIdx.x, gi = t / GL, h = t % LPP;
     const QuadLanes<LPP> q4;
-    const unsigned chunks = cnt / PLQ ? cnt / PLQ : 1u;
-    const int steps = red_log2(cnt) < 6 ? red_log2(cnt) : 6;
+    const unsigned chunks = red_fold_chunks(cnt, PLQ);
+    const int steps = red_fold_steps(cnt, 6);
     const unsigned pair = blockIdx.x / chunks, j = blockIdx.x % chunks;
     const unsigned c0 = pair == 0 ? 0u : 2u * pair, c1 = c0 + 1;
     const bool has1 = c1 < 2u + (unsigned)nm;
diff --git a/crypto_amd/csrc/sort_launch.hip.h b/crypto_amd/csrc/sort_launch.hip.h
--- a/crypto_amd/csrc/sort_launch.hip.h
+++ b/crypto_amd/csrc/sort_launch.hip.h
@@ -29,6 +29,7 @@
     size_t n;
     uint32_t flag_base;
     int c, W;
+    int radix13;
     uint32_t key_wstride;
     uint32_t val_base, val_wstride;
     int part_log;
@@ -41,6 +42,7 @@
 void launch_psort(hipStream_t s, const PsParams &q, uint32_t NB, uint32_t *cnt1, uint32_t *off1, uint32_t *bsums, void *pairs, uint32_t *off, uint32_t *entries,
                   uint32_t heavy_thr, uint32_t *heavy, uint32_t heavy_cap, const uint32_t *dyn_args = nullptr, uint32_t *dyn = nullptr);
 void launch_id_flags(hipStream_t s, const uint32_t *bases, int aff_stride, int flag_word, size_t n, uint8_t *out);
+void launch_id_rows(hipStream_t s, const uint32_t *tab, int aff_stride, int flag_word, size_t n, int W, uint8_t *out);
 void launch_raw_record_hash(hipStream_t s, const uint8_t *raw, size_t stride, size_t x_off, size_t y_off, size_t inf_off, const uint8_t *is_inf, int words, size_t n, uint64_t *out);
 void launch_g1_scale(hipStream_t s, const uint32_t *p_abi, const uint8_t *is_inf, const uint32_t *scalars, int scalar_stride, const uint8_t *negate, size_t n, uint32_t *out_abi, uint8_t *out_inf,
                      const uint32_t *add_abi = nullptr, const uint8_t *add_inf = nullptr);
```
